# cc-ai/MUNIT

Hardware: AMD Instinct MI355X
Metric: images/sec (gen_update+dis_update) @256x256 bs=8 (higher is better)
Workload: dtype f32; 1 GPU; config_256.yaml AdaINGen_double+MsImageDis dis_update+gen_update, 256x256, per-GPU batch 8, fp32; global_batch=8, parallelism=dp1, gen_state=1

## Files before the change

### include/munit_hip.h

```cpp
#ifndef MUNIT_HIP_H
#define MUNIT_HIP_H

#include <stddef.h>
#include <stdint.h>

#ifdef __cplusplus
extern "C" {
#endif

typedef void* munit_stream_t;

enum { MUNIT_OK = 0, MUNIT_ERR_ARG = -1, MUNIT_ERR_WORKSPACE = -2, MUNIT_ERR_LAUNCH = -3 };
enum { MUNIT_ACT_NONE = 0, MUNIT_ACT_RELU = 1, MUNIT_ACT_LRELU = 2, MUNIT_ACT_TANH = 3 };
enum { MUNIT_PAD_ZERO = 0, MUNIT_PAD_REFLECT = 1 };
enum { MUNIT_COMPUTE_F32 = 0, MUNIT_COMPUTE_BF16 = 1, MUNIT_COMPUTE_F32X3 = 2 };
enum { MUNIT_DTYPE_F32 = 0, MUNIT_DTYPE_BF16 = 1 };

int munit_version(void);
const char* munit_last_error(void);

typedef void* munit_comm_t;
int munit_comm_unique_id(void* id_out, size_t bytes);
int munit_comm_init(munit_comm_t* comm, int rank, int world, const void* unique_id);
int munit_comm_allreduce(munit_comm_t comm, float* buf, size_t count, munit_stream_t stream);
int munit_comm_destroy(munit_comm_t comm);
int munit_shutdown(void);

int munit_stream_wait_stream(munit_stream_t waiter, munit_stream_t signaler);

typedef struct {
  int B, H, W, Cin;
  int Cout, KH, KW;
  int stride, pad, pad_mode;
  int upsample;
  int act;
  float slope;
  int compute;
  int in_dtype, out_dtype;
} munit_conv_desc;

int munit_conv2d_out_hw(const munit_conv_desc* d, int* Ho, int* Wo);

size_t munit_conv2d_fwd_workspace_bytes(const munit_conv_desc* d);
int munit_conv2d_fwd(const munit_conv_desc* d, const void* x, const float* w, const float* bias,
                     void* y, void* ws, size_t ws_bytes, munit_stream_t stream);

size_t munit_conv2d_dgrad_workspace_bytes(const munit_conv_desc* d);
int munit_conv2d_dgrad(const munit_conv_desc* d, const void* dy, const float* w, const void* add,
                       void* dx, void* ws, size_t ws_bytes, munit_stream_t stream);

size_t munit_conv2d_wgrad_workspace_bytes(const munit_conv_desc* d);
int munit_conv2d_wgrad(const munit_conv_desc* d, const void* x, const void* dy, float* dw,
                       float* db, float beta, void* ws, size_t ws_bytes, munit_stream_t stream);

enum { MUNIT_PASS_FWD = 0, MUNIT_PASS_DGRAD = 1, MUNIT_PASS_WGRAD = 2 };
enum { MUNIT_PREP_NONE = 0, MUNIT_PREP_DGRAD = 1, MUNIT_PREP_SUBPIXEL = 2, MUNIT_PREP_CAST = 3,
       MUNIT_PREP_WINOGRAD = 4, MUNIT_PREP_WINOGRAD_DGRAD = 5, MUNIT_PREP_SUBPIXEL_WINOGRAD = 6,
       MUNIT_PREP_WINOGRAD_S2 = 7, MUNIT_PREP_WINOGRAD_S2_DGRAD = 8,
       MUNIT_PREP_SUBPIXEL_WINOGRAD_DGRAD = 9  };
typedef struct {
  const float* w;
  float* wp;
  int Cout, KH, KW, Cin;
  int kind;
  int ps;
  int bf16;
} munit_prep_item;
size_t munit_conv2d_prepared_weight_bytes(const munit_conv_desc* d, int pass);
int munit_conv2d_prep_item(const munit_conv_desc* d, int pass, const float* w, float* wp, munit_prep_item* out);
int munit_conv2d_prepare_weights(const munit_prep_item* item, munit_stream_t stream);
int munit_conv2d_prepare_weights_batch(const munit_prep_item* items_dev, int n, munit_stream_t stream);
int munit_conv2d_fwd_prepared(const munit_conv_desc* d, const void* x, const float* w, const void* wp,
                              const float* bias, void* y, void* ws, size_t ws_bytes, munit_stream_t stream);
int munit_conv2d_dgrad_prepared(const munit_conv_desc* d, const void* dy, const float* w, const void* wp,
                                const void* add, void* dx, void* ws, size_t ws_bytes, munit_stream_t stream);

size_t munit_linear_workspace_bytes(int B, int K, int N);
int munit_linear_fwd(const float* x, const float* w, const float* bias, float* y, int B, int K, int N, int act,
                     float slope, void* ws, size_t ws_bytes, munit_stream_t stream);
int munit_linear_bwd(const float* x, const float* w, const float* dy, float* dx, float* dw, float* db, int B, int K,
                     int N, float beta, void* ws, size_t ws_bytes, munit_stream_t stream);

double munit_conv2d_executed_flops(const munit_conv_desc* d, int pass);
const char* munit_conv2d_kernel_name(const munit_conv_desc* d, int pass);

int munit_act_bwd(int act, float slope, const float* y, const float* dy, float* dx, size_t n,
                  munit_stream_t stream);

size_t munit_instnorm_workspace_bytes(int B, int HW, int C);
int munit_instnorm_fwd(const float* x, float* y, float* stats, int B, int HW, int C,
                       const float* adain, int ad_ld, int w_off, int b_off, const float* residual,
                       int relu, float eps, void* ws, size_t ws_bytes, munit_stream_t stream);
int munit_instnorm_bwd(const float* x, const float* dy, const float* stats, float* dx, int B, int HW,
                       int C, const float* adain, float* d_adain, int ad_ld, int w_off, int b_off,
                       int relu, void* ws, size_t ws_bytes, munit_stream_t stream);

int munit_instnorm_route(int B, int HW, int C, int dtype);

int munit_instnorm_fwd_bf16(const void* x, void* y, float* stats, int B, int HW, int C,
                            const float* adain, int ad_ld, int w_off, int b_off, const void* residual,
                            int relu, float eps, void* ws, size_t ws_bytes, munit_stream_t stream);
int munit_instnorm_bwd_bf16(const void* x, const void* dy, const float* stats, void* dx, int B, int HW,
                            int C, const float* adain, float* d_adain, int ad_ld, int w_off, int b_off,
                            int relu, void* ws, size_t ws_bytes, munit_stream_t stream);

size_t munit_layernorm_workspace_bytes(int B, int HW, int C);
int munit_layernorm_fwd(const float* x, float* y, float* stats, int B, int HW, int C,
                        const float* gamma, const float* beta, int relu, float eps, void* ws,
                        size_t ws_bytes, munit_stream_t stream);
int munit_layernorm_bwd(const float* x, const float* dy, const float* stats, float* dx, int B, int HW,
                        int C, const float* gamma, const float* beta, float* dgamma, float* dbeta,
                        float acc, int relu, float eps, void* ws, size_t ws_bytes,
                        munit_stream_t stream);

int munit_layernorm_fwd_bf16(const void* x, void* y, float* stats, int B, int HW, int C,
                             const float* gamma, const float* beta, int relu, float eps, void* ws,
                             size_t ws_bytes, munit_stream_t stream);
int munit_layernorm_bwd_bf16(const void* x, const void* dy, const float* stats, void* dx, int B, int HW,
                             int C, const float* gamma, const float* beta, float* dgamma, float* dbeta,
                             float acc, int relu, float eps, void* ws, size_t ws_bytes,
                             munit_stream_t stream);

int munit_avgpool3s2_fwd(const float* x, float* y, int B, int H, int W, int C, munit_stream_t stream);
int munit_avgpool3s2_bwd(const float* dy, float* dx, int B, int H, int W, int C, munit_stream_t stream);
int munit_gap_fwd(const float* x, float* y, int B, int HW, int C, munit_stream_t stream);
int munit_gap_bwd(const float* dy, float* dx, int B, int HW, int C, munit_stream_t stream);

size_t munit_loss_workspace_bytes(size_t n);
int munit_l1_mean_fwd(const float* a, const float* b, const float* mask, size_t npix, int C, float* out,
                      void* ws, size_t ws_bytes, munit_stream_t stream);
int munit_l1_mean_bwd(const float* a, const float* b, const float* mask, size_t npix, int C,
                      const float* gout, float* da, float* db, munit_stream_t stream);
int munit_l1_mean_fwd_bf16(const void* a, const void* b, const float* mask, size_t npix, int C, float* out,
                           void* ws, size_t ws_bytes, munit_stream_t stream);
int munit_l1_mean_bwd_bf16(const void* a, const void* b, const float* mask, size_t npix, int C,
                           const float* gout, void* da, void* db, munit_stream_t stream);
int munit_pair_l1_fwd(const float* x_a, const float* x_b, const float* x_ab, const float* x_ba, size_t npix, int C,
                      float* out, void* ws, size_t ws_bytes, munit_stream_t stream);
int munit_pair_l1_bwd(const float* x_a, const float* x_b, const float* x_ab, const float* x_ba, size_t npix, int C,
                      const float* gout, float* dx_ab, float* dx_ba, munit_stream_t stream);
int munit_mse_const_fwd(const float* x, float target, size_t n, float* out, void* ws, size_t ws_bytes,
                        munit_stream_t stream);
int munit_mse_const_bwd(const float* x, float target, size_t n, const float* gout, float* dx,
                        munit_stream_t stream);
size_t munit_lsgan_workspace_bytes(int nseg);
int munit_lsgan_fwd(const float* const* x, const size_t* n, const float* target, int nseg, float* out, float* seg_out,
                    void* ws, size_t ws_bytes, munit_stream_t stream);
int munit_lsgan_bwd(const float* const* x, const size_t* n, const float* target, int nseg, const float* gout,
                    float* const* dx, munit_stream_t stream);
size_t munit_nsgan_workspace_bytes(int nseg);
int munit_nsgan_fwd(const float* const* x, const size_t* n, const float* target, int nseg, float* out, float* seg_out,
                    void* ws, size_t ws_bytes, munit_stream_t stream);
int munit_nsgan_bwd(const float* const* x, const size_t* n, const float* target, int nseg, const float* gout,
                    float* const* dx, munit_stream_t stream);
int munit_weighted_sum(const float* const* terms, const float* w, int n, float* out,
                       munit_stream_t stream);

int munit_adam_step(float* p, const float* g, float* m, float* v, size_t n, double lr, double beta1,
                    double beta2, double eps, double weight_decay, int step, munit_stream_t stream);

int munit_extraadam_step(float* p, const float* g, float* m, float* v, float* p_saved, size_t n, double lr,
                         double beta1, double beta2, double eps, double weight_decay, int step, int mode,
                         munit_stream_t stream);

int munit_scale(const float* x, float* y, size_t n, float alpha, int accumulate, munit_stream_t stream);

typedef struct {
  long long src_off;
  int src_h, src_w;
  int rs_h, rs_w;
  int crop_i, crop_j;
  int flip;
  int kind;
} munit_image_desc;

int munit_image_ksize(int src_size, int rs_size);
size_t munit_image_preprocess_workspace_bytes(int B, int out_h, int out_w, int ksize_max);
int munit_image_preprocess(const unsigned char* pool, const munit_image_desc* descs, int B, int out_h,
                           int out_w, int ksize_max, float* out, void* ws, size_t ws_bytes,
                           munit_stream_t stream);
size_t munit_mask_preprocess_workspace_bytes(int B, int out_h, int out_w);
int munit_mask_preprocess(const unsigned char* pool, const munit_image_desc* descs, int B, int out_h,
                          int out_w, float* out, void* ws, size_t ws_bytes, munit_stream_t stream);
size_t munit_label_preprocess_workspace_bytes(int N, int out_h, int out_w);
int munit_label_preprocess(const unsigned char* pool, const munit_image_desc* descs, int N, int out_h,
                           int out_w, float* out, void* ws, size_t ws_bytes, munit_stream_t stream);

typedef struct {
  const float* data;
  int n;
  int channels;
  int layout;
} munit_grid_src;

size_t munit_image_grid_workspace_bytes(int nsrc, int H, int W, int nrow);
int munit_image_grid_u8(const munit_grid_src* src, int nsrc, int H, int W, int nrow, float pre_add, float pre_mul,
                        unsigned char* out, void* ws, size_t ws_bytes, munit_stream_t stream);

int munit_seg_input_fwd(const float* x, float* y, size_t npix, munit_stream_t stream);
int munit_seg_input_bwd(const float* dy, float* dx, size_t npix, munit_stream_t stream);
int munit_space_to_batch(const float* x, float* y, int N, int H, int W, int C, int f, int inverse, munit_stream_t stream);
int munit_maxpool3s2_fwd(const float* x, float* y, unsigned char* idx, int B, int H, int W, int C, munit_stream_t stream);
int munit_maxpool3s2_bwd(const float* dy, const unsigned char* idx, float* dx, int B, int H, int W, int C,
                         munit_stream_t stream);
int munit_add_relu_fwd(const float* a, const float* r, float* y, size_t n, munit_stream_t stream);
size_t munit_seg_ce_workspace_bytes(int B, int h, int w, int S);
int munit_seg_ce_fwd(const float* logits, const int* labels, const float* mask, int B, int h, int w, int S, float norm,
                     float* out, void* ws, size_t ws_bytes, munit_stream_t stream);
int munit_seg_ce_bwd(const float* logits, const int* labels, const float* mask, int B, int h, int w, int S, float norm,
                     const float* gout, float* dlogits, void* ws, size_t ws_bytes, munit_stream_t stream);
int munit_seg_ce_gt_fwd(const float* logits, const float* gt, const float* mask, int B, int h, int w, int S, float norm,
                        float* out, void* ws, size_t ws_bytes, munit_stream_t stream);
int munit_seg_ce_gt_bwd(const float* logits, const float* gt, const float* mask, int B, int h, int w, int S, float norm,
                        const float* gout, float* dlogits, void* ws, size_t ws_bytes, munit_stream_t stream);

size_t munit_seg_ce_direct_workspace_bytes(int B, int h, int w, int S, int K);
int munit_seg_ce_direct_fwd(const float* logits, const float* gt, int B, int h, int w, int S, int K, float norm, float* out,
                            void* ws, size_t ws_bytes, munit_stream_t stream);
int munit_seg_ce_direct_bwd(const float* logits, const float* gt, int B, int h, int w, int S, int K, float norm,
                            const float* gout, float* dlogits, void* ws, size_t ws_bytes, munit_stream_t stream);
int munit_avgpool7_fwd(const float* x, float* y, int B, int H, int W, int C, munit_stream_t stream);
int munit_avgpool7_bwd(const float* dy, float* dx, int B, int H, int W, int C, munit_stream_t stream);
int munit_seg_labels(const float* logits, int B, int h, int w, int S, int* labels, munit_stream_t stream);

size_t munit_batchnorm_workspace_bytes(int C);
int munit_batchnorm_fwd(const float* x, float* y, float* mean, float* rstd, float* running_mean, float* running_var,
                        long long R, int C, const float* gamma, const float* beta, int relu, int eval, float eps,
                        float momentum, void* ws, size_t ws_bytes, munit_stream_t stream);
int munit_batchnorm_bwd(const float* x, const float* dy, const float* y, const float* gamma, const float* mean,
                        const float* rstd, float* dx, float* dgamma, float* dbeta, float acc, long long R, int C,
                        int relu, void* ws, size_t ws_bytes, munit_stream_t stream);
size_t munit_batchnorm_dp_workspace_bytes(int C);
int munit_batchnorm_dp_stats_local(const float* x, long long R_local, int C, int W, int rank, float* xch, size_t xch_floats,
                                   void* ws, size_t ws_bytes, munit_stream_t stream);
int munit_batchnorm_dp_fwd_apply(const float* x, float* y, float* mean, float* rstd, float* running_mean, float* running_var,
                                 long long R_local, int C, int W, const float* xch, size_t xch_floats, const float* gamma,
                                 const float* beta, int relu, float eps, float momentum, munit_stream_t stream);
// ... 52 lines not shown
```

### munit_amd/_lib.py

```python
import ctypes
import os
from ctypes import POINTER, Structure, c_char_p, c_double, c_float, c_int, c_size_t, c_void_p

_HERE = os.path.dirname(os.path.abspath(__file__))
LIB_PATH = os.environ.get("MUNIT_HIP_LIB") or os.path.join(_HERE, "libmunit_hip.so")

ACT = {"none": 0, "relu": 1, "lrelu": 2, "tanh": 3}
PAD = {"zero": 0, "reflect": 1}
COMPUTE = {"f32": 0, "bf16": 1, "f32x3": 2}
DTYPE = {"f32": 0, "bf16": 1}


class ConvDesc(Structure):
    _fields_ = [("B", c_int), ("H", c_int), ("W", c_int), ("Cin", c_int),
                ("Cout", c_int), ("KH", c_int), ("KW", c_int),
                ("stride", c_int), ("pad", c_int), ("pad_mode", c_int),
                ("upsample", c_int), ("act", c_int), ("slope", c_float), ("compute", c_int),
                ("in_dtype", c_int), ("out_dtype", c_int)]


class PrepItem(Structure):
    _fields_ = [("w", c_void_p), ("wp", c_void_p), ("Cout", c_int), ("KH", c_int), ("KW", c_int), ("Cin", c_int),
                ("kind", c_int), ("ps", c_int), ("bf16", c_int)]


class ImageDesc(Structure):
    _fields_ = [("src_off", ctypes.c_longlong), ("src_h", c_int), ("src_w", c_int), ("rs_h", c_int), ("rs_w", c_int),
                ("crop_i", c_int), ("crop_j", c_int), ("flip", c_int), ("kind", c_int)]


class GemmProblem(Structure):
    _fields_ = [("A", c_void_p), ("B", c_void_p), ("C", c_void_p)]


class GridSrc(Structure):
    _fields_ = [("data", c_void_p), ("n", c_int), ("channels", c_int), ("layout", c_int)]


class RectDesc(Structure):
    _fields_ = [("B", c_int), ("H", c_int), ("W", c_int), ("Cin", c_int), ("x_ld", c_int), ("Cout", c_int), ("y_ld", c_int),
                ("KH", c_int), ("KW", c_int), ("stride", c_int), ("pad_h", c_int), ("pad_w", c_int), ("relu", c_int)]


WINDOW = {"max": 0, "avg": 1}
RECT_TILES = ("128x128", "64x64", "128x64")

_P = c_void_p
_DESC = POINTER(ConvDesc)

SIGNATURES = {
    "munit_version": (c_int, []),
    "munit_last_error": (c_char_p, []),
    "munit_stream_wait_stream": (c_int, [_P, _P]),
    "munit_comm_unique_id": (c_int, [_P, c_size_t]),
    "munit_comm_init": (c_int, [_P, c_int, c_int, _P]),
    "munit_comm_allreduce": (c_int, [_P, _P, c_size_t, _P]),
    "munit_comm_destroy": (c_int, [_P]),
    "munit_shutdown": (c_int, []),
    "munit_conv2d_out_hw": (c_int, [_DESC, POINTER(c_int), POINTER(c_int)]),
    "munit_conv2d_fwd_workspace_bytes": (c_size_t, [_DESC]),
    "munit_conv2d_fwd": (c_int, [_DESC, _P, _P, _P, _P, _P, c_size_t, _P]),
    "munit_conv2d_dgrad_workspace_bytes": (c_size_t, [_DESC]),
    "munit_conv2d_dgrad": (c_int, [_DESC, _P, _P, _P, _P, _P, c_size_t, _P]),
    "munit_conv2d_wgrad_workspace_bytes": (c_size_t, [_DESC]),
    "munit_conv2d_wgrad": (c_int, [_DESC, _P, _P, _P, _P, c_float, _P, c_size_t, _P]),
    "munit_conv2d_prepared_weight_bytes": (c_size_t, [_DESC, c_int]),
    "munit_conv2d_prep_item": (c_int, [_DESC, c_int, _P, _P, POINTER(PrepItem)]),
    "munit_conv2d_prepare_weights": (c_int, [POINTER(PrepItem), _P]),
    "munit_conv2d_prepare_weights_batch": (c_int, [_P, c_int, _P]),
    "munit_conv2d_fwd_prepared": (c_int, [_DESC, _P, _P, _P, _P, _P, _P, c_size_t, _P]),
    "munit_conv2d_dgrad_prepared": (c_int, [_DESC, _P, _P, _P, _P, _P, _P, c_size_t, _P]),
    "munit_conv2d_executed_flops": (c_double, [_DESC, c_int]),
    "munit_conv2d_kernel_name": (c_char_p, [_DESC, c_int]),
    "munit_linear_workspace_bytes": (c_size_t, [c_int, c_int, c_int]),
    "munit_linear_fwd": (c_int, [_P, _P, _P, _P, c_int, c_int, c_int, c_int, c_float, _P, c_size_t, _P]),
    "munit_linear_bwd": (c_int, [_P, _P, _P, _P, _P, _P, c_int, c_int, c_int, c_float, _P, c_size_t, _P]),
    "munit_act_bwd": (c_int, [c_int, c_float, _P, _P, _P, c_size_t, _P]),
    "munit_instnorm_workspace_bytes": (c_size_t, [c_int, c_int, c_int]),
    "munit_instnorm_route": (c_int, [c_int, c_int, c_int, c_int]),
    "munit_instnorm_fwd": (c_int, [_P, _P, _P, c_int, c_int, c_int, _P, c_int, c_int, c_int, _P, c_int,
                                   c_float, _P, c_size_t, _P]),
    "munit_instnorm_bwd": (c_int, [_P, _P, _P, _P, c_int, c_int, c_int, _P, _P, c_int, c_int, c_int, c_int,
                                   _P, c_size_t, _P]),
    "munit_instnorm_fwd_bf16": (c_int, [_P, _P, _P, c_int, c_int, c_int, _P, c_int, c_int, c_int, _P, c_int,
                                        c_float, _P, c_size_t, _P]),
    "munit_instnorm_bwd_bf16": (c_int, [_P, _P, _P, _P, c_int, c_int, c_int, _P, _P, c_int, c_int, c_int, c_int,
                                        _P, c_size_t, _P]),
    "munit_layernorm_workspace_bytes": (c_size_t, [c_int, c_int, c_int]),
    "munit_layernorm_fwd": (c_int, [_P, _P, _P, c_int, c_int, c_int, _P, _P, c_int, c_float, _P, c_size_t, _P]),
    "munit_layernorm_bwd": (c_int, [_P, _P, _P, _P, c_int, c_int, c_int, _P, _P, _P, _P, c_float, c_int,
                                    c_float, _P, c_size_t, _P]),
    "munit_layernorm_fwd_bf16": (c_int, [_P, _P, _P, c_int, c_int, c_int, _P, _P, c_int, c_float, _P, c_size_t, _P]),
    "munit_layernorm_bwd_bf16": (c_int, [_P, _P, _P, _P, c_int, c_int, c_int, _P, _P, _P, _P, c_float, c_int,
                                         c_float, _P, c_size_t, _P]),
    "munit_avgpool3s2_fwd": (c_int, [_P, _P, c_int, c_int, c_int, c_int, _P]),
    "munit_avgpool3s2_bwd": (c_int, [_P, _P, c_int, c_int, c_int, c_int, _P]),
    "munit_gap_fwd": (c_int, [_P, _P, c_int, c_int, c_int, _P]),
    "munit_gap_bwd": (c_int, [_P, _P, c_int, c_int, c_int, _P]),
    "munit_loss_workspace_bytes": (c_size_t, [c_size_t]),
    "munit_l1_mean_fwd": (c_int, [_P, _P, _P, c_size_t, c_int, _P, _P, c_size_t, _P]),
    "munit_l1_mean_bwd": (c_int, [_P, _P, _P, c_size_t, c_int, _P, _P, _P, _P]),
    "munit_l1_mean_fwd_bf16": (c_int, [_P, _P, _P, c_size_t, c_int, _P, _P, c_size_t, _P]),
    "munit_l1_mean_bwd_bf16": (c_int, [_P, _P, _P, c_size_t, c_int, _P, _P, _P, _P]),
    "munit_pair_l1_fwd": (c_int, [_P, _P, _P, _P, c_size_t, c_int, _P, _P, c_size_t, _P]),
    "munit_pair_l1_bwd": (c_int, [_P, _P, _P, _P, c_size_t, c_int, _P, _P, _P, _P]),
    "munit_mse_const_fwd": (c_int, [_P, c_float, c_size_t, _P, _P, c_size_t, _P]),
    "munit_mse_const_bwd": (c_int, [_P, c_float, c_size_t, _P, _P, _P]),
    "munit_lsgan_workspace_bytes": (c_size_t, [c_int]),
    "munit_lsgan_fwd": (c_int, [POINTER(c_void_p), POINTER(c_size_t), POINTER(c_float), c_int, _P, _P, _P, c_size_t, _P]),
    "munit_lsgan_bwd": (c_int, [POINTER(c_void_p), POINTER(c_size_t), POINTER(c_float), c_int, _P, POINTER(c_void_p), _P]),
    "munit_nsgan_workspace_bytes": (c_size_t, [c_int]),
    "munit_nsgan_fwd": (c_int, [POINTER(c_void_p), POINTER(c_size_t), POINTER(c_float), c_int, _P, _P, _P, c_size_t, _P]),
    "munit_nsgan_bwd": (c_int, [POINTER(c_void_p), POINTER(c_size_t), POINTER(c_float), c_int, _P, POINTER(c_void_p), _P]),
    "munit_weighted_sum": (c_int, [POINTER(c_void_p), POINTER(c_float), c_int, _P, _P]),
    "munit_adam_step": (c_int, [_P, _P, _P, _P, c_size_t, c_double, c_double, c_double, c_double, c_double, c_int,
                                _P]),
    "munit_extraadam_step": (c_int, [_P, _P, _P, _P, _P, c_size_t, c_double, c_double, c_double, c_double,
                                     c_double, c_int, c_int, _P]),
    "munit_scale": (c_int, [_P, _P, c_size_t, c_float, c_int, _P]),
    "munit_image_ksize": (c_int, [c_int, c_int]),
    "munit_image_preprocess_workspace_bytes": (c_size_t, [c_int, c_int, c_int, c_int]),
    "munit_image_preprocess": (c_int, [_P, _P, c_int, c_int, c_int, c_int, _P, _P, c_size_t, _P]),
    "munit_mask_preprocess_workspace_bytes": (c_size_t, [c_int, c_int, c_int]),
    "munit_mask_preprocess": (c_int, [_P, _P, c_int, c_int, c_int, _P, _P, c_size_t, _P]),
    "munit_label_preprocess_workspace_bytes": (c_size_t, [c_int, c_int, c_int]),
    "munit_label_preprocess": (c_int, [_P, _P, c_int, c_int, c_int, _P, _P, c_size_t, _P]),
    "munit_image_grid_workspace_bytes": (c_size_t, [c_int, c_int, c_int, c_int]),
    "munit_image_grid_u8": (c_int, [POINTER(GridSrc), c_int, c_int, c_int, c_int, c_float, c_float, _P, _P, c_size_t, _P]),
    "munit_seg_input_fwd": (c_int, [_P, _P, c_size_t, _P]),
    "munit_seg_input_bwd": (c_int, [_P, _P, c_size_t, _P]),
    "munit_space_to_batch": (c_int, [_P, _P, c_int, c_int, c_int, c_int, c_int, c_int, _P]),
    "munit_maxpool3s2_fwd": (c_int, [_P, _P, _P, c_int, c_int, c_int, c_int, _P]),
    "munit_maxpool3s2_bwd": (c_int, [_P, _P, _P, c_int, c_int, c_int, c_int, _P]),
    "munit_add_relu_fwd": (c_int, [_P, _P, _P, c_size_t, _P]),
    "munit_seg_ce_workspace_bytes": (c_size_t, [c_int, c_int, c_int, c_int]),
    "munit_seg_ce_fwd": (c_int, [_P, _P, _P, c_int, c_int, c_int, c_int, c_float, _P, _P, c_size_t, _P]),
    "munit_seg_ce_bwd": (c_int, [_P, _P, _P, c_int, c_int, c_int, c_int, c_float, _P, _P, _P, c_size_t, _P]),
    "munit_seg_ce_gt_fwd": (c_int, [_P, _P, _P, c_int, c_int, c_int, c_int, c_float, _P, _P, c_size_t, _P]),
    "munit_seg_ce_gt_bwd": (c_int, [_P, _P, _P, c_int, c_int, c_int, c_int, c_float, _P, _P, _P, c_size_t, _P]),
    "munit_seg_labels": (c_int, [_P, c_int, c_int, c_int, c_int, _P, _P]),
    "munit_seg_ce_direct_workspace_bytes": (c_size_t, [c_int, c_int, c_int, c_int, c_int]),
    "munit_seg_ce_direct_fwd": (c_int, [_P, _P, c_int, c_int, c_int, c_int, c_int, c_float, _P, _P, c_size_t, _P]),
    "munit_seg_ce_direct_bwd": (c_int, [_P, _P, c_int, c_int, c_int, c_int, c_int, c_float, _P, _P, _P, c_size_t, _P]),
    "munit_avgpool7_fwd": (c_int, [_P, _P, c_int, c_int, c_int, c_int, _P]),
    "munit_avgpool7_bwd": (c_int, [_P, _P, c_int, c_int, c_int, c_int, _P]),
    "munit_batchnorm_workspace_bytes": (c_size_t, [c_int]),
    "munit_batchnorm_fwd": (c_int, [_P, _P, _P, _P, _P, _P, ctypes.c_longlong, c_int, _P, _P, c_int, c_int, c_float, c_float,
                                    _P, c_size_t, _P]),
    "munit_batchnorm_bwd": (c_int, [_P, _P, _P, _P, _P, _P, _P, _P, _P, c_float, ctypes.c_longlong, c_int, c_int, _P,
                                    c_size_t, _P]),
    "munit_batchnorm_dp_workspace_bytes": (c_size_t, [c_int]),
    "munit_batchnorm_dp_stats_local": (c_int, [_P, ctypes.c_longlong, c_int, c_int, c_int, _P, c_size_t, _P, c_size_t, _P]),
    "munit_batchnorm_dp_fwd_apply": (c_int, [_P, _P, _P, _P, _P, _P, ctypes.c_longlong, c_int, c_int, _P, c_size_t, _P, _P,
                                             c_int, c_float, c_float, _P]),
    "munit_batchnorm_dp_bwd_local": (c_int, [_P, _P, _P, _P, _P, ctypes.c_longlong, c_int, c_int, c_int, c_int, _P, c_size_t,
                                             _P, c_size_t, _P]),
    "munit_batchnorm_dp_bwd_finish": (c_int, [_P, _P, _P, _P, _P, _P, _P, _P, _P, c_float, ctypes.c_longlong, c_int, c_int,
                                              c_int, c_int, _P, c_size_t, _P, c_size_t, _P]),
    "munit_maxpool2_fwd": (c_int, [_P, _P, _P, c_int, c_int, c_int, c_int, _P]),
    "munit_maxpool2_bwd": (c_int, [_P, _P, _P, c_int, c_int, c_int, c_int, _P]),
    "munit_avgpool16_fwd": (c_int, [_P, _P, c_int, c_int, c_int, c_int, _P]),
    "munit_avgpool16_bwd": (c_int, [_P, _P, c_int, c_int, c_int, c_int, _P]),
    "munit_gemm_f32": (c_int, [POINTER(GemmProblem), c_int, c_int, c_int, c_int, c_int, c_int, c_int, c_int, c_float,
                               c_float, _P]),
    "munit_fid_moments_workspace_bytes": (c_size_t, [c_int, c_int]),
    "munit_fid_moments": (c_int, [_P, c_int, c_int, _P, _P, _P, c_size_t, _P]),
    "munit_sqrt_newton_schulz_workspace_bytes": (c_size_t, [c_int, c_int]),
    "munit_sqrt_newton_schulz": (c_int, [_P, c_int, c_int, c_int, _P, _P, c_size_t, _P]),
    "munit_frechet_distance_workspace_bytes": (c_size_t, [c_int]),
    "munit_frechet_distance": (c_int, [_P, _P, _P, _P, c_int, c_int, _P, _P, c_size_t, _P]),
    "munit_conv2d_rect_out_hw": (c_int, [POINTER(RectDesc), POINTER(c_int), POINTER(c_int)]),
    "munit_conv2d_rect_tile": (c_int, [POINTER(RectDesc)]),
    "munit_conv2d_rect_fwd": (c_int, [POINTER(RectDesc), _P, _P, _P, _P, c_int, _P]),
    "munit_window3_fwd": (c_int, [_P, _P, c_int, c_int, c_int, c_int, c_int, c_int, c_int, c_int, c_int, _P]),
    "munit_inception_input": (c_int, [_P, c_int, c_int, c_int, c_int, _P, _P]),
}

_lib = None


def load():
    global _lib
    if _lib is not None:
        return _lib
    if not os.path.exists(LIB_PATH):
        raise RuntimeError(
            "munit_amd: %s not found. Build it with `python -c 'import __graft_entry__ as g; g.build()'` "
            "(or `make -C munit_amd/csrc`). There is no CPU / PyTorch fallback." % LIB_PATH)
    lib = ctypes.CDLL(LIB_PATH)
    for name, (res, args) in SIGNATURES.items():
        try:
            fn = getattr(lib, name)
        except AttributeError as e:
            raise RuntimeError("munit_amd: %s does not export %s" % (LIB_PATH, name)) from e
        fn.restype = res
        fn.argtypes = args
    _lib = lib
    return lib


def check(rc, what=""):
    if rc != 0:
        msg = load().munit_last_error()
        raise RuntimeError("munit_hip %s failed (rc=%d): %s" % (what, rc, (msg or b"").decode()))
```

### munit_amd/csrc/common.h

```cpp
#pragma once
#include <hip/hip_runtime.h>
#include <cstdarg>
#include <cstdio>
#include <cstdlib>
#include "../../include/munit_hip.h"

typedef float f32x4 __attribute__((ext_vector_type(4)));
typedef float f32x16 __attribute__((ext_vector_type(16)));

typedef __bf16 bf16_t;
typedef __bf16 bf16v4 __attribute__((ext_vector_type(4)));
typedef __bf16 bf16v8 __attribute__((ext_vector_type(8)));

__device__ inline f32x4 ld4(const float* p) { return *reinterpret_cast<const f32x4*>(p); }
__device__ inline f32x4 ld4(const bf16_t* p) {
  const bf16v4 h = *reinterpret_cast<const bf16v4*>(p);
  return f32x4{(float)h[0], (float)h[1], (float)h[2], (float)h[3]};
}
__device__ inline void st4(float* p, f32x4 v) { *reinterpret_cast<f32x4*>(p) = v; }
__device__ inline void st4(bf16_t* p, f32x4 v) {
  *reinterpret_cast<bf16v4*>(p) = bf16v4{(bf16_t)v[0], (bf16_t)v[1], (bf16_t)v[2], (bf16_t)v[3]};
}
__device__ inline float ld1(const float* p) { return *p; }
__device__ inline float ld1(const bf16_t* p) { return (float)*p; }
__device__ inline void st1(float* p, float v) { *p = v; }
__device__ inline void st1(bf16_t* p, float v) { *p = (bf16_t)v; }

void munit_set_error(const char* fmt, ...);

#define MUNIT_CHECK_ARG(cond, ...)         \
  do {                                     \
    if (!(cond)) {                         \
      munit_set_error(__VA_ARGS__);        \
      return MUNIT_ERR_ARG;                \
    }                                      \
  } while (0)

#define MUNIT_CHECK_LAUNCH(what)                                                   \
  do {                                                                             \
    hipError_t e_ = hipGetLastError();                                             \
    if (e_ != hipSuccess) {                                                        \
      munit_set_error("%s: launch failed: %s", what, hipGetErrorString(e_));       \
      return MUNIT_ERR_LAUNCH;                                                     \
    }                                                                              \
  } while (0)

#define MUNIT_ENV_FLAG(name) ([]() -> bool { static const bool v_ = getenv(name) != nullptr; return v_; }())

static inline size_t align_up(size_t v, size_t a) { return (v + a - 1) / a * a; }
static inline int cdiv(long long a, long long b) { return (int)((a + b - 1) / b); }

__device__ inline float wave_sum(float v) {
#pragma unroll
  for (int off = 32; off > 0; off >>= 1) v += __shfl_xor(v, off, 64);
  return v;
}

__device__ inline float apply_act(float v, int act, float slope) {
  if (act == MUNIT_ACT_RELU) return v > 0.f ? v : 0.f;
  if (act == MUNIT_ACT_LRELU) return v > 0.f ? v : v * slope;
  if (act == MUNIT_ACT_TANH) return tanhf(v);
  return v;
}

__device__ inline int src_coord(int v, int Hu, int ups, int reflect) {
  const bool inside = v >= 0 && v < Hu;
  int r = v < 0 ? -v : v;
  r = r >= Hu ? 2 * Hu - 2 - r : r;
  r = reflect ? r : (inside ? v : -1);
  return r < 0 ? -1 : (r >> ups);
}

double munit_igemm_executed_flops(const munit_conv_desc* d, int pass);
const char* munit_igemm_kernel_name(const munit_conv_desc* d, int pass);

bool munit_small_fwd_supported(const munit_conv_desc* d);
bool munit_small_fwd_ok(const munit_conv_desc* d);
bool munit_small_wgrad_ok(const munit_conv_desc* d);
enum SmallFwdKernel { SMALL_FWD_PK, SMALL_FWD_MFMA, SMALL_FWD_PATCH };
SmallFwdKernel munit_small_fwd_kernel(int Cin);
bool munit_small_wgrad_pk();
size_t munit_small_fwd_workspace(const munit_conv_desc* d);
int munit_small_fwd(const munit_conv_desc* d, int Ho, int Wo, const void* x, const float* w, const float* bias,
                    float* y, void* ws, hipStream_t st);
size_t munit_small_wgrad_workspace(const munit_conv_desc* d, int Ho);
int munit_small_wgrad(const munit_conv_desc* d, int Ho, int Wo, const void* x, const float* dy, float* dw,
                      float* db, float beta, void* ws, hipStream_t st);
```

### munit_amd/csrc/conv_igemm.hip

```cpp
#include "common.h"
#include "wino.h"
#include <cstdlib>

namespace {

struct IgemmParams {
  const float* x;
  const float* w;
  const float* bias;
  void* y;
  int B, H, W, Cin;
  int Hu, Wu, ups;
  int Ho, Wo, Cout;
  int KH, KW, stride, pad, reflect;
  int Ktot;
  long long w_row;
  long long y_sb;
  long long y_sh;
  int y_sw;
  int M;
  int act;
  float slope;
  int ps;
  long long w_phase;
  long long y_phase_row;
  int y_phase_col;
  int n_tiles;
  int f_pad, f_ups, f_reflect, f_Hu, f_Wu;
  int frame;
  int ksplit, kt_per_split;
  float* slab;
  int ct;
  int patch;
  int out_bf16;
  int bf16s;
  int cin4;
};

__device__ inline f32x4 bf16x8_add4(f32x4 l, f32x4 a, f32x4 b, f32x4 c) {
  const bf16v8 L = __builtin_bit_cast(bf16v8, l), A = __builtin_bit_cast(bf16v8, a), B = __builtin_bit_cast(bf16v8, b),
               C = __builtin_bit_cast(bf16v8, c);
  bf16v8 r;
#pragma unroll
  for (int e = 0; e < 8; ++e) r[e] = (bf16_t)((float)L[e] + (((float)A[e] + (float)B[e]) + (float)C[e]));
  return __builtin_bit_cast(f32x4, r);
}

__device__ inline void decode_pixel(int m, int Ho, int Wo, int frame, int& b, int& oh, int& ow) {
  if (!frame) {
    const int HoWo = Ho * Wo;
    b = m / HoWo;
    const int rem = m - b * HoWo;
    oh = rem / Wo;
    ow = rem - oh * Wo;
  } else {
    const int F = frame, F2 = 2 * frame;
    const int nb = F2 * Wo + F2 * (Ho - F2);
    b = m / nb;
    int r = m - b * nb;
    if (r < F2 * Wo) {
      const int q = r / Wo;
      ow = r - q * Wo;
      oh = q < F ? q : Ho - F2 + q;
    } else {
      r -= F2 * Wo;
      const int rr = r / F2, q = r - rr * F2;
      oh = F + rr;
      ow = q < F ? q : Wo - F2 + q;
    }
  }
}

constexpr int BM = 128;
constexpr int BK = 32;
#ifndef IGEMM_WAVES
#define IGEMM_WAVES 8
#endif
constexpr int NWAVES = IGEMM_WAVES;
constexpr int NTHR = 64 * NWAVES;
constexpr int LDS_LD = BK + 4;

__device__ inline uint2 fold_cands(int i, int Hu, int ups, int P, int reflect) {
  unsigned long long pk = ~0ull;
  int n = 0;
  auto push = [&](int v) {
    if (n < 4) {
      const int sh = 16 * n;
      pk = (pk & ~(0xFFFFull << sh)) | ((unsigned long long)(unsigned)v << sh);
      ++n;
    }
  };
  const int nu = 1 << ups;
  for (int du = 0; du < nu; ++du) {
    const int hu = (i << ups) + du;
    push(hu + P);
    if (reflect) {
      if (hu >= 1 && hu <= P) push(P - hu);
      if (hu >= Hu - 1 - P && hu <= Hu - 2) push(2 * Hu - 2 - hu + P);
    }
  }
  return make_uint2((unsigned)(pk & 0xFFFFFFFFull), (unsigned)(pk >> 32));
}
__device__ inline int cand_at(uint2 v, int a) {
  const unsigned w = (a & 2) ? v.y : v.x;
  return (int)((w >> ((a & 1) * 16)) & 0xFFFFu);
}

typedef __bf16 bf16x4 __attribute__((ext_vector_type(4)));
typedef __bf16 bf16x8 __attribute__((ext_vector_type(8)));

__device__ const float munit_zero_page[32] = {0.f};

template <int BN, bool ALIGNED, int ROLE, int CT = 0>
__global__ __launch_bounds__(NTHR, NWAVES == 8 ? ((CT == 3 && BN == 64) ? 6 : 4) : 2) void conv_igemm_kernel(IgemmParams p) {
  constexpr bool BF16 = CT == 1 || CT == 2;
  constexpr bool DMA = CT == 3 || CT == 4 || CT == 5;
  constexpr bool BF16S = CT == 4;
  constexpr bool CIN4 = CT == 5;
  static_assert(!CIN4 || ROLE != 2, "4-channel taps: single-gather roles only");
  static_assert(!DMA || (ALIGNED && NWAVES == 8), "direct-to-LDS loads: aligned variants only");
  constexpr bool PATCH = DMA && ROLE == 2;
  constexpr int NPL = CT == 2 ? 3 : 1;
  static_assert(!BF16 || ALIGNED, "bf16 operands need Cin % 32 == 0");
  constexpr int WN = NWAVES == 8 ? 32 : 64;
  constexpr int WAVES_N = BN / WN;
  constexpr int WAVES_M = NWAVES / WAVES_N;
  constexpr int WM = BM / WAVES_M;
  constexpr int MT = WM / 16;
  constexpr int NT = WN / 16;
#ifndef IGEMM_LOADER_WAVES
#define IGEMM_LOADER_WAVES 8
#endif
  constexpr int LW = (CT == 3 && ROLE != 2 && NWAVES == 8) ? IGEMM_LOADER_WAVES : NWAVES;
  constexpr int RSTEP = 64 * LW / 8;
  constexpr int AROWS = BM / RSTEP;
  constexpr int BROWS = BN / RSTEP;
  constexpr int CLD = BN + 4;
  static_assert(BM * CLD <= 2 * (BM + BN) * LDS_LD, "C staging tile must fit in the operand buffers");
  constexpr int SMEM_FLOATS = DMA ? (2 * (BM + BN) * 32 > BM * CLD ? 2 * (BM + BN) * 32 : BM * CLD) : 2 * (BM + BN) * LDS_LD;
  __shared__ __attribute__((aligned(16))) float smem[SMEM_FLOATS];
  float* const As = smem;
  float* const Bs = smem + 2 * BM * LDS_LD;

  const int tid = threadIdx.x;
  const int lane = tid & 63;
  const int wave = tid >> 6;
  const int wm = wave / WAVES_N, wn = wave % WAVES_N;

  int tile = blockIdx.x;
  {
    const int nb = gridDim.x, q = nb >> 3, r = nb & 7, xcd = tile & 7, idx = tile >> 3;
    tile = (xcd < r ? xcd * (q + 1) : r * (q + 1) + (xcd - r) * q) + idx;
  }
  const int n_tile = tile % p.n_tiles;
  const int m_tile = tile / p.n_tiles;
  const int m0 = m_tile * BM;
  const int n0 = n_tile * BN;

  const float* __restrict__ xg = p.x;
  const float* __restrict__ wg = p.w;
  long long y_base = 0;
  if (p.ps > 1) {
    const int pa = blockIdx.y / p.ps, pb = blockIdx.y % p.ps;
    wg += (long long)blockIdx.y * p.w_phase;
    y_base = (long long)pa * p.y_phase_row + (long long)pb * p.y_phase_col;
  }

  const int c4 = tid & 7;
  const int r0 = tid >> 3;
  int a_base[AROWS];
  int a_ih0[AROWS], a_iw0[AROWS];
  bool a_ok[AROWS];
  uint2 a_ch[AROWS], a_cw[AROWS];
  int a_nc[AROWS];
  int f_h1[PATCH ? AROWS : 1], f_w1[PATCH ? AROWS : 1];
#pragma unroll
  for (int i = 0; i < AROWS; ++i) {
    int m = m0 + r0 + RSTEP * i;
    a_ok[i] = m < p.M;
    int mm = a_ok[i] ? m : 0;
    int b, oh, ow;
    decode_pixel(mm, p.Ho, p.Wo, p.frame, b, oh, ow);
    a_base[i] = b * p.H * p.W;
    a_ih0[i] = oh * p.stride - p.pad;
    a_iw0[i] = ow * p.stride - p.pad;
    if constexpr (PATCH) {
      constexpr int NONE = -(1 << 20);
      const int P = p.f_pad, K1 = p.KH - 1;
      int h1 = NONE, w1 = NONE;
      if (p.f_reflect) {
        if (oh >= 1 && oh <= P) h1 = P - oh - K1;
        else if (oh >= p.f_Hu - 1 - P && oh <= p.f_Hu - 2) h1 = 2 * p.f_Hu - 2 - oh + P - K1;
        if (ow >= 1 && ow <= P) w1 = P - ow - K1;
        else if (ow >= p.f_Wu - 1 - P && ow <= p.f_Wu - 2) w1 = 2 * p.f_Wu - 2 - ow + P - K1;
      }
      a_ih0[i] = oh + P - K1;
      a_iw0[i] = ow + P - K1;
      f_h1[i] = h1;
      f_w1[i] = w1;
    } else if constexpr (ROLE == 2) {
      a_ch[i] = fold_cands(oh, p.f_Hu, p.f_ups, p.f_pad, p.f_reflect);
      a_cw[i] = fold_cands(ow, p.f_Wu, p.f_ups, p.f_pad, p.f_reflect);
      int nh = 0, nw = 0;
      for (int a = 0; a < 4; ++a) {
        nh += cand_at(a_ch[i], a) != 0xFFFF;
        nw += cand_at(a_cw[i], a) != 0xFFFF;
      }
      a_nc[i] = nh | (nw << 4);
    }
  }

  f32x4 ra[AROWS], rb[BROWS];
  f32x4 rx[ROLE == 2 ? AROWS : 1];
  int kh = 0, kw = 0, c0 = 0;
  const int nk_total = (p.Ktot + BK - 1) / BK;
  const int kt_begin = p.ksplit > 1 ? blockIdx.z * p.kt_per_split : 0;
  const int kt_end = p.ksplit > 1 ? min(nk_total, kt_begin + p.kt_per_split) : nk_total;
  if constexpr (ALIGNED) {
    if (kt_begin > 0) {
      const int k0 = kt_begin * BK, tap = k0 / p.Cin;
      c0 = k0 - tap * p.Cin;
      kh = tap / p.KW;
      kw = tap - kh * p.KW;
    }
  }
  int aoff[AROWS];
  int aoff1[ROLE == 2 ? AROWS : 1];
  int aoffp[PATCH ? 3 : 1][AROWS];
  f32x4 xp[PATCH ? 3 : 1][AROWS];
  bool wave_patch = false;

  auto tap_setup = [&]() {
#pragma unroll
    for (int i = 0; i < AROWS; ++i) {
      if constexpr (PATCH) {
        const int vh0 = a_ih0[i] + kh, vh1 = f_h1[i] + kh, vw0 = a_iw0[i] + kw, vw1 = f_w1[i] + kw;
        const bool h0 = a_ok[i] && (unsigned)vh0 < (unsigned)p.H, h1 = a_ok[i] && (unsigned)vh1 < (unsigned)p.H;
        const bool w0 = (unsigned)vw0 < (unsigned)p.W, w1 = (unsigned)vw1 < (unsigned)p.W;
        aoff[i] = (h0 && w0) ? (a_base[i] + vh0 * p.W + vw0) * p.Cin : -1;
        aoffp[0][i] = (h0 && w1) ? (a_base[i] + vh0 * p.W + vw1) * p.Cin : -1;
        aoffp[1][i] = (h1 && w0) ? (a_base[i] + vh1 * p.W + vw0) * p.Cin : -1;
        aoffp[2][i] = (h1 && w1) ? (a_base[i] + vh1 * p.W + vw1) * p.Cin : -1;
        if (i == 0) wave_patch = false;
        wave_patch = wave_patch || __builtin_amdgcn_ballot_w64((aoffp[0][i] & aoffp[1][i] & aoffp[2][i]) >= 0) != 0;
      } else if constexpr (ROLE == 2) {
        const int nw = a_nc[i] >> 4;
        const int ncomb = (a_nc[i] & 15) * nw;
        int o0 = -1, o1 = -1;
        {
          const int vh = cand_at(a_ch[i], 0) + kh - (p.KH - 1);
          const int vw = cand_at(a_cw[i], 0) + kw - (p.KW - 1);
          const bool ok = a_ok[i] && vh >= 0 && vh < p.H && vw >= 0 && vw < p.W;
          o0 = ok ? (a_base[i] + vh * p.W + vw) * p.Cin : -1;
        }
        {
          const int vh = cand_at(a_ch[i], nw >= 2 ? 0 : 1) + kh - (p.KH - 1);
          const int vw = cand_at(a_cw[i], nw >= 2 ? 1 : 0) + kw - (p.KW - 1);
          const bool ok = a_ok[i] && ncomb >= 2 && vh >= 0 && vh < p.H && vw >= 0 && vw < p.W;
          o1 = ok ? (a_base[i] + vh * p.W + vw) * p.Cin : -1;
        }
        aoff[i] = o0;
        aoff1[i] = o1;
      } else {
        const int ih = src_coord(a_ih0[i] + kh, p.Hu, p.ups, p.reflect);
        const int iw = src_coord(a_iw0[i] + kw, p.Wu, p.ups, p.reflect);
        const bool ok = a_ok[i] && ih >= 0 && iw >= 0;
// ... 205 lines not shown
#pragma unroll
      for (int pl = 0; pl < NPL; ++pl)
#pragma unroll
        for (int nt = 0; nt < NT; ++nt)
          hb[pl][nt] = *reinterpret_cast<const bf16x8*>(&Bc[pl * (BN * 32) + (wn * WN + nt * 16 + frag_row) * 32 + fr_col]);
#pragma unroll
      for (int mt = kg * (MT / 2); mt < (kg + 1) * (MT / 2); ++mt) {
        bf16x8 ha[NPL];
#pragma unroll
        for (int pl = 0; pl < NPL; ++pl)
          ha[pl] = *reinterpret_cast<const bf16x8*>(&Ac[pl * (BM * 32) + (wm * WM + mt * 16 + frag_row) * 32 + fr_col]);
#pragma unroll
        for (int sum = NPL - 1; sum >= 0; --sum)
#pragma unroll
          for (int i = 0; i <= sum; ++i)
#pragma unroll
            for (int nt = 0; nt < NT; ++nt)
              acc[mt][nt] = __builtin_amdgcn_mfma_f32_16x16x32_bf16(ha[i], hb[sum - i][nt], acc[mt][nt], 0, 0, 0);
      }
      return;
    }
    if constexpr (DMA) {
      const float* Ac = smem + buf * (BM * 32);
      const float* Bc = smem + 2 * BM * 32 + buf * (BN * 32);
      const int pos = ((kg * 4 + (lane >> 4)) ^ ((frag_row >> 1) & 7)) * 4;
      f32x4 a[MT], b[NT];
#pragma unroll
      for (int nt = 0; nt < NT; ++nt)
        b[nt] = *reinterpret_cast<const f32x4*>(&Bc[(wn * WN + nt * 16 + frag_row) * 32 + pos]);
#pragma unroll
      for (int mt = 0; mt < MT; ++mt)
        a[mt] = *reinterpret_cast<const f32x4*>(&Ac[(wm * WM + mt * 16 + frag_row) * 32 + pos]);
      if constexpr (BF16S) {
#pragma unroll
        for (int mt = 0; mt < MT; ++mt)
#pragma unroll
          for (int nt = 0; nt < NT; ++nt)
            acc[mt][nt] = __builtin_amdgcn_mfma_f32_16x16x32_bf16(__builtin_bit_cast(bf16x8, a[mt]),
                                                                  __builtin_bit_cast(bf16x8, b[nt]), acc[mt][nt], 0, 0, 0);
        return;
      }
#pragma unroll
      for (int t = 0; t < 4; ++t)
#pragma unroll
        for (int mt = 0; mt < MT; ++mt)
#pragma unroll
          for (int nt = 0; nt < NT; ++nt)
            acc[mt][nt] = __builtin_amdgcn_mfma_f32_16x16x4f32(a[mt][t], b[nt][t], acc[mt][nt], 0, 0, 0);
      return;
    }
    const float* Ac = As + buf * (BM * LDS_LD);
    const float* Bc = Bs + buf * (BN * LDS_LD);
    f32x4 a[MT], b[NT];
#pragma unroll
    for (int nt = 0; nt < NT; ++nt)
      b[nt] = *reinterpret_cast<const f32x4*>(&Bc[(wn * WN + nt * 16 + frag_row) * LDS_LD + kg * 16 + frag_k]);
    constexpr int MB = (ROLE == 2 && MT >= 4) ? MT / 2 : MT;
#pragma unroll
    for (int m0t = 0; m0t < MT; m0t += MB) {
#pragma unroll
      for (int mt = m0t; mt < m0t + MB; ++mt)
        a[mt] = *reinterpret_cast<const f32x4*>(&Ac[(wm * WM + mt * 16 + frag_row) * LDS_LD + kg * 16 + frag_k]);
#pragma unroll
      for (int t = 0; t < 4; ++t)
#pragma unroll
        for (int mt = m0t; mt < m0t + MB; ++mt)
#pragma unroll
          for (int nt = 0; nt < NT; ++nt)
            acc[mt][nt] = __builtin_amdgcn_mfma_f32_16x16x4f32(a[mt][t], b[nt][t], acc[mt][nt], 0, 0, 0);
      if constexpr (MB != MT) __builtin_amdgcn_sched_barrier(0);
    }
  };

  const int nk = kt_end - kt_begin;
  auto patch_tile = [&](int buf) {
    if constexpr (PATCH) {
      if (!wave_patch) return;
#pragma unroll
      for (int i = 0; i < AROWS; ++i) {
        if ((aoffp[0][i] & aoffp[1][i] & aoffp[2][i]) >= 0) {
          f32x4* l = reinterpret_cast<f32x4*>(smem + buf * (BM * 32) + (r0 + RSTEP * i) * 32 + c4 * 4);
          if constexpr (BF16S) *l = bf16x8_add4(*l, xp[0][i], xp[1][i], xp[2][i]);
          else *l = *l + ((xp[0][i] + xp[1][i]) + xp[2][i]);
        }
      }
    }
  };
  if constexpr (DMA) {
    if (nk > 0) dma_tile(kt_begin, 0);
    asm volatile("s_waitcnt vmcnt(0)" ::: "memory");
    if (nk > 0) patch_tile(0);
    __syncthreads();
    for (int kt = 0; kt < nk; ++kt) {
      const int cur = kt & 1;
      if (kt + 1 < nk) dma_tile(kt_begin + kt + 1, cur ^ 1);
      compute_half(cur, 0);
      compute_half(cur, 1);
      asm volatile("s_waitcnt vmcnt(0)" ::: "memory");
      if (kt + 1 < nk) patch_tile(cur ^ 1);
      __syncthreads();
    }
  } else if constexpr (CT == 2) {
    if (nk > 0) load_tile(kt_begin);
    for (int kt = 0; kt < nk; ++kt) {
      __syncthreads();
      store_tile(0);
      if (kt + 1 < nk) load_tile(kt_begin + kt + 1);
      __syncthreads();
      compute_half(0, 0);
      compute_half(0, 1);
    }
    __syncthreads();
  } else {
    if (nk > 0) {
      load_tile(kt_begin);
      store_tile(0);
    }
    __syncthreads();
    if (nk > 1) load_tile(kt_begin + 1);
    for (int kt = 0; kt < nk; ++kt) {
      const int cur = kt & 1;
      compute_half(cur, 0);
      if (kt + 1 < nk) {
#ifndef ABL_NOLDSW
        store_tile(cur ^ 1);
#endif
#ifndef ABL_NOGLOBAL
        if (kt + 2 < nk) load_tile(kt_begin + kt + 2);
#endif
      }
      if constexpr (ROLE == 2) __builtin_amdgcn_sched_barrier(0);
      compute_half(cur, 1);
#ifndef ABL_NOBAR
      __syncthreads();
#endif
    }
  }

  float* const Cs = smem;
#pragma unroll
  for (int nt = 0; nt < NT; ++nt)
#pragma unroll
    for (int mt = 0; mt < MT; ++mt)
#pragma unroll
      for (int r = 0; r < 4; ++r)
        Cs[(wm * WM + mt * 16 + 4 * (lane >> 4) + r) * CLD + wn * WN + nt * 16 + (lane & 15)] = acc[mt][nt][r];
  __syncthreads();
  constexpr int CQ = BN / 4;
  constexpr int CRPT = NTHR / CQ;
  const int cq = tid % CQ, cr0 = tid / CQ;
  const int n = n0 + cq * 4;
  const bool split = p.ksplit > 1;
  float* const sl = split ? p.slab + ((long long)blockIdx.y * p.ksplit + blockIdx.z) * (long long)p.M * p.Cout : nullptr;
  const bool vec = (p.Cout & 3) == 0 && (split || ((p.y_sw & 3) == 0 && (p.y_sh & 3) == 0 && (p.y_sb & 3) == 0));
  f32x4 bv = {0.f, 0.f, 0.f, 0.f};
  if (!split && p.bias != nullptr) {
#pragma unroll
    for (int e = 0; e < 4; ++e)
      if (n + e < p.Cout) bv[e] = p.bias[n + e];
  }
#pragma unroll 2
  for (int row = cr0; row < BM; row += CRPT) {
    const int m = m0 + row;
    if (m >= p.M || n >= p.Cout) continue;
    f32x4 v = *reinterpret_cast<const f32x4*>(&Cs[row * CLD + cq * 4]);
    if (split) {
      float* dst = sl + (long long)m * p.Cout + n;
      if (vec) {
        *reinterpret_cast<f32x4*>(dst) = v;
      } else {
#pragma unroll
        for (int e = 0; e < 4; ++e)
          if (n + e < p.Cout) dst[e] = v[e];
      }
      continue;
    }
    int b, oh, ow;
    decode_pixel(m, p.Ho, p.Wo, p.frame, b, oh, ow);
    const long long off = y_base + (long long)b * p.y_sb + (long long)oh * p.y_sh + (long long)ow * p.y_sw + n;
#pragma unroll
    for (int e = 0; e < 4; ++e) v[e] = apply_act(v[e] + bv[e], p.act, p.slope);
    if (p.out_bf16) {
      bf16_t* dst = reinterpret_cast<bf16_t*>(p.y) + off;
      if (vec) {
        st4(dst, v);
      } else {
#pragma unroll
        for (int e = 0; e < 4; ++e)
          if (n + e < p.Cout) dst[e] = (bf16_t)v[e];
      }
    } else {
      float* dst = reinterpret_cast<float*>(p.y) + off;
      if (vec) {
        *reinterpret_cast<f32x4*>(dst) = v;
      } else {
#pragma unroll
        for (int e = 0; e < 4; ++e)
          if (n + e < p.Cout) dst[e] = v[e];
      }
    }
  }
}

__global__ void splitk_epilogue_kernel(IgemmParams p, int phases) {
  const long long per = (long long)p.M * p.Cout;
  const long long total = per * phases;
  for (long long i = (long long)blockIdx.x * blockDim.x + threadIdx.x; i < total;
       i += (long long)gridDim.x * blockDim.x) {
    const int ph = (int)(i / per);
    const long long r = i - (long long)ph * per;
    const int m = (int)(r / p.Cout), n = (int)(r - (long long)m * p.Cout);
    float s = 0.f;
    for (int k = 0; k < p.ksplit; ++k) s += p.slab[((long long)ph * p.ksplit + k) * per + r];
    int b, oh, ow;
    decode_pixel(m, p.Ho, p.Wo, p.frame, b, oh, ow);
    long long off = (long long)b * p.y_sb + (long long)oh * p.y_sh + (long long)ow * p.y_sw + n;
    if (p.ps > 1) off += (long long)(ph / p.ps) * p.y_phase_row + (long long)(ph % p.ps) * p.y_phase_col;
    const float bv = p.bias != nullptr ? p.bias[n] : 0.f;
    const float res = apply_act(s + bv, p.act, p.slope);
    if (p.out_bf16) reinterpret_cast<bf16_t*>(p.y)[off] = (bf16_t)res;
    else reinterpret_cast<float*>(p.y)[off] = res;
  }
}

typedef munit_prep_item PrepItem;

__device__ inline void prep_dgrad_elem(const PrepItem& it, long long i) {
  const int ps = it.ps, TH = it.KH / ps, TW = it.KW / ps;
  long long r_ = i;
  int co = (int)(r_ % it.Cout); r_ /= it.Cout;
  int r = (int)(r_ % TW); r_ /= TW;
  int t = (int)(r_ % TH); r_ /= TH;
  int ci = (int)(r_ % it.Cin); r_ /= it.Cin;
  int ph = (int)r_;
  int pa = ph / ps, pb = ph % ps;
  int kh = pa + ps * (TH - 1 - t);
  int kw = pb + ps * (TW - 1 - r);
  const float v = it.w[(((long long)co * it.KH + kh) * it.KW + kw) * it.Cin + ci];
  if (it.bf16) reinterpret_cast<bf16_t*>(it.wp)[i] = (bf16_t)v;
  else it.wp[i] = v;
}

__device__ inline void prep_cast_elem(const PrepItem& it, long long i) { reinterpret_cast<bf16_t*>(it.wp)[i] = (bf16_t)it.w[i]; }

__device__ inline void prep_subpixel_elem(const PrepItem& it, long long i) {
  const long long merged = (long long)4 * 9 * it.Cout * it.Cin;
  if (i >= merged) {
    reinterpret_cast<bf16_t*>(it.wp)[i] = (bf16_t)it.w[i - merged];
    return;
  }
  long long r = i;
  const int ci = (int)(r % it.Cin); r /= it.Cin;
  const int dw = (int)(r % 3); r /= 3;
  const int dh = (int)(r % 3); r /= 3;
  const int co = (int)(r % it.Cout); r /= it.Cout;
  const int ph = (int)r;
  const int a = ph >> 1, b = ph & 1;
  const int h0 = a == 0 ? (dh == 0 ? 0 : dh == 1 ? 2 : 4) : (dh == 0 ? 0 : dh == 1 ? 1 : 3);
  const int hn = a == 0 ? (dh == 2 ? 1 : 2) : (dh == 0 ? 1 : 2);
  const int w0 = b == 0 ? (dw == 0 ? 0 : dw == 1 ? 2 : 4) : (dw == 0 ? 0 : dw == 1 ? 1 : 3);
  const int wn = b == 0 ? (dw == 2 ? 1 : 2) : (dw == 0 ? 1 : 2);
  float s = 0.f;
  for (int kh = h0; kh < h0 + hn; ++kh)
    for (int kw = w0; kw < w0 + wn; ++kw) s += it.w[(((long long)co * 5 + kh) * 5 + kw) * it.Cin + ci];
  if (it.bf16) reinterpret_cast<bf16_t*>(it.wp)[i] = (bf16_t)s;
  else it.wp[i] = s;
}

__host__ __device__ inline long long prep_elems(const PrepItem& it) {
  const long long cc = (long long)it.Cout * it.Cin;
  if (it.kind == MUNIT_PREP_SUBPIXEL) return it.bf16 ? (4 * 9 + 25) * cc : 4 * 9 * cc;
  if (it.kind == MUNIT_PREP_WINOGRAD || it.kind == MUNIT_PREP_WINOGRAD_DGRAD) return wino_image_elems(it.Cin, it.Cout);
  if (it.kind == MUNIT_PREP_SUBPIXEL_WINOGRAD_DGRAD) return cc * it.KH * it.KW + 4 * wino_image_elems(it.Cin, it.Cout);
  if (it.kind == MUNIT_PREP_SUBPIXEL_WINOGRAD || it.kind == MUNIT_PREP_WINOGRAD_S2 || it.kind == MUNIT_PREP_WINOGRAD_S2_DGRAD)
    return 4 * wino_image_elems(it.Cin, it.Cout);
  return cc * it.KH * it.KW;
}

__host__ __device__ inline long long prep_trips(const PrepItem& it) {
  const bool wino = it.kind == MUNIT_PREP_WINOGRAD || it.kind == MUNIT_PREP_WINOGRAD_DGRAD || it.kind == MUNIT_PREP_SUBPIXEL_WINOGRAD ||
                    it.kind == MUNIT_PREP_WINOGRAD_S2 || it.kind == MUNIT_PREP_WINOGRAD_S2_DGRAD;
  if (it.kind == MUNIT_PREP_SUBPIXEL_WINOGRAD_DGRAD) return (long long)it.Cout * it.Cin * (it.KH * it.KW + 4);
  return wino ? prep_elems(it) / 16 : prep_elems(it);
}
template <bool DEV>
__global__ void prep_weights_kernel(const PrepItem* __restrict__ items, PrepItem one) {
  const PrepItem it = DEV ? items[blockIdx.y] : one;
  const long long total = prep_trips(it);
  for (long long i = (long long)blockIdx.x * blockDim.x + threadIdx.x; i < total; i += (long long)gridDim.x * blockDim.x) {
    if (it.kind == MUNIT_PREP_SUBPIXEL) prep_subpixel_elem(it, i);
    else if (it.kind == MUNIT_PREP_WINOGRAD || it.kind == MUNIT_PREP_WINOGRAD_DGRAD)
      wino_weight_item(it.w, it.wp, it.Cout, it.Cin, it.kind == MUNIT_PREP_WINOGRAD_DGRAD, i);
    else if (it.kind == MUNIT_PREP_SUBPIXEL_WINOGRAD) wino_subpixel_weight_item(it.w, it.wp, it.Cout, it.Cin, i);
    else if (it.kind == MUNIT_PREP_WINOGRAD_S2) wino_s2_weight_item(it.w, it.wp, it.Cout, it.Cin, i);
    else if (it.kind == MUNIT_PREP_WINOGRAD_S2_DGRAD) wino_s2_dgrad_weight_item(it.w, it.wp, it.Cout, it.Cin, i);
    else if (it.kind == MUNIT_PREP_SUBPIXEL_WINOGRAD_DGRAD) {
      const long long nd = (long long)it.Cout * it.Cin * it.KH * it.KW;
      if (i < nd) prep_dgrad_elem(it, i);
      else wino_subpixel_dgrad_weight_item(it.w, it.wp + nd, it.Cout, it.Cin, i - nd);
    }
    else if (it.kind == MUNIT_PREP_CAST) prep_cast_elem(it, i);
    else prep_dgrad_elem(it, i);
  }
}

int launch_prep_one(const PrepItem& it, hipStream_t st) {
  const long long total = prep_trips(it);
  const int blocks = (int)std::min<long long>((total + 255) / 256, 4096);
  hipLaunchKernelGGL(prep_weights_kernel<false>, dim3(blocks), dim3(256), 0, st, nullptr, it);
  MUNIT_CHECK_LAUNCH("prep_weights");
  return MUNIT_OK;
}

template <typename T>
__global__ void fold_kernel(const T* __restrict__ g, const T* __restrict__ add,
                            T* __restrict__ dx, int B, int H, int W, int C, int ups, int pad,
                            int reflect, int Hq, int Wq) {
  const int C4 = C >> 2;
  const long long total = (long long)B * H * W * C4;
  const int Hu = H << ups, Wu = W << ups;
  for (long long i = (long long)blockIdx.x * blockDim.x + threadIdx.x; i < total;
       i += (long long)gridDim.x * blockDim.x) {
    long long r_ = i;
    int c4 = (int)(r_ % C4); r_ /= C4;
    int iw = (int)(r_ % W); r_ /= W;
    int ih = (int)(r_ % H); r_ /= H;
    int b = (int)r_;
    f32x4 s = {0.f, 0.f, 0.f, 0.f};
    const int nu = 1 << ups;
    for (int du = 0; du < nu; ++du) {
      int hu = (ih << ups) + du;
      int qr[3], nr = 0;
      qr[nr++] = hu + pad;
      if (reflect) {
        if (hu >= 1 && hu <= pad) qr[nr++] = pad - hu;
        if (hu >= Hu - 1 - pad && hu <= Hu - 2) qr[nr++] = 2 * Hu - 2 - hu + pad;
      }
      for (int dv = 0; dv < nu; ++dv) {
        int wu = (iw << ups) + dv;
        int qc[3], nc = 0;
        qc[nc++] = wu + pad;
        if (reflect) {
          if (wu >= 1 && wu <= pad) qc[nc++] = pad - wu;
          if (wu >= Wu - 1 - pad && wu <= Wu - 2) qc[nc++] = 2 * Wu - 2 - wu + pad;
        }
        for (int a = 0; a < nr; ++a) {
          if (qr[a] >= Hq) continue;
          for (int c = 0; c < nc; ++c) {
            if (qc[c] >= Wq) continue;
            s += ld4(g + (((long long)b * Hq + qr[a]) * Wq + qc[c]) * C + c4 * 4);
          }
        }
      }
    }
    if (add != nullptr) s += ld4(add + i * 4);
    st4(dx + i * 4, s);
  }
}

__global__ void fold_scalar_kernel(const float* __restrict__ g, const float* __restrict__ add,
                                   float* __restrict__ dx, int B, int H, int W, int C, int ups, int pad,
                                   int reflect, int Hq, int Wq) {
  const long long total = (long long)B * H * W * C;
  const int Hu = H << ups, Wu = W << ups;
  for (long long i = (long long)blockIdx.x * blockDim.x + threadIdx.x; i < total;
       i += (long long)gridDim.x * blockDim.x) {
    long long r_ = i;
    int c = (int)(r_ % C); r_ /= C;
    int iw = (int)(r_ % W); r_ /= W;
    int ih = (int)(r_ % H); r_ /= H;
    int b = (int)r_;
    float s = 0.f;
    const int nu = 1 << ups;
    for (int du = 0; du < nu; ++du) {
      int hu = (ih << ups) + du;
      int qr[3], nr = 0;
      qr[nr++] = hu + pad;
      if (reflect) {
        if (hu >= 1 && hu <= pad) qr[nr++] = pad - hu;
        if (hu >= Hu - 1 - pad && hu <= Hu - 2) qr[nr++] = 2 * Hu - 2 - hu + pad;
      }
      for (int dv = 0; dv < nu; ++dv) {
        int wu = (iw << ups) + dv;
        int qc[3], nc = 0;
        qc[nc++] = wu + pad;
        if (reflect) {
          if (wu >= 1 && wu <= pad) qc[nc++] = pad - wu;
          if (wu >= Wu - 1 - pad && wu <= Wu - 2) qc[nc++] = 2 * Wu - 2 - wu + pad;
        }
        for (int a = 0; a < nr; ++a) {
          if (qr[a] >= Hq) continue;
          for (int cc = 0; cc < nc; ++cc) {
            if (qc[cc] >= Wq) continue;
            s += g[(((long long)b * Hq + qr[a]) * Wq + qc[cc]) * C + c];
          }
        }
      }
    }
    if (add != nullptr) s += add[i];
    dx[i] = s;
  }
}

__global__ void add_inplace_kernel(float* __restrict__ y, const float* __restrict__ a, long long n) {
  for (long long i = (long long)blockIdx.x * blockDim.x + threadIdx.x; i < n; i += (long long)gridDim.x * blockDim.x)
    y[i] += a[i];
}

int pick_ksplit(int M, int Cout, int Ktot, int phases) {
  const int bn = Cout <= 64 ? 64 : 128;
  const int tiles = cdiv(M, BM) * cdiv(Cout, bn) * phases;
  const int nk = cdiv(Ktot, BK);
  if (tiles >= 192 || nk < 16 || MUNIT_ENV_FLAG("MUNIT_DEBUG_NO_SPLITK")) return 1;
  int ks = std::min(cdiv(512, tiles), nk / 4);
  return std::max(1, std::min(ks, 32));
}
size_t splitk_bytes(int M, int Cout, int Ktot, int phases) {
  const int ks = pick_ksplit(M, Cout, Ktot, phases);
  return ks > 1 ? align_up((size_t)ks * phases * M * Cout * sizeof(float), 256) : 0;
}

enum IgemmForm {
  IG_REFUSED_BF16_CIN, IG_REFUSED_CIN4_FOLD, IG_REFUSED_BF16_FOLD, IG_REFUSED_FOLD_UNALIGNED,
  IG_CIN4,
  IG_BF16S,
  IG_PATCH,
  IG_DMA,
  IG_CT2,
  IG_CT1,
  IG_F32,
  IG_UNALIGNED
};
IgemmForm igemm_form(const IgemmParams& p, int role) {
  if (p.bf16s && (p.Cin % (2 * BK) != 0 || NWAVES != 8)) return IG_REFUSED_BF16_CIN;
  const int cin = p.bf16s ? p.Cin / 2 : p.Cin, w_row = p.bf16s ? p.w_row / 2 : p.w_row;
  const bool aligned = (cin % BK == 0) && (w_row % 4 == 0);
  if (p.cin4) return role == 2 ? IG_REFUSED_CIN4_FOLD : IG_CIN4;
  if (p.bf16s) return role == 2 && (!p.patch || p.frame) ? IG_REFUSED_BF16_FOLD : IG_BF16S;
  if (role == 2) {
    if (!aligned) return IG_REFUSED_FOLD_UNALIGNED;
    if (p.ct == 0 && p.patch && !p.frame && NWAVES == 8 && !MUNIT_ENV_FLAG("MUNIT_DEBUG_NO_PATCH")) return IG_PATCH;
    return p.ct == 2 ? IG_CT2 : p.ct == 1 ? IG_CT1 : IG_F32;
  }
  if (aligned && p.ct == 0 && NWAVES == 8 && !MUNIT_ENV_FLAG("MUNIT_DEBUG_NO_DMA")) return IG_DMA;
  if (!aligned) return IG_UNALIGNED;
  return p.ct == 2 ? IG_CT2 : p.ct == 1 ? IG_CT1 : IG_F32;
}
int igemm_bn(const IgemmParams& p) { return p.Cout <= 64 ? 64 : 128; }

#define IGEMM_LAUNCH(...)                                                                                  \
  do {                                                                                                     \
    if (bn == 64) hipLaunchKernelGGL((conv_igemm_kernel<64, __VA_ARGS__>), grid, block, 0, st, q);         \
    else hipLaunchKernelGGL((conv_igemm_kernel<128, __VA_ARGS__>), grid, block, 0, st, q);                 \
  } while (0)

template <int ROLE>
int launch_igemm(const IgemmParams& p, int phases, hipStream_t st, void* slab = nullptr, size_t slab_bytes = 0) {
  const int bn = igemm_bn(p);
  IgemmParams q = p;
  const IgemmForm form = igemm_form(p, ROLE);
  switch (form) {
    case IG_REFUSED_BF16_CIN:
      munit_set_error("conv_igemm: bf16 storage needs a multiple of 64 input channels (got %d)", p.Cin);
      return MUNIT_ERR_ARG;
    case IG_REFUSED_CIN4_FOLD:
      munit_set_error("conv_igemm: 4-channel taps are not a folded-backward-data form");
      return MUNIT_ERR_ARG;
    case IG_REFUSED_BF16_FOLD:
      munit_set_error("conv_igemm: bf16-storage folded backward-data exists for the LDS-patch form only");
      return MUNIT_ERR_ARG;
    case IG_REFUSED_FOLD_UNALIGNED:
      munit_set_error("conv_igemm: folded backward-data needs Cout %% 32 == 0");
      return MUNIT_ERR_ARG;
    default: break;
  }
  if (p.bf16s) {
    q.Cin = p.Cin / 2; q.Ktot = p.Ktot / 2; q.w_row = p.w_row / 2; q.w_phase = p.w_phase / 2;
    slab = nullptr;
  }
  q.n_tiles = cdiv(p.Cout, bn);
  const int m_tiles = cdiv(p.M, BM);
  q.ksplit = 1;
  if (slab != nullptr) {
    const int ks = pick_ksplit(p.M, p.Cout, p.Ktot, phases);
    if (ks > 1 && slab_bytes >= splitk_bytes(p.M, p.Cout, p.Ktot, phases)) {
      const int nk = cdiv(p.Ktot, BK);
      q.kt_per_split = cdiv(nk, ks);
      q.ksplit = cdiv(nk, q.kt_per_split);
      q.slab = reinterpret_cast<float*>(slab);
    }
  }
  dim3 grid((unsigned)(m_tiles * q.n_tiles), (unsigned)phases, (unsigned)q.ksplit);
  dim3 block(NTHR);
  switch (form) {
    case IG_CIN4:
      if constexpr (ROLE != 2) IGEMM_LAUNCH(true, ROLE, 5);
      break;
    case IG_BF16S: IGEMM_LAUNCH(true, ROLE, 4); break;
    case IG_PATCH: IGEMM_LAUNCH(true, 2, 3); break;
    case IG_DMA: IGEMM_LAUNCH(true, ROLE, 3); break;
    case IG_CT2: IGEMM_LAUNCH(true, ROLE, 2); break;
    case IG_CT1: IGEMM_LAUNCH(true, ROLE, 1); break;
    case IG_F32: IGEMM_LAUNCH(true, ROLE); break;
    default:
      if constexpr (ROLE != 2) IGEMM_LAUNCH(false, ROLE);
      break;
  }
  MUNIT_CHECK_LAUNCH("conv_igemm");
  if (q.ksplit > 1) {
    const long long total = (long long)p.M * p.Cout * phases;
    const int blocks = (int)std::min<long long>((total + 255) / 256, 4096);
    hipLaunchKernelGGL(splitk_epilogue_kernel, dim3(blocks), dim3(256), 0, st, q, phases);
    MUNIT_CHECK_LAUNCH("splitk_epilogue");
  }
  return MUNIT_OK;
}

int check_desc(const munit_conv_desc* d) {
  MUNIT_CHECK_ARG(d != nullptr, "conv: null descriptor");
  MUNIT_CHECK_ARG(d->B > 0 && d->H > 0 && d->W > 0 && d->Cin > 0 && d->Cout > 0, "conv: bad dims");
  MUNIT_CHECK_ARG(d->KH > 0 && d->KW > 0 && d->stride > 0 && d->pad >= 0, "conv: bad kernel geometry");
  MUNIT_CHECK_ARG(d->upsample == 0 || d->upsample == 1, "conv: upsample must be 0 or 1");
  MUNIT_CHECK_ARG(d->compute >= MUNIT_COMPUTE_F32 && d->compute <= MUNIT_COMPUTE_F32X3, "conv: bad compute mode %d", d->compute);
  MUNIT_CHECK_ARG(d->pad_mode == MUNIT_PAD_ZERO || d->pad_mode == MUNIT_PAD_REFLECT, "conv: bad pad mode");
  MUNIT_CHECK_ARG((d->in_dtype == MUNIT_DTYPE_F32 || d->in_dtype == MUNIT_DTYPE_BF16) &&
                  (d->out_dtype == MUNIT_DTYPE_F32 || d->out_dtype == MUNIT_DTYPE_BF16), "conv: bad tensor dtype");
  MUNIT_CHECK_ARG(d->in_dtype == MUNIT_DTYPE_F32 || d->Cin % 64 == 0, "conv: a bf16 input needs Cin %% 64 == 0 (got %d)", d->Cin);
  MUNIT_CHECK_ARG(d->out_dtype == MUNIT_DTYPE_F32 || d->Cout % 64 == 0, "conv: a bf16 output needs Cout %% 64 == 0 (got %d)", d->Cout);
  const int Hu = d->H << d->upsample, Wu = d->W << d->upsample;
  if (d->pad_mode == MUNIT_PAD_REFLECT)
    MUNIT_CHECK_ARG(d->pad < Hu && d->pad < Wu, "conv: reflect pad %d needs input > pad (got %dx%d)", d->pad, Hu, Wu);
  MUNIT_CHECK_ARG(Hu + 2 * d->pad >= d->KH && Wu + 2 * d->pad >= d->KW, "conv: kernel larger than padded input");
  MUNIT_CHECK_ARG((long long)d->B * Hu * Wu < (1ll << 31) / 4, "conv: too many pixels for 32-bit tile indices");
  MUNIT_CHECK_ARG((long long)d->B * (Hu + 2 * d->pad) * (Wu + 2 * d->pad) * std::max(d->Cin, d->Cout) < (1ll << 31),
                  "conv: tensor too large for the 32-bit element offsets of the tile loader");
  return MUNIT_OK;
}

}

extern "C" int munit_conv2d_out_hw(const munit_conv_desc* d, int* Ho, int* Wo) {
  int rc = check_desc(d);
  if (rc) return rc;
  *Ho = ((d->H << d->upsample) + 2 * d->pad - d->KH) / d->stride + 1;
  *Wo = ((d->W << d->upsample) + 2 * d->pad - d->KW) / d->stride + 1;
  return MUNIT_OK;
}

namespace {
bool subpixel_ok(const munit_conv_desc* d) {
  return d->upsample == 1 && d->KH == 5 && d->KW == 5 && d->pad == 2 && d->stride == 1 &&
         d->pad_mode == MUNIT_PAD_REFLECT && d->Cin % 32 == 0 && d->H >= 3 && d->W >= 3 &&
         !MUNIT_ENV_FLAG("MUNIT_DEBUG_NO_SUBPIXEL");
}
}

namespace {
__global__ void pad3to4_image_kernel(const float* __restrict__ x, f32x4* __restrict__ x4, long long npix) {
  for (long long i = (long long)blockIdx.x * blockDim.x + threadIdx.x; i < npix; i += (long long)gridDim.x * blockDim.x)
    x4[i] = f32x4{x[3 * i], x[3 * i + 1], x[3 * i + 2], 0.f};
}
__global__ void pad3to4_weight_kernel(const float* __restrict__ w, float* __restrict__ w4, int N, int taps, int kpad) {
  const long long total = (long long)N * kpad;
  for (long long i = (long long)blockIdx.x * blockDim.x + threadIdx.x; i < total; i += (long long)gridDim.x * blockDim.x) {
    const int n = (int)(i / kpad), k = (int)(i - (long long)n * kpad);
    const int tap = k >> 2, c = k & 3;
    w4[i] = (tap < taps && c < 3) ? w[((long long)n * taps + tap) * 3 + c] : 0.f;
  }
}
struct Cin4Plan {
  int kpad;
  size_t x4_bytes, w4_bytes;
};
Cin4Plan plan_cin4(long long npix, int N, int taps) {
  Cin4Plan c;
  c.kpad = (taps * 4 + BK - 1) / BK * BK;
  c.x4_bytes = align_up((size_t)npix * 4 * sizeof(float), 256);
  c.w4_bytes = align_up((size_t)N * c.kpad * sizeof(float), 256);
  return c;
}
int build_cin4(const Cin4Plan& c, const float* x3, long long npix, const float* w3, int N, int taps, void* ws, hipStream_t st) {
  f32x4* x4 = reinterpret_cast<f32x4*>(ws);
  float* w4 = reinterpret_cast<float*>(reinterpret_cast<char*>(ws) + c.x4_bytes);
  hipLaunchKernelGGL(pad3to4_image_kernel, dim3((unsigned)std::min<long long>((npix + 255) / 256, 8192)), dim3(256), 0, st, x3, x4, npix);
  MUNIT_CHECK_LAUNCH("pad3to4_image");
  hipLaunchKernelGGL(pad3to4_weight_kernel, dim3((unsigned)cdiv((long long)N * c.kpad, 256)), dim3(256), 0, st, w3, w4, N, taps, c.kpad);
  MUNIT_CHECK_LAUNCH("pad3to4_weight");
  return MUNIT_OK;
}
bool cin4_fwd_ok(const munit_conv_desc* d) {
  return d->Cin == 3 && d->in_dtype == MUNIT_DTYPE_F32 && d->upsample == 0 && d->KH * d->KW <= 64 && d->Cout % 4 == 0 &&
         NWAVES == 8 && !MUNIT_ENV_FLAG("MUNIT_DEBUG_NO_CIN4");
}

void set_cin4(IgemmParams* p, const Cin4Plan& c) { p->Ktot = c.kpad; p->w_row = c.kpad; p->cin4 = 1; }

IgemmParams fwd_params(const munit_conv_desc* d, int Ho, int Wo) {
  IgemmParams p{};
  p.B = d->B; p.H = d->H; p.W = d->W; p.Cin = d->Cin;
  p.ups = d->upsample; p.Hu = d->H << p.ups; p.Wu = d->W << p.ups;
  p.Ho = Ho; p.Wo = Wo; p.Cout = d->Cout;
  p.KH = d->KH; p.KW = d->KW; p.stride = d->stride; p.pad = d->pad;
  p.reflect = d->pad_mode == MUNIT_PAD_REFLECT;
  p.Ktot = d->KH * d->KW * d->Cin;
  p.w_row = p.Ktot;
  p.y_sw = d->Cout;
  p.y_sh = (long long)Wo * d->Cout;
  p.y_sb = (long long)Ho * Wo * d->Cout;
  p.M = d->B * Ho * Wo;
  p.act = d->act; p.slope = d->slope;
  p.ct = d->compute;
  p.ps = 1;
  p.bf16s = d->in_dtype == MUNIT_DTYPE_BF16;
  p.out_bf16 = d->out_dtype == MUNIT_DTYPE_BF16;
  return p;
}
IgemmParams subpixel_phase_params(const IgemmParams& p, const munit_conv_desc* d, int Wo) {
  IgemmParams q = p;
  q.ups = 0; q.Hu = d->H; q.Wu = d->W;
  q.Ho = d->H; q.Wo = d->W;
  q.KH = 3; q.KW = 3; q.pad = 1; q.reflect = 0;
  q.Ktot = 9 * d->Cin; q.w_row = q.Ktot;
  q.y_sw = 2 * d->Cout;
  q.y_sh = (long long)2 * Wo * d->Cout;
  q.M = d->B * d->H * d->W;
  q.ps = 2;
  q.w_phase = (long long)d->Cout * q.Ktot;
  q.y_phase_row = (long long)Wo * d->Cout;
  q.y_phase_col = d->Cout;
  return q;
}
void set_subpixel_frame(IgemmParams* p, const munit_conv_desc* d, int Ho, int Wo, int ring) {
  p->frame = ring;
  p->M = d->B * (2 * ring * Wo + 2 * ring * (Ho - 2 * ring));
}

bool wino_geometry_ok(const munit_conv_desc* d) {
  return d->compute == MUNIT_COMPUTE_F32 && d->in_dtype == MUNIT_DTYPE_F32 && d->out_dtype == MUNIT_DTYPE_F32 &&
         d->KH == 3 && d->KW == 3 && d->stride == 1 && d->pad == 1 && d->upsample == 0 && d->act != MUNIT_ACT_TANH;
}
bool wino_fwd_ok(const munit_conv_desc* d) { return wino_geometry_ok(d) && munit_wino_ok(d->B, d->H, d->W, d->Cin, d->Cout); }
long long wino_s2_min_blocks(bool dgrad) {
  static const char* const e = getenv("MUNIT_WINO_S2_MIN_BLOCKS");
  static const long long v = e ? atoll(e) : 0;
  return e ? v : dgrad ? 100 : 192;
}
bool wino_s2_fwd_ok(const munit_conv_desc* d) {
  return d->compute == MUNIT_COMPUTE_F32 && d->in_dtype == MUNIT_DTYPE_F32 && d->out_dtype == MUNIT_DTYPE_F32 && d->KH == 4 &&
         d->KW == 4 && d->stride == 2 && d->pad == 1 && d->upsample == 0 && d->act != MUNIT_ACT_TANH && d->H >= 4 && d->W >= 4 &&
         munit_wino_ok(d->B, d->H, d->W, d->Cin, d->Cout) && !MUNIT_ENV_FLAG("MUNIT_DEBUG_NO_WINOGRAD_S2") &&
         (long long)cdiv((long long)d->B * cdiv(d->H / 2, 3) * cdiv(d->W / 2, 3), 64) * (d->Cout / 64) >= wino_s2_min_blocks(false);
}
bool wino_s2_dgrad_ok(const munit_conv_desc* d) {
  if (!(d->compute == MUNIT_COMPUTE_F32 && d->in_dtype == MUNIT_DTYPE_F32 && d->out_dtype == MUNIT_DTYPE_F32 && d->KH == 4 &&
        d->KW == 4 && d->stride == 2 && d->pad == 1 && d->upsample == 0 && d->H >= 4 && d->W >= 4 && d->H % 2 == 0 && d->W % 2 == 0 &&
        d->Cout % 8 == 0 && d->Cin % 64 == 0 && !MUNIT_ENV_FLAG("MUNIT_DEBUG_NO_WINOGRAD_S2") && !MUNIT_ENV_FLAG("MUNIT_DEBUG_NO_WINOGRAD")))
    return false;
  const int Hd = d->H / 2, Wd = d->W / 2;
  if (d->pad_mode == MUNIT_PAD_REFLECT && (Hd % 3 == 0 || Wd % 3 == 0)) return false;
  if ((long long)d->B * d->H * d->W * std::max(d->Cin, d->Cout) >= (1ll << 29)) return false;
  return (long long)cdiv((long long)d->B * cdiv(Hd + 1, 3) * cdiv(Wd + 1, 3), 64) * (d->Cin / 64) * 4 >= wino_s2_min_blocks(true);
}
bool subpixel_wino_ok(const munit_conv_desc* d) {
  return d->compute == MUNIT_COMPUTE_F32 && d->in_dtype == MUNIT_DTYPE_F32 && d->out_dtype == MUNIT_DTYPE_F32 &&
         d->act != MUNIT_ACT_TANH && munit_wino_ok(d->B, d->H, d->W, d->Cin, d->Cout);
}

enum FwdRoute { FWD_SMALL, FWD_SUBPIXEL_WINO, FWD_SUBPIXEL, FWD_WINO, FWD_WINO_S2, FWD_CIN4, FWD_IGEMM };
struct FwdPlan {
  int rc;
  FwdRoute route;
  int Ho, Wo;
  munit_prep_item prep;
  Cin4Plan cin4;
  int ring;
  size_t img_bytes, ws_bytes;
};
FwdPlan plan_fwd(const munit_conv_desc* d) {
  FwdPlan pl{};
  if ((pl.rc = munit_conv2d_out_hw(d, &pl.Ho, &pl.Wo)) != MUNIT_OK) return pl;
  const int Ho = pl.Ho, Wo = pl.Wo, Ktot = d->KH * d->KW * d->Cin;
  const bool bf16 = d->in_dtype == MUNIT_DTYPE_BF16;
  int kind = bf16 ? MUNIT_PREP_CAST : MUNIT_PREP_NONE;
  if (munit_small_fwd_ok(d)) {
    pl.route = FWD_SMALL; kind = MUNIT_PREP_NONE;
  } else if (subpixel_ok(d)) {
    const bool wino = subpixel_wino_ok(d);
    pl.route = wino ? FWD_SUBPIXEL_WINO : FWD_SUBPIXEL; kind = wino ? MUNIT_PREP_SUBPIXEL_WINOGRAD : MUNIT_PREP_SUBPIXEL;
    pl.ring = wino ? 1 : 2;
  } else if (wino_fwd_ok(d)) {
    pl.route = FWD_WINO; kind = MUNIT_PREP_WINOGRAD;
  } else if (wino_s2_fwd_ok(d)) {
    pl.route = FWD_WINO_S2; kind = MUNIT_PREP_WINOGRAD_S2;
  } else {
    pl.route = cin4_fwd_ok(d) ? FWD_CIN4 : FWD_IGEMM;
  }
  pl.prep = munit_prep_item{nullptr, nullptr, d->Cout, d->KH, d->KW, d->Cin, kind, 1, pl.route != FWD_SMALL && bf16};
  pl.ws_bytes = pl.img_bytes = kind == MUNIT_PREP_NONE ? 0 : align_up((size_t)prep_elems(pl.prep) * (bf16 ? 2 : 4), 256);
  if (pl.route == FWD_SMALL) pl.ws_bytes = munit_small_fwd_workspace(d);
  if (pl.route == FWD_CIN4) pl.cin4 = plan_cin4((long long)d->B * d->H * d->W, d->Cout, d->KH * d->KW), pl.ws_bytes = pl.cin4.x4_bytes + pl.cin4.w4_bytes;
  if (bf16 || munit_small_fwd_supported(d)) return pl;
  if (pl.ring)
    pl.ws_bytes += std::max(splitk_bytes(d->B * (4 * Wo + 4 * (Ho - 4)), d->Cout, Ktot, 1), splitk_bytes(d->B * (2 * Wo + 2 * (Ho - 2)), d->Cout, Ktot, 1));
  if (pl.route == FWD_IGEMM) pl.ws_bytes += splitk_bytes(d->B * Ho * Wo, d->Cout, Ktot, 1);
  return pl;
}

enum WinoForm { WINO_FWD, WINO_FWD_S2, WINO_FWD_SUBPIXEL, WINO_DGRAD, WINO_DGRAD_S2, WINO_DGRAD_UP };
WinoParams wino_params(const munit_conv_desc* d, int Ho, int Wo, WinoForm f, const float* x, const float* u, const float* bias, float* y) {
  const bool fwd = f <= WINO_FWD_SUBPIXEL, refl = d->pad_mode == MUNIT_PAD_REFLECT;
  WinoParams q{};
  q.x = x; q.u = u; q.bias = bias; q.y = y;
  q.B = d->B; q.H = d->H; q.W = d->W;
  q.xc = fwd ? d->Cin : d->Cout; q.N = fwd ? d->Cout : d->Cin; q.K = q.xc;
  const int oh = fwd ? Ho : d->H, ow = fwd ? Wo : d->W;
  q.y_sw = q.N; q.y_sh = (long long)ow * q.N; q.y_sb = (long long)oh * ow * q.N;
  q.mode = refl ? 0 : 1;
  q.th = d->H / 2; q.tw = d->W / 2;
  q.act = fwd ? d->act : MUNIT_ACT_NONE; q.slope = fwd ? d->slope : 0.f;
  switch (f) {
    case WINO_FWD: break;
    case WINO_FWD_S2:
      q.K = 4 * q.xc; q.s2 = 1; q.Ho = Ho; q.Wo = Wo;
      q.th = cdiv(Ho, 3); q.tw = cdiv(Wo, 3);
      break;
    case WINO_FWD_SUBPIXEL:
      q.y_sw *= 2; q.y_sh *= 2; q.y_prow = (long long)Wo * d->Cout; q.y_pcol = d->Cout;
      q.u_phase = wino_image_elems(d->Cin, d->Cout); q.phases = 4;
      q.mode = 1; q.edge = 1;
      break;
    case WINO_DGRAD: q.mode = refl ? 2 : 1; break;
    case WINO_DGRAD_S2:
      q.H = d->H / 2; q.W = d->W / 2; q.s2 = 2; q.Ho = d->H; q.Wo = d->W;
      q.th = cdiv(q.H + 1, 3); q.tw = cdiv(q.W + 1, 3);
      q.u_phase = wino_image_elems(d->Cout, d->Cin); q.phases = 4;
      break;
    case WINO_DGRAD_UP:
      q.H = Ho; q.W = Wo; q.K = 4 * q.xc; q.s2 = 3; q.mode = 1;
      q.th = (d->H - 4) / 2; q.tw = (d->W - 4) / 2;
      break;
  }
  q.cpp = q.xc / 8; q.NB = q.N / 64;
  q.x_bytes = (unsigned)((size_t)d->B * q.H * q.W * q.xc * 4);
  q.bth = cdiv(q.th, 8); q.btw = cdiv(q.tw, 8);
  return q;
}
}

extern "C" size_t munit_conv2d_fwd_workspace_bytes(const munit_conv_desc* d) {
  const FwdPlan pl = plan_fwd(d);
  return pl.rc ? 0 : pl.ws_bytes;
}

extern "C" int munit_conv2d_fwd(const munit_conv_desc* d, const void* x, const float* w,
                                const float* bias, void* y, void* ws, size_t ws_bytes,
                                munit_stream_t stream) {
  return munit_conv2d_fwd_prepared(d, x, w, nullptr, bias, y, ws, ws_bytes, stream);
}

extern "C" int munit_conv2d_fwd_prepared(const munit_conv_desc* d, const void* x, const float* w, const void* wp,
                                         const float* bias, void* y, void* ws, size_t ws_bytes,
                                         munit_stream_t stream) {
  const FwdPlan pl = plan_fwd(d);
  int rc = pl.rc;
  if (rc) return rc;
  const int Ho = pl.Ho, Wo = pl.Wo;
  MUNIT_CHECK_ARG(x && w && y, "conv2d_fwd: null pointer");
  MUNIT_CHECK_ARG(pl.route != FWD_SMALL || d->out_dtype == MUNIT_DTYPE_F32, "conv2d_fwd: the 3-channel image head writes fp32");
  hipStream_t st = (hipStream_t)stream;
  if (pl.ws_bytes != 0 && (ws == nullptr || ws_bytes < pl.ws_bytes)) {
    munit_set_error("conv2d_fwd: workspace %zu < %zu", ws_bytes, pl.ws_bytes);
    return MUNIT_ERR_WORKSPACE;
  }
  if (pl.route == FWD_SMALL) return munit_small_fwd(d, Ho, Wo, x, w, bias, reinterpret_cast<float*>(y), ws, st);
  const float* wimg = w;
  if (pl.prep.kind != MUNIT_PREP_NONE) {
    wimg = reinterpret_cast<const float*>(wp);
    if (wimg == nullptr) {
      munit_prep_item it = pl.prep;
      it.w = w; it.wp = reinterpret_cast<float*>(ws);
      rc = launch_prep_one(it, st);
      if (rc) return rc;
      wimg = it.wp;
    }
  }
  if (pl.route == FWD_WINO || pl.route == FWD_WINO_S2 || pl.route == FWD_SUBPIXEL_WINO) {
    const WinoForm f = pl.route == FWD_WINO ? WINO_FWD : pl.route == FWD_WINO_S2 ? WINO_FWD_S2 : WINO_FWD_SUBPIXEL;
    rc = munit_wino_launch(wino_params(d, Ho, Wo, f, reinterpret_cast<const float*>(x), wimg, bias, reinterpret_cast<float*>(y)), st);
    if (rc || pl.route != FWD_SUBPIXEL_WINO) return rc;
  }
  IgemmParams p = fwd_params(d, Ho, Wo);
  p.x = reinterpret_cast<const float*>(x); p.w = wimg; p.bias = bias; p.y = y;
  if (pl.route == FWD_CIN4) {
    const long long npix = (long long)d->B * d->H * d->W;
    rc = build_cin4(pl.cin4, reinterpret_cast<const float*>(x), npix, w, d->Cout, d->KH * d->KW, ws, st);
    if (rc) return rc;
    p.x = reinterpret_cast<const float*>(ws);
    p.w = reinterpret_cast<const float*>(reinterpret_cast<const char*>(ws) + pl.cin4.x4_bytes);
    set_cin4(&p, pl.cin4);
    return launch_igemm<0>(p, 1, st);
  }
  if (pl.ring) {
    if (pl.route == FWD_SUBPIXEL) rc = launch_igemm<0>(subpixel_phase_params(p, d, Wo), 4, st);
    if (rc) return rc;
    set_subpixel_frame(&p, d, Ho, Wo, pl.ring);
    p.w = pl.prep.bf16 ? reinterpret_cast<const float*>(reinterpret_cast<const bf16_t*>(wimg) + (size_t)4 * 9 * d->Cout * d->Cin) : w;
  }
  return launch_igemm<0>(p, 1, st, ws ? reinterpret_cast<char*>(ws) + pl.img_bytes : nullptr, ws ? ws_bytes - pl.img_bytes : 0);
}

namespace {
__global__ void box2x2_kernel(const f32x4* __restrict__ dy, f32x4* __restrict__ s, int B, int H, int W, int C4) {
  const long long total = (long long)B * H * W * C4;
  for (long long i = (long long)blockIdx.x * blockDim.x + threadIdx.x; i < total; i += (long long)gridDim.x * blockDim.x) {
    const int c = (int)(i % C4);
    long long r = i / C4;
    const int v = (int)(r % W); r /= W;
    const int u = (int)(r % H);
    f32x4 a = dy[i];
    if (v + 1 < W) a += dy[i + C4];
    if (u + 1 < H) {
      a += dy[i + (long long)W * C4];
      if (v + 1 < W) a += dy[i + (long long)W * C4 + C4];
    }
    s[i] = a;
    (void)c;
  }
}

enum DgradRoute {
  DG_WINO_S2,
  DG_WINO,
  DG_SMALL,
  DG_FOLD_UPWINO,
  DG_FOLD_BOXSUM,
  DG_FOLD,
  DG_CIN4,
  DG_DIRECT,
  DG_CORR
};
struct DgradPlan {
  int rc;
  DgradRoute route;
  int Ho, Wo, ps, TH, TW, Hq, Wq;
  bool bf16s;
  bool patch;
  munit_prep_item prep;
  munit_conv_desc t;
  Cin4Plan cin4;
  size_t off_g, off_tail, slab_bytes, ws_bytes;
};
int max_fold_cands(int H, int ups, int P, int reflect) {
  const int Hu = H << ups;
  int worst = 0;
  for (int i = 0; i < H; ++i) {
    int n = 0;
    for (int du = 0; du < (1 << ups); ++du) {
      const int hu = (i << ups) + du;
      ++n;
      if (reflect) {
        if (hu >= 1 && hu <= P) ++n;
        if (hu >= Hu - 1 - P && hu <= Hu - 2) ++n;
      }
    }
    worst = std::max(worst, n);
    if (i == 2 * P + 2 && H > 4 * P + 8) i = H - 2 * P - 4;
  }
  return worst;
}
DgradPlan plan_dgrad(const munit_conv_desc* d) {
  DgradPlan pl{};
  if ((pl.rc = munit_conv2d_out_hw(d, &pl.Ho, &pl.Wo)) != MUNIT_OK) return pl;
  if (d->KH % d->stride != 0 || d->KW % d->stride != 0) {
    munit_set_error("conv2d_dgrad: kernel %dx%d not a multiple of stride %d", d->KH, d->KW, d->stride);
    pl.rc = MUNIT_ERR_ARG;
    return pl;
  }
  pl.ps = d->stride;
  pl.TH = d->KH / d->stride;
  pl.TW = d->KW / d->stride;
  pl.Hq = d->stride * (pl.Ho + pl.TH - 1);
  pl.Wq = d->stride * (pl.Wo + pl.TW - 1);
  const bool direct = d->pad == 0 && d->upsample == 0 && pl.Hq == d->H && pl.Wq == d->W;
  const int reflect = d->pad_mode == MUNIT_PAD_REFLECT;
  munit_conv_desc& t = pl.t;
  t.B = d->B; t.H = pl.Ho; t.W = pl.Wo; t.Cin = d->Cout; t.Cout = d->Cin; t.KH = pl.TH; t.KW = pl.TW;
  t.stride = 1; t.pad = pl.TH - 1; t.pad_mode = MUNIT_PAD_ZERO; t.upsample = 0; t.act = MUNIT_ACT_NONE;
  t.in_dtype = d->out_dtype; t.out_dtype = MUNIT_DTYPE_F32;
  int kind = MUNIT_PREP_DGRAD;
  if (wino_s2_dgrad_ok(d)) {
    pl.route = DG_WINO_S2; kind = MUNIT_PREP_WINOGRAD_S2_DGRAD;
  } else if (wino_geometry_ok(d) && munit_wino_ok(d->B, d->H, d->W, d->Cout, d->Cin)) {
    pl.route = DG_WINO; kind = MUNIT_PREP_WINOGRAD_DGRAD;
  } else if (!direct && pl.ps == 1 && munit_small_fwd_supported(&t) && !MUNIT_ENV_FLAG("MUNIT_DEBUG_NO_SMALL_DGRAD")) {
    pl.route = DG_SMALL;
  } else {
    pl.bf16s = d->out_dtype == MUNIT_DTYPE_BF16;
    const bool foldable = !direct && d->stride == 1 && d->Cout % 32 == 0 && d->KH == d->KW &&
                          (d->H << d->upsample) + 2 * d->pad < 0xFFFF && (d->W << d->upsample) + 2 * d->pad < 0xFFFF &&
                          max_fold_cands(d->H, d->upsample, d->pad, reflect) <= 4 &&
                          max_fold_cands(d->W, d->upsample, d->pad, reflect) <= 4 && !MUNIT_ENV_FLAG("MUNIT_DEBUG_NO_FOLD");
    pl.patch = foldable && d->upsample == 0 && max_fold_cands(d->H, 0, d->pad, reflect) <= 2 &&
               max_fold_cands(d->W, 0, d->pad, reflect) <= 2;
    if (foldable && (!pl.bf16s || pl.patch)) {
      const bool boxsum = !pl.bf16s && d->in_dtype == MUNIT_DTYPE_F32 && d->upsample == 1 && d->KH == 5 && d->pad == 2 && reflect &&
                          d->Cin % 4 == 0 && d->H >= 8 && d->W >= 8 && !MUNIT_ENV_FLAG("MUNIT_DEBUG_NO_BOXSUM");
      const bool upwino = boxsum && d->compute == MUNIT_COMPUTE_F32 && d->H % 2 == 0 && d->W % 2 == 0 && d->Cout % 8 == 0 &&
                          d->Cin % 64 == 0 && (long long)d->B * 4 * d->H * d->W * d->Cout < (1ll << 29) &&
                          !MUNIT_ENV_FLAG("MUNIT_DEBUG_NO_WINOGRAD");
      pl.route = upwino ? DG_FOLD_UPWINO : boxsum ? DG_FOLD_BOXSUM : DG_FOLD;
      if (upwino) kind = MUNIT_PREP_SUBPIXEL_WINOGRAD_DGRAD;
    } else if (!direct && pl.ps == 1 && d->Cout == 3 && d->out_dtype == MUNIT_DTYPE_F32 && pl.TH * pl.TW <= 64 && d->Cin % 4 == 0 &&
               NWAVES == 8 && !MUNIT_ENV_FLAG("MUNIT_DEBUG_NO_CIN4")) {
      pl.route = DG_CIN4;
    } else {
      pl.route = direct ? DG_DIRECT : DG_CORR;
    }
  }
  pl.prep = munit_prep_item{nullptr, nullptr, d->Cout, d->KH, d->KW, d->Cin, kind, pl.ps, pl.bf16s};
  pl.off_g = align_up((size_t)prep_elems(pl.prep) * (pl.bf16s ? 2 : 4), 256);
  size_t g_bytes = align_up((size_t)d->B * pl.Hq * pl.Wq * d->Cin * (d->in_dtype == MUNIT_DTYPE_BF16 ? 2 : 4), 256), tail = 0;
  switch (pl.route) {
    case DG_WINO_S2: case DG_WINO: case DG_FOLD: g_bytes = 256; break;
    case DG_SMALL: tail = munit_small_fwd_workspace(&t); break;
    case DG_FOLD_UPWINO: case DG_FOLD_BOXSUM:
      g_bytes = align_up((size_t)d->B * pl.Ho * pl.Wo * d->Cout * sizeof(float), 256);
      tail = pl.slab_bytes = splitk_bytes(d->B * (4 * d->W + 4 * (d->H - 4)), d->Cin, d->KH * d->KW * d->Cout, 1);
      break;
    case DG_CIN4:
      pl.cin4 = plan_cin4((long long)d->B * pl.Ho * pl.Wo, d->Cin, pl.TH * pl.TW);
      tail = pl.cin4.x4_bytes + pl.cin4.w4_bytes;
      break;
    case DG_DIRECT: case DG_CORR:
      if (!pl.bf16s)
        tail = pl.slab_bytes = splitk_bytes(d->B * (pl.Ho + pl.TH - 1) * (pl.Wo + pl.TW - 1), d->Cin, pl.TH * pl.TW * d->Cout, pl.ps * pl.ps);
      break;
  }
  pl.off_tail = pl.off_g + g_bytes;
  pl.ws_bytes = pl.off_tail + tail;
  return pl;
}

IgemmParams dgrad_fold_params(const munit_conv_desc* d, const DgradPlan& pl) {
  IgemmParams p{};
  p.B = d->B; p.H = pl.Ho; p.W = pl.Wo; p.Cin = d->Cout;
  p.ups = 0; p.Hu = pl.Ho; p.Wu = pl.Wo;
  p.Ho = d->H; p.Wo = d->W; p.Cout = d->Cin;
  p.KH = d->KH; p.KW = d->KW; p.stride = 1; p.pad = d->KH - 1; p.reflect = 0;
  p.Ktot = d->KH * d->KW * d->Cout;
  p.w_row = p.Ktot;
  p.y_sw = d->Cin;
  p.y_sh = (long long)d->W * d->Cin;
  p.y_sb = (long long)d->H * d->W * d->Cin;
  p.M = d->B * d->H * d->W;
  p.act = MUNIT_ACT_NONE; p.slope = 0.f;
  p.ct = d->compute;
  p.ps = 1;
  p.f_pad = d->pad; p.f_ups = d->upsample; p.f_reflect = d->pad_mode == MUNIT_PAD_REFLECT;
  p.f_Hu = d->H << d->upsample; p.f_Wu = d->W << d->upsample;
  p.patch = pl.patch;
  p.bf16s = pl.bf16s; p.out_bf16 = d->in_dtype == MUNIT_DTYPE_BF16;
  return p;
}
bool dgrad_fold_dtypes_ok(const munit_conv_desc* d, const DgradPlan& pl) {
  return d->in_dtype != MUNIT_DTYPE_BF16 || pl.bf16s || pl.patch;
}
IgemmParams boxsum_interior_params(const IgemmParams& p, const munit_conv_desc* d) {
  IgemmParams q = p;
  q.Ho = d->H - 4; q.Wo = d->W - 4;
  q.stride = 2; q.pad = -2;
  q.M = d->B * q.Ho * q.Wo;
  return q;
}
void set_boxsum_frame(IgemmParams* p, const munit_conv_desc* d) {
  p->frame = 2;
  p->M = d->B * (4 * d->W + 4 * (d->H - 4));
}
IgemmParams dgrad_corr_params(const munit_conv_desc* d, const DgradPlan& pl) {
  IgemmParams p{};
  p.B = d->B; p.H = pl.Ho; p.W = pl.Wo; p.Cin = d->Cout;
  p.ups = 0; p.Hu = pl.Ho; p.Wu = pl.Wo;
  p.Ho = pl.Ho + pl.TH - 1; p.Wo = pl.Wo + pl.TW - 1; p.Cout = d->Cin;
  p.KH = pl.TH; p.KW = pl.TW; p.stride = 1; p.pad = pl.TH - 1;
  p.reflect = 0;
  p.Ktot = pl.TH * pl.TW * d->Cout;
  p.w_row = p.Ktot;
  p.y_sw = pl.ps * d->Cin;
  p.y_sh = (long long)pl.ps * pl.Wq * d->Cin;
  p.y_sb = (long long)pl.Hq * pl.Wq * d->Cin;
  p.M = d->B * p.Ho * p.Wo;
  p.act = MUNIT_ACT_NONE; p.slope = 0.f;
  p.ct = d->compute;
  p.ps = pl.ps;
  p.w_phase = (long long)d->Cin * p.Ktot;
  p.y_phase_row = (long long)pl.Wq * d->Cin;
  p.y_phase_col = d->Cin;
  p.bf16s = pl.bf16s; p.out_bf16 = d->in_dtype == MUNIT_DTYPE_BF16;
  return p;
}
bool fold_vectorised(const munit_conv_desc* d) { return d->Cin % 4 == 0; }
}

extern "C" size_t munit_conv2d_dgrad_workspace_bytes(const munit_conv_desc* d) {
  const DgradPlan pl = plan_dgrad(d);
  return pl.rc ? 0 : pl.ws_bytes;
}

extern "C" int munit_conv2d_dgrad(const munit_conv_desc* d, const void* dy, const float* w,
                                  const void* add, void* dx, void* ws, size_t ws_bytes,
                                  munit_stream_t stream) {
  return munit_conv2d_dgrad_prepared(d, dy, w, nullptr, add, dx, ws, ws_bytes, stream);
}

namespace {
template <typename T>
int launch_fold(const munit_conv_desc* d, const DgradPlan& pl, const void* g, const void* add, void* dx, hipStream_t st) {
  const int reflect = d->pad_mode == MUNIT_PAD_REFLECT;
  long long total = (long long)d->B * d->H * d->W * (d->Cin / 4);
  int blocks = (int)std::min<long long>((total + 255) / 256, 8192);
  hipLaunchKernelGGL(fold_kernel<T>, dim3(blocks), dim3(256), 0, st, reinterpret_cast<const T*>(g),
                     reinterpret_cast<const T*>(add), reinterpret_cast<T*>(dx), d->B, d->H, d->W, d->Cin, d->upsample,
                     d->pad, reflect, pl.Hq, pl.Wq);
  MUNIT_CHECK_LAUNCH("fold");
  return MUNIT_OK;
}
int launch_fold_scalar(const munit_conv_desc* d, const DgradPlan& pl, const float* g, const float* add, float* dx, hipStream_t st) {
  const int reflect = d->pad_mode == MUNIT_PAD_REFLECT;
  long long total = (long long)d->B * d->H * d->W * d->Cin;
  int blocks = (int)std::min<long long>((total + 255) / 256, 8192);
  hipLaunchKernelGGL(fold_scalar_kernel, dim3(blocks), dim3(256), 0, st, g, add, dx, d->B, d->H, d->W,
                     d->Cin, d->upsample, d->pad, reflect, pl.Hq, pl.Wq);
  MUNIT_CHECK_LAUNCH("fold");
  return MUNIT_OK;
}
int launch_add_inplace(const munit_conv_desc* d, float* dx, const float* add, hipStream_t st) {
  long long n = (long long)d->B * d->H * d->W * d->Cin;
  int blocks = (int)std::min<long long>((n + 255) / 256, 8192);
  hipLaunchKernelGGL(add_inplace_kernel, dim3(blocks), dim3(256), 0, st, dx, add, n);
  MUNIT_CHECK_LAUNCH("add_inplace");
  return MUNIT_OK;
}
}

extern "C" int munit_conv2d_dgrad_prepared(const munit_conv_desc* d, const void* dy_, const float* w, const void* wp,
                                           const void* add_, void* dx_, void* ws, size_t ws_bytes,
                                           munit_stream_t stream) {
  const DgradPlan pl = plan_dgrad(d);
  int rc = pl.rc;
  if (rc) return rc;
  MUNIT_CHECK_ARG(dy_ && (w || wp) && dx_ && ws, "conv2d_dgrad: null pointer");
  if (ws_bytes < pl.ws_bytes) {
    munit_set_error("conv2d_dgrad: workspace %zu < %zu", ws_bytes, pl.ws_bytes);
    return MUNIT_ERR_WORKSPACE;
  }
  const float* dy = reinterpret_cast<const float*>(dy_);
  const float* add = reinterpret_cast<const float*>(add_);
  float* dx = reinterpret_cast<float*>(dx_);
  const bool dx_bf16 = d->in_dtype == MUNIT_DTYPE_BF16;
  MUNIT_CHECK_ARG(!dx_bf16 || d->Cin % 4 == 0, "conv2d_dgrad: bf16 dx needs Cin %% 4 == 0");
  hipStream_t st = (hipStream_t)stream;
  const float* wt = reinterpret_cast<const float*>(wp);
  float* g = reinterpret_cast<float*>(reinterpret_cast<char*>(ws) + pl.off_g);
  char* tail = reinterpret_cast<char*>(ws) + pl.off_tail;
  if (wt == nullptr) {
    munit_prep_item it = pl.prep;
    it.w = w; it.wp = reinterpret_cast<float*>(ws);
    rc = launch_prep_one(it, st);
    if (rc) return rc;
    wt = it.wp;
  }
  switch (pl.route) {
    case DG_WINO_S2:
      rc = munit_wino_launch(wino_params(d, pl.Ho, pl.Wo, WINO_DGRAD_S2, dy, wt, nullptr, dx), st);
      if (rc || add == nullptr) return rc;
      return launch_add_inplace(d, dx, add, st);
    case DG_WINO: {
      WinoParams q = wino_params(d, pl.Ho, pl.Wo, WINO_DGRAD, dy, wt, nullptr, dx);
      q.add = add;
      return munit_wino_launch(q, st);
    }
    case DG_SMALL:
      MUNIT_CHECK_ARG(!dx_bf16, "conv2d_dgrad: the 3-channel data gradient is fp32");
      rc = munit_small_fwd(&pl.t, pl.Hq, pl.Wq, dy_, wt, nullptr, g, tail, st);
      if (rc) return rc;
      return launch_fold_scalar(d, pl, g, add, dx, st);
    case DG_FOLD_UPWINO: case DG_FOLD_BOXSUM: case DG_FOLD: {
      IgemmParams p = dgrad_fold_params(d, pl);
      p.x = dy; p.w = wt; p.bias = nullptr; p.y = dx;
      MUNIT_CHECK_ARG(dgrad_fold_dtypes_ok(d, pl), "conv2d_dgrad: unsupported dtype combination");
      if (pl.route == DG_FOLD) {
        rc = launch_igemm<2>(p, 1, st);
      } else {
        if (pl.route == DG_FOLD_UPWINO) {
          rc = munit_wino_launch(wino_params(d, pl.Ho, pl.Wo, WINO_DGRAD_UP, dy, wt + (size_t)d->Cout * 25 * d->Cin, nullptr,
                                             dx + ((long long)2 * d->W + 2) * d->Cin), st);
        } else {
          const long long total = (long long)d->B * pl.Ho * pl.Wo * (d->Cout / 4);
          hipLaunchKernelGGL(box2x2_kernel, dim3((unsigned)std::min<long long>((total + 255) / 256, 16384)), dim3(256), 0, st,
                             reinterpret_cast<const f32x4*>(dy), reinterpret_cast<f32x4*>(g), d->B, pl.Ho, pl.Wo, d->Cout / 4);
          MUNIT_CHECK_LAUNCH("box2x2");
          IgemmParams q = boxsum_interior_params(p, d);
          q.x = g;
          q.y = dx + ((long long)2 * d->W + 2) * d->Cin;
          rc = launch_igemm<0>(q, 1, st);
        }
        if (rc) return rc;
        set_boxsum_frame(&p, d);
        rc = launch_igemm<2>(p, 1, st, tail, pl.slab_bytes);
      }
      if (rc || add == nullptr) return rc;
      MUNIT_CHECK_ARG(!dx_bf16, "conv2d_dgrad: `add` with a bf16 dx is not supported on the folded path");
      return launch_add_inplace(d, dx, add, st);
    }
    case DG_CIN4: case DG_DIRECT: case DG_CORR: break;
  }
  MUNIT_CHECK_ARG(pl.TH == pl.TW, "conv2d_dgrad: non-square kernels are not supported");
  const bool direct = pl.route == DG_DIRECT && add == nullptr;
  IgemmParams p = dgrad_corr_params(d, pl);
  p.x = dy; p.w = wt; p.bias = nullptr; p.y = direct ? (void*)dx : (void*)g;
  if (pl.route == DG_CIN4) {
    rc = build_cin4(pl.cin4, dy, (long long)d->B * pl.Ho * pl.Wo, wt, d->Cin, pl.TH * pl.TW, tail, st);
    if (rc) return rc;
    p.x = reinterpret_cast<const float*>(tail);
    p.w = reinterpret_cast<const float*>(tail + pl.cin4.x4_bytes);
    set_cin4(&p, pl.cin4);
    rc = launch_igemm<1>(p, 1, st);
  } else {
    rc = launch_igemm<1>(p, pl.ps * pl.ps, st, tail, pl.slab_bytes);
  }
  if (rc || direct) return rc;
  if (!fold_vectorised(d)) return launch_fold_scalar(d, pl, g, add, dx, st);
  return dx_bf16 ? launch_fold<bf16_t>(d, pl, g, add_, dx_, st) : launch_fold<float>(d, pl, g, add_, dx_, st);
}

extern "C" int munit_conv2d_prep_item(const munit_conv_desc* d, int pass, const float* w, float* wp, munit_prep_item* out) {
  int Ho, Wo;
  int rc = munit_conv2d_out_hw(d, &Ho, &Wo);
  if (rc) return rc;
  MUNIT_CHECK_ARG(out != nullptr, "conv2d_prep_item: null item");
  MUNIT_CHECK_ARG(pass == MUNIT_PASS_FWD || pass == MUNIT_PASS_DGRAD, "conv2d_prep_item: pass must be MUNIT_PASS_FWD or _DGRAD");
  munit_prep_item it;
  if (pass == MUNIT_PASS_FWD) {
    it = plan_fwd(d).prep;
  } else {
    const DgradPlan pl = plan_dgrad(d);
    if (pl.rc) return pl.rc;
    it = pl.prep;
  }
  it.w = w; it.wp = wp;
  *out = it;
  return MUNIT_OK;
}

extern "C" size_t munit_conv2d_prepared_weight_bytes(const munit_conv_desc* d, int pass) {
  munit_prep_item it;
  if (munit_conv2d_prep_item(d, pass, nullptr, nullptr, &it) || it.kind == MUNIT_PREP_NONE) return 0;
  return (size_t)prep_elems(it) * (it.bf16 ? 2 : 4);
}

extern "C" int munit_conv2d_prepare_weights(const munit_prep_item* item, munit_stream_t stream) {
  MUNIT_CHECK_ARG(item && item->w && item->wp, "conv2d_prepare_weights: null pointer");
  const bool wino = item->kind == MUNIT_PREP_WINOGRAD || item->kind == MUNIT_PREP_WINOGRAD_DGRAD;
  const bool spw = item->kind == MUNIT_PREP_SUBPIXEL_WINOGRAD || item->kind == MUNIT_PREP_SUBPIXEL_WINOGRAD_DGRAD;
  const bool ws2 = item->kind == MUNIT_PREP_WINOGRAD_S2 || item->kind == MUNIT_PREP_WINOGRAD_S2_DGRAD;
  MUNIT_CHECK_ARG(!ws2 || (item->KH == 4 && item->KW == 4 && !item->bf16 &&
                           (item->kind == MUNIT_PREP_WINOGRAD_S2 ? item->Cin % 8 == 0 && item->Cout % 64 == 0
                                                                 : item->Cout % 8 == 0 && item->Cin % 64 == 0)),
                  "conv2d_prepare_weights: stride-2 Winograd image needs a 4x4 fp32 filter, K %% 8 == 0, N %% 64 == 0");
  MUNIT_CHECK_ARG(!spw || (item->KH == 5 && item->KW == 5 && !item->bf16 &&
                           (item->kind != MUNIT_PREP_SUBPIXEL_WINOGRAD_DGRAD ? item->Cin % 8 == 0 && item->Cout % 64 == 0
                                                                       : item->Cout % 8 == 0 && item->Cin % 64 == 0)),
                  "conv2d_prepare_weights: sub-pixel Winograd image needs a 5x5 fp32 filter, Cin %% 8 == 0, Cout %% 64 == 0");
  MUNIT_CHECK_ARG(item->kind == MUNIT_PREP_DGRAD || item->kind == MUNIT_PREP_SUBPIXEL || wino || spw || ws2 || (item->kind == MUNIT_PREP_CAST && item->bf16),
                  "conv2d_prepare_weights: bad kind %d", item->kind);
  MUNIT_CHECK_ARG(!wino || (item->KH == 3 && item->KW == 3 && !item->bf16 &&
                            (item->kind != MUNIT_PREP_WINOGRAD_DGRAD ? item->Cin % 8 == 0 && item->Cout % 64 == 0
                                                               : item->Cout % 8 == 0 && item->Cin % 64 == 0)),
                  "conv2d_prepare_weights: Winograd image needs a 3x3 fp32 filter, K %% 8 == 0, N %% 64 == 0");
  MUNIT_CHECK_ARG(item->ps >= 1 && item->KH % item->ps == 0 && item->KW % item->ps == 0, "conv2d_prepare_weights: bad phase count");
  MUNIT_CHECK_ARG(item->kind != MUNIT_PREP_SUBPIXEL || (item->KH == 5 && item->KW == 5), "conv2d_prepare_weights: sub-pixel needs 5x5");
  return launch_prep_one(*item, (hipStream_t)stream);
}

extern "C" int munit_conv2d_prepare_weights_batch(const munit_prep_item* items_dev, int n, munit_stream_t stream) {
  MUNIT_CHECK_ARG(items_dev != nullptr && n > 0 && n <= 65535, "conv2d_prepare_weights_batch: bad table (n=%d)", n);
  hipLaunchKernelGGL(prep_weights_kernel<true>, dim3(64, (unsigned)n), dim3(256), 0, (hipStream_t)stream, items_dev, PrepItem{});
  MUNIT_CHECK_LAUNCH("prep_weights_batch");
  return MUNIT_OK;
}

namespace {
const char* igemm_refusal(IgemmForm f) {
  switch (f) {
    case IG_REFUSED_BF16_CIN: return "refused: bf16 storage needs a multiple of 64 input channels";
    case IG_REFUSED_CIN4_FOLD: return "refused: 4-channel taps are not a folded backward-data form";
    case IG_REFUSED_BF16_FOLD: return "refused: bf16-storage folded backward-data exists for the LDS-patch form only";
    case IG_REFUSED_FOLD_UNALIGNED: return "refused: folded backward-data needs Cout % 32 == 0";
    default: return nullptr;
  }
}
}

const char* munit_igemm_kernel_name(const munit_conv_desc* d, int pass) {
  const bool refl = d->pad_mode == MUNIT_PAD_REFLECT;
  const bool x_bf16 = d->in_dtype == MUNIT_DTYPE_BF16, y_bf16 = d->out_dtype == MUNIT_DTYPE_BF16;
  static const char* const head[2][3][2] = {
      {{"conv_head_pk_kernel", "conv_head_pk_kernel<bf16_t>"}, {"conv_head_mfma_kernel", "conv_head_mfma_kernel<bf16_t>"},
       {"conv_patch_fwd_kernel", "conv_patch_fwd_kernel<bf16_t>"}},
      {{"conv_head_pk_kernel (padded-domain correlation)", "conv_head_pk_kernel<bf16_t> (padded-domain correlation)"},
       {"conv_head_mfma_kernel (padded-domain correlation)", "conv_head_mfma_kernel<bf16_t> (padded-domain correlation)"},
       {"conv_patch_fwd_kernel (padded-domain correlation)", "conv_patch_fwd_kernel<bf16_t> (padded-domain correlation)"}}};
  if (pass == MUNIT_PASS_FWD) {
    const FwdPlan fp = plan_fwd(d);
    if (fp.rc) return "invalid";
    const int Ho = fp.Ho, Wo = fp.Wo;
    IgemmParams p = fwd_params(d, Ho, Wo);
    const int bn = igemm_bn(p);
    switch (fp.route) {
      case FWD_SMALL: return y_bf16 ? "refused: the 3-channel image head writes fp32" : head[0][munit_small_fwd_kernel(d->Cin)][x_bf16];
      case FWD_SUBPIXEL_WINO: return "conv_wino_kernel<1, 0> x4 sub-pixel phases + conv_igemm_kernel frame";
      case FWD_SUBPIXEL: {
        const IgemmForm ph = igemm_form(subpixel_phase_params(p, d, Wo), 0);
        set_subpixel_frame(&p, d, Ho, Wo, fp.ring);
        const IgemmForm fr = igemm_form(p, 0);
        if (igemm_refusal(ph)) return igemm_refusal(ph);
        if (igemm_refusal(fr)) return igemm_refusal(fr);
        if (ph != fr) return "invalid";
        if (ph == IG_BF16S) return bn == 64 ? "conv_igemm_kernel<64, true, 0, 4> x4 sub-pixel phases + frame"
                                            : "conv_igemm_kernel<128, true, 0, 4> x4 sub-pixel phases + frame";
        if (ph == IG_CT1) return "conv_igemm_kernel<.., 0, 1> x4 sub-pixel phases + frame";
        if (ph == IG_CT2) return "conv_igemm_kernel<.., 0, 2> x4 sub-pixel phases + frame";
        return "conv_igemm_kernel x4 sub-pixel phases + frame";
      }
      case FWD_WINO: return refl ? "conv_wino_kernel<0, 0>" : "conv_wino_kernel<1, 0>";
      case FWD_WINO_S2: return refl ? "conv_wino_kernel<0, 1>" : "conv_wino_kernel<1, 1>";
      case FWD_CIN4: set_cin4(&p, fp.cin4); break;
      case FWD_IGEMM: break;
    }
    const IgemmForm f = igemm_form(p, 0);
    if (igemm_refusal(f)) return igemm_refusal(f);
    if (fp.route == FWD_CIN4) return y_bf16 ? "conv_igemm_kernel<.., 5> (3 input channels as 4-channel taps, bf16 y)"
                                            : "conv_igemm_kernel<.., 5> (3 input channels as 4-channel taps)";
    if (f == IG_BF16S) return bn == 64 ? "conv_igemm_kernel<64, true, 0, 4>" : "conv_igemm_kernel<128, true, 0, 4>";
    if (f == IG_CT1) return "conv_igemm_kernel<.., 0, 1>";
    if (f == IG_CT2) return "conv_igemm_kernel<.., 0, 2>";
    return "conv_igemm_kernel<fwd>";
  }
  const DgradPlan pl = plan_dgrad(d);
  if (pl.rc) return "invalid";
  if (x_bf16 && d->Cin % 4 != 0) return "refused: bf16 dx needs Cin % 4 == 0";
  switch (pl.route) {
    case DG_WINO_S2: return refl ? "conv_wino_kernel<0, 2>" : "conv_wino_kernel<1, 2>";
    case DG_WINO: return refl ? "conv_wino_kernel<2, 0>" : "conv_wino_kernel<1, 0>";
    case DG_SMALL: return x_bf16 ? "refused: the 3-channel data gradient is fp32" : head[1][munit_small_fwd_kernel(d->Cout)][y_bf16];
    case DG_FOLD_UPWINO: case DG_FOLD_BOXSUM: case DG_FOLD: {
      if (!dgrad_fold_dtypes_ok(d, pl)) return "refused: unsupported dtype combination";
      IgemmParams p = dgrad_fold_params(d, pl);
      const int bn = igemm_bn(p);
      if (pl.route == DG_FOLD_UPWINO) return "conv_wino_kernel<1, 3> + conv_igemm_kernel frame";
      if (pl.route == DG_FOLD_BOXSUM) {
        const IgemmForm in = igemm_form(boxsum_interior_params(p, d), 0);
        set_boxsum_frame(&p, d);
        const IgemmForm fr = igemm_form(p, 2);
        if (igemm_refusal(in)) return igemm_refusal(in);
        if (igemm_refusal(fr)) return igemm_refusal(fr);
        if (in == IG_CT1 && fr == IG_CT1) return "box2x2_kernel + conv_igemm_kernel<.., 1> (box-sum backward-data)";
        if (in == IG_CT2 && fr == IG_CT2) return "box2x2_kernel + conv_igemm_kernel<.., 2> (box-sum backward-data)";
        return "box2x2_kernel + conv_igemm_kernel (box-sum backward-data)";
      }
      const IgemmForm f = igemm_form(p, 2);
      if (igemm_refusal(f)) return igemm_refusal(f);
      if (f == IG_BF16S) return bn == 64 ? "conv_igemm_kernel<64, true, 2, 4> (LDS-patch fold)" : "conv_igemm_kernel<128, true, 2, 4> (LDS-patch fold)";
      if (f == IG_PATCH) return "conv_igemm_kernel<.., 2, 3> (LDS-patch fold)";
      if (f == IG_CT1) return "conv_igemm_kernel<.., 2, 1> (folded gather)";
      if (f == IG_CT2) return "conv_igemm_kernel<.., 2, 2> (folded gather)";
      return "conv_igemm_kernel<.., 2, 0> (folded gather)";
    }
    case DG_CIN4: case DG_DIRECT: case DG_CORR: break;
  }
  if (pl.TH != pl.TW) return "refused: non-square kernels are not supported";
  IgemmParams p = dgrad_corr_params(d, pl);
  const int bn = igemm_bn(p);
  if (pl.route == DG_CIN4) set_cin4(&p, pl.cin4);
  const IgemmForm f = igemm_form(p, 1);
  if (igemm_refusal(f)) return igemm_refusal(f);
  if (pl.route == DG_CIN4) return x_bf16 ? "conv_igemm_kernel<.., 1, 5> (3 output channels as 4-channel taps) + fold_kernel<bf16_t>"
                                         : "conv_igemm_kernel<.., 1, 5> (3 output channels as 4-channel taps)";
  if (pl.route == DG_DIRECT) {
    if (f == IG_BF16S) return bn == 64 ? "conv_igemm_kernel<64, true, 1, 4> direct" : "conv_igemm_kernel<128, true, 1, 4> direct";
    if (f == IG_CT1) return "conv_igemm_kernel<.., 1, 1> direct";
    if (f == IG_CT2) return "conv_igemm_kernel<.., 1, 2> direct";
    return "conv_igemm_kernel<dgrad direct>";
  }
  const bool fold16 = x_bf16 && fold_vectorised(d);
  if (f == IG_BF16S) {
    if (fold16) return bn == 64 ? "conv_igemm_kernel<64, true, 1, 4> phases + fold_kernel<bf16_t>" : "conv_igemm_kernel<128, true, 1, 4> phases + fold_kernel<bf16_t>";
    return bn == 64 ? "conv_igemm_kernel<64, true, 1, 4> phases + fold_kernel" : "conv_igemm_kernel<128, true, 1, 4> phases + fold_kernel";
  }
  if (f == IG_CT1) return fold16 ? "conv_igemm_kernel<.., 1, 1> phases + fold_kernel<bf16_t>" : "conv_igemm_kernel<.., 1, 1> phases + fold_kernel";
  if (f == IG_CT2) return fold16 ? "conv_igemm_kernel<.., 1, 2> phases + fold_kernel<bf16_t>" : "conv_igemm_kernel<.., 1, 2> phases + fold_kernel";
  return fold16 ? "conv_igemm_kernel<.., 1, .> phases + fold_kernel<bf16_t>" : "conv_igemm_kernel<.., 1, .> phases + fold_kernel";
}

double munit_igemm_executed_flops(const munit_conv_desc* d, int pass) {
  int Ho, Wo;
  if (munit_conv2d_out_hw(d, &Ho, &Wo)) return 0.0;
  const double cc = 2.0 * d->Cin * d->Cout;
  if (pass == MUNIT_PASS_FWD) {
    const FwdPlan fp = plan_fwd(d);
    switch (fp.route) {
      case FWD_SUBPIXEL_WINO: return cc * d->B * ((double)(d->H / 2) * (d->W / 2) * 4 * 16 + (2.0 * Wo + 2.0 * (Ho - 2)) * 25);
      case FWD_SUBPIXEL: return cc * d->B * ((double)d->H * d->W * 4 * 9 + (4.0 * Wo + 4.0 * (Ho - 4)) * 25);
      case FWD_WINO: return cc * d->B * (d->H / 2) * (d->W / 2) * 16;
      case FWD_WINO_S2: return 4 * cc * d->B * cdiv(Ho, 3) * cdiv(Wo, 3) * 16;
      case FWD_CIN4: return 2.0 * d->Cout * d->B * Ho * Wo * fp.cin4.kpad;
      default: return cc * d->B * Ho * Wo * d->KH * d->KW;
    }
  }
  const DgradPlan pl = plan_dgrad(d);
  if (pl.rc) return 0.0;
  switch (pl.route) {
    case DG_WINO_S2: return 4 * cc * d->B * cdiv(d->H / 2 + 1, 3) * cdiv(d->W / 2 + 1, 3) * 16;
    case DG_WINO: return cc * d->B * (d->H / 2) * (d->W / 2) * 16;
    case DG_FOLD_UPWINO: return cc * d->B * ((double)((d->H - 4) / 2) * ((d->W - 4) / 2) * 4 * 16 + (4.0 * d->W + 4.0 * (d->H - 4)) * 25);
    case DG_FOLD_BOXSUM: return cc * d->B * ((double)(d->H - 4) * (d->W - 4) + 4.0 * d->W + 4.0 * (d->H - 4)) * d->KH * d->KW;
    case DG_FOLD: return cc * d->B * d->H * d->W * d->KH * d->KW;
    case DG_DIRECT: return cc * d->B * Ho * Wo * d->KH * d->KW;
    case DG_CIN4: return 2.0 * d->Cin * d->B * (double)(pl.Ho + pl.TH - 1) * (pl.Wo + pl.TW - 1) * pl.cin4.kpad;
    case DG_SMALL: case DG_CORR: return cc * d->B * (double)(pl.Ho + pl.TH - 1) * (pl.Wo + pl.TW - 1) * pl.TH * pl.TW * pl.ps * pl.ps;
  }
  return 0.0;
}

namespace {
munit_conv_desc linear_desc(int B, int K, int N, int act, float slope, int compute) {
  munit_conv_desc d{};
  d.B = B; d.H = 1; d.W = 1; d.Cin = K; d.Cout = N; d.KH = 1; d.KW = 1; d.stride = 1; d.pad = 0;
  d.pad_mode = MUNIT_PAD_ZERO; d.upsample = 0; d.act = act; d.slope = slope; d.compute = compute;
  return d;
}
}
// ... 31 lines not shown
```

### munit_amd/csrc/conv_small.hip

```cpp
#include "common.h"

namespace {

struct SmallParams {
  const void* x;
  const float* w;
  const float* bias;
  const float* dy;
  float* y;
  float* slab;
  int B, H, W, Cin, Ho, Wo;
  int pad, reflect, act;
  float slope;
  int tiles_x, tiles_y;
  int rows_per_unit, units_per_img;
};

__device__ inline int map_coord(int v, int n, int reflect) {
  if (v < 0) return reflect ? -v : -1;
  if (v >= n) return reflect ? 2 * n - 2 - v : -1;
  return v;
}

template <int CO, int K, typename XT>
// ... 32 lines not shown
#pragma unroll 1
      for (int c4 = 0; c4 < 4; ++c4) {
#pragma unroll
        for (int kw = 0; kw < K; ++kw) {
          const f32x4 xv = patch[c4 * PLANE + (ty + kh) * PW + tx + kw];
#pragma unroll
          for (int c = 0; c < CO; ++c) {
            const f32x4 wv = *reinterpret_cast<const f32x4*>(wg + ((long long)(c * K + kh) * K + kw) * p.Cin + ch0 + c4 * 4);
            acc[c] = fmaf(wv[0], xv[0], acc[c]);
            acc[c] = fmaf(wv[1], xv[1], acc[c]);
            acc[c] = fmaf(wv[2], xv[2], acc[c]);
            acc[c] = fmaf(wv[3], xv[3], acc[c]);
          }
        }
      }
    }
  }
  const int oh = oh0 + ty, ow = ow0 + tx;
  if (oh < p.Ho && ow < p.Wo) {
    float* yo = p.y + (((long long)b * p.Ho + oh) * p.Wo + ow) * CO;
#pragma unroll
    for (int c = 0; c < CO; ++c) {
      float v = acc[c] + (p.bias != nullptr ? p.bias[c] : 0.f);
      yo[c] = apply_act(v, p.act, p.slope);
    }
  }
}

__device__ const float munit_head_zero16[4] = {0.f, 0.f, 0.f, 0.f};

template <typename XT>
__global__ __launch_bounds__(256, 2) void conv_head_mfma_kernel(SmallParams p) {
  constexpr int K = 7, CO = 3, TW = 16, TH = 8, PW = TW + K - 1, PH = TH + K - 1, PS = 64;
  constexpr int NG_W = 2 * (TW / 4);
  constexpr int NPIX = PH * PW;
  static_assert(NPIX % 4 == 0, "patch fills go four pixels at a time");
  __shared__ __attribute__((aligned(16))) float patch[NPIX * PS];
  const int tid = threadIdx.x, lane = tid & 63;
  const int ty = __builtin_amdgcn_readfirstlane(tid >> 6);
  const int blk = lane >> 2, j = lane & 3;
  int bid = blockIdx.x;
  const int tile_x = bid % p.tiles_x; bid /= p.tiles_x;
  const int tile_y = bid % p.tiles_y;
  const int b = bid / p.tiles_y;
  const int ow0 = tile_x * TW, oh0 = tile_y * TH;
  const XT* xb = reinterpret_cast<const XT*>(p.x) + (long long)b * p.H * p.W * p.Cin;
  const float* __restrict__ wg = p.w;

  f32x4 acc[NG_W];
#pragma unroll
  for (int g = 0; g < NG_W; ++g) acc[g] = f32x4{0.f, 0.f, 0.f, 0.f};
  const int wi = j < CO ? j : 0;
  const float wmask = j < CO ? 1.f : 0.f;

  for (int ch0 = 0; ch0 < p.Cin; ch0 += 64) {
    __syncthreads();
    {
      const int wv = __builtin_amdgcn_readfirstlane(tid >> 6);
      const int sub = lane >> 4, c4 = (lane & 15) ^ (4 * sub);
      constexpr int NG = NPIX / 4, PER = (NG + 3) / 4;
      if constexpr (sizeof(XT) == 4) {
#pragma unroll
        for (int it = 0; it < PER; ++it) {
          const int grp = wv + 4 * it;
          if (grp < NG) {
            const int pix = 4 * grp + sub;
            const int pr = pix / PW, pc = pix - pr * PW;
            const int ih = map_coord(oh0 + pr - p.pad, p.H, p.reflect);
            const int iw = map_coord(ow0 + pc - p.pad, p.W, p.reflect);
            const void* g = (ih >= 0 && iw >= 0) ? (const void*)(xb + ((long long)ih * p.W + iw) * p.Cin + ch0 + c4 * 4)
                                                 : (const void*)munit_head_zero16;
            __builtin_amdgcn_global_load_lds((const __attribute__((address_space(1))) void*)g,
                                             (__attribute__((address_space(3))) void*)(patch + grp * 4 * PS), 16, 0, 0);
          }
        }
        asm volatile("s_waitcnt vmcnt(0)" ::: "memory");
      } else {
        f32x4 stage[PER];
#pragma unroll
        for (int it = 0; it < PER; ++it) {
          const int grp = wv + 4 * it;
          f32x4 v = {0.f, 0.f, 0.f, 0.f};
          if (grp < NG) {
            const int pix = 4 * grp + sub;
            const int pr = pix / PW, pc = pix - pr * PW;
            const int ih = map_coord(oh0 + pr - p.pad, p.H, p.reflect);
            const int iw = map_coord(ow0 + pc - p.pad, p.W, p.reflect);
            if (ih >= 0 && iw >= 0) v = ld4(xb + ((long long)ih * p.W + iw) * p.Cin + ch0 + c4 * 4);
          }
          stage[it] = v;
        }
#pragma unroll
        for (int it = 0; it < PER; ++it) {
          const int grp = wv + 4 * it;
          if (grp < NG) *reinterpret_cast<f32x4*>(&patch[grp * 4 * PS + lane * 4]) = stage[it];
        }
      }
    }
    __syncthreads();
    const float* wl = wg + (long long)wi * K * K * p.Cin + ch0 + 4 * blk;
    f32x4 wrow[K], wnext[K];
#pragma unroll
    for (int kw = 0; kw < K; ++kw) wrow[kw] = *reinterpret_cast<const f32x4*>(wl + (long long)kw * p.Cin) * wmask;
#pragma unroll 1
    for (int kh = 0; kh < K; ++kh) {
      const int khn = kh + 1 < K ? kh + 1 : kh;
#pragma unroll
      for (int kw = 0; kw < K; ++kw)
        wnext[kw] = *reinterpret_cast<const f32x4*>(wl + (long long)(khn * K + kw) * p.Cin) * wmask;
#pragma unroll
      for (int kw = 0; kw < K; ++kw) {
        f32x4 xf[NG_W];
#pragma unroll
        for (int g = 0; g < NG_W; ++g) {
          const int q = (ty + 4 * (g >> 2) + kh) * PW + 4 * (g & 3) + j + kw;
          xf[g] = *reinterpret_cast<const f32x4*>(&patch[q * PS + 4 * (blk ^ (4 * (q & 3)))]);
        }
#pragma unroll
        for (int t = 0; t < 4; ++t)
#pragma unroll
          for (int g = 0; g < NG_W; ++g)
            acc[g] = __builtin_amdgcn_mfma_f32_4x4x1f32(wrow[kw][t], xf[g][t], acc[g], 0, 0, 0);
      }
#pragma unroll
      for (int kw = 0; kw < K; ++kw) wrow[kw] = wnext[kw];
    }
  }
#pragma unroll
  for (int g = 0; g < NG_W; ++g) {
    const int oh = oh0 + ty + 4 * (g >> 2);
    float v[CO];
#pragma unroll
    for (int c = 0; c < CO; ++c) {
      float s = acc[g][c];
      s += __shfl_xor(s, 4, 64);
      s += __shfl_xor(s, 8, 64);
      s += __shfl_xor(s, 16, 64);
      s += __shfl_xor(s, 32, 64);
      v[c] = s;
    }
    const int ow = ow0 + 4 * (g & 3) + j;
    if (blk == 0 && oh < p.Ho && ow < p.Wo) {
      float* yo = p.y + (((long long)b * p.Ho + oh) * p.Wo + ow) * CO;
#pragma unroll
      for (int c = 0; c < CO; ++c) yo[c] = apply_act(v[c] + (p.bias != nullptr ? p.bias[c] : 0.f), p.act, p.slope);
    }
  }
}

constexpr int HP_TW = 32, HP_TH = 16, HP_K = 7, HP_PW = HP_TW + HP_K - 1, HP_PH = HP_TH + HP_K - 1, HP_CP = 8;
constexpr int HP_IDX = 20;
constexpr int HP_ROW = (HP_CP / 4) * 2 * HP_IDX * 4;
constexpr int HP_ITEMS = HP_PH * (HP_CP / 4) * 2 * HP_IDX;

__global__ void head_pk_weights_kernel(const float* __restrict__ w, float* __restrict__ wp, int Cin) {
  const int total = (Cin / HP_CP) * HP_K * 2 * HP_K * 12;
  for (int i = blockIdx.x * blockDim.x + threadIdx.x; i < total; i += gridDim.x * blockDim.x) {
    int r = i;
    const int e = r % 12; r /= 12;
    const int kw = r % HP_K; r /= HP_K;
    const int quad = r & 1; r >>= 1;
    const int kh = r % HP_K;
    const int pass = r / HP_K;
    const int co = e < 8 ? (e & 1) : 2, c = e < 8 ? (e >> 1) : e - 8;
    wp[i] = w[((long long)(co * HP_K + kh) * HP_K + kw) * Cin + pass * HP_CP + quad * 4 + c];
  }
}

template <typename XT>
__global__ __launch_bounds__(256, 4) void conv_head_pk_kernel(SmallParams p, const float* __restrict__ wp) {
  __shared__ __attribute__((aligned(16))) float patch[HP_PH * HP_ROW];
  const int tid = threadIdx.x, lane = tid & 63;
  const int wv = __builtin_amdgcn_readfirstlane(tid >> 6);
  const int j = lane & 15, lr = 4 * wv + (lane >> 4);
  int bid = blockIdx.x;
  const int tile_x = bid % p.tiles_x; bid /= p.tiles_x;
  const int tile_y = bid % p.tiles_y;
  const int b = bid / p.tiles_y;
  const int ow0 = tile_x * HP_TW, oh0 = tile_y * HP_TH;
  const XT* xb = reinterpret_cast<const XT*>(p.x) + (long long)b * p.H * p.W * p.Cin;

  constexpr int PER = (HP_ITEMS + 255) / 256;
  int foff[PER];
#pragma unroll
  for (int it = 0; it < PER; ++it) {
    const int n = (wv + 4 * it) * 64 + lane;
    int r = n;
    const int idx = r % HP_IDX; r /= HP_IDX;
    const int par = r & 1; r >>= 1;
    const int quad = r & 1;
    const int row = r >> 1;
    const int pc = 2 * idx + par;
    const int ih = map_coord(oh0 + row - p.pad, p.H, p.reflect);
    const int iw = map_coord(ow0 + pc - p.pad, p.W, p.reflect);
    foff[it] = (n < HP_ITEMS && pc < HP_PW && ih >= 0 && iw >= 0) ? (ih * p.W + iw) * p.Cin + quad * 4 : -1;
  }

  typedef float f32x2 __attribute__((ext_vector_type(2)));
  f32x2 a01 = {0.f, 0.f}, b01 = {0.f, 0.f};
  f32x2 a2 = {0.f, 0.f}, b2 = {0.f, 0.f};
  const float* rd = patch + lr * HP_ROW + j * 4;
  const int npass = p.Cin / HP_CP;
  for (int pass = 0; pass < npass; ++pass) {
    __syncthreads();
    if constexpr (sizeof(XT) == 4) {
#pragma unroll
      for (int it = 0; it < PER; ++it) {
        const int n0 = (wv + 4 * it) * 64;
        if (n0 < HP_ITEMS) {
          const void* g = foff[it] >= 0 ? (const void*)(xb + foff[it] + pass * HP_CP) : (const void*)munit_head_zero16;
          if (n0 + 64 <= HP_ITEMS || n0 + lane < HP_ITEMS)
            __builtin_amdgcn_global_load_lds((const __attribute__((address_space(1))) void*)g,
                                             (__attribute__((address_space(3))) void*)(patch + n0 * 4), 16, 0, 0);
        }
      }
      asm volatile("s_waitcnt vmcnt(0)" ::: "memory");
    } else {
      f32x4 stage[PER];
#pragma unroll
      for (int it = 0; it < PER; ++it) {
        f32x4 v = {0.f, 0.f, 0.f, 0.f};
        if (foff[it] >= 0) v = ld4(xb + foff[it] + pass * HP_CP);
        stage[it] = v;
      }
#pragma unroll
      for (int it = 0; it < PER; ++it) {
        const int n = (wv + 4 * it) * 64 + lane;
        if (n < HP_ITEMS) *reinterpret_cast<f32x4*>(&patch[n * 4]) = stage[it];
      }
    }
    __syncthreads();
#pragma unroll 1
    for (int kh = 0; kh < HP_K; ++kh) {
#pragma unroll
      for (int quad = 0; quad < 2; ++quad) {
        f32x4 xs[8];
#pragma unroll
        for (int i = 0; i < 8; ++i)
          xs[i] = *reinterpret_cast<const f32x4*>(rd + kh * HP_ROW + ((quad * 2 + (i & 1)) * HP_IDX + (i >> 1)) * 4);
        const float* wq = wp + (((pass * HP_K + kh) * 2 + quad) * HP_K) * 12;
#pragma unroll
        for (int kw = 0; kw < HP_K; ++kw) {
          const f32x4 xa = xs[kw], xb2 = xs[kw + 1];
#pragma unroll
          for (int c = 0; c < 4; ++c) {
            const f32x2 w01 = {wq[kw * 12 + 2 * c], wq[kw * 12 + 2 * c + 1]};
            a01 = __builtin_elementwise_fma(f32x2{xa[c], xa[c]}, w01, a01);
            b01 = __builtin_elementwise_fma(f32x2{xb2[c], xb2[c]}, w01, b01);
          }
#pragma unroll
          for (int h = 0; h < 2; ++h) {
            const f32x2 w2 = {wq[kw * 12 + 8 + 2 * h], wq[kw * 12 + 9 + 2 * h]};
            a2 = __builtin_elementwise_fma(f32x2{xa[2 * h], xa[2 * h + 1]}, w2, a2);
            b2 = __builtin_elementwise_fma(f32x2{xb2[2 * h], xb2[2 * h + 1]}, w2, b2);
          }
        }
      }
    }
  }
  const int oh = oh0 + lr, ow = ow0 + 2 * j;
  if (oh < p.Ho) {
    const float bias0 = p.bias != nullptr ? p.bias[0] : 0.f, bias1 = p.bias != nullptr ? p.bias[1] : 0.f,
                bias2 = p.bias != nullptr ? p.bias[2] : 0.f;
    float* yo = p.y + (((long long)b * p.Ho + oh) * p.Wo + ow) * 3;
    if (ow < p.Wo) {
      yo[0] = apply_act(a01[0] + bias0, p.act, p.slope);
      yo[1] = apply_act(a01[1] + bias1, p.act, p.slope);
      yo[2] = apply_act((a2[0] + a2[1]) + bias2, p.act, p.slope);
    }
    if (ow + 1 < p.Wo) {
      yo[3] = apply_act(b01[0] + bias0, p.act, p.slope);
      yo[4] = apply_act(b01[1] + bias1, p.act, p.slope);
      yo[5] = apply_act((b2[0] + b2[1]) + bias2, p.act, p.slope);
    }
  }
}

template <int CO, int K, typename XT>
__global__ __launch_bounds__(256) void conv_lanes_wgrad_kernel(SmallParams p) {
  const int lane = threadIdx.x & 63;
  const int wv = __builtin_amdgcn_readfirstlane(threadIdx.x >> 6);
  const int G = p.Cin >> 6;
  const long long unit = (long long)blockIdx.x * 4 + wv;
  const long long per_band = (long long)K * G;
  const long long nunits = (long long)p.B * p.units_per_img * per_band;
  if (unit >= nunits) return;
  const int g = (int)(unit % G);
  const int kh = (int)((unit / G) % K);
  const long long band = unit / per_band;
  const int bi = (int)(band % p.units_per_img);
  const int b = (int)(band / p.units_per_img);
  const int ci = g * 64 + lane;

  float acc[CO][K];
#pragma unroll
  for (int c = 0; c < CO; ++c)
#pragma unroll
    for (int kw = 0; kw < K; ++kw) acc[c][kw] = 0.f;
  float bsum[CO];
#pragma unroll
  for (int c = 0; c < CO; ++c) bsum[c] = 0.f;

  constexpr int CH = (64 / K) * K;
  const int oh_begin = bi * p.rows_per_unit, oh_end = min(p.Ho, oh_begin + p.rows_per_unit);
  for (int oh = oh_begin; oh < oh_end; ++oh) {
    const int ih = map_coord(oh - p.pad + kh, p.H, p.reflect);
    const bool rowok = ih >= 0;
    const XT* rowp = reinterpret_cast<const XT*>(p.x) + ((long long)b * p.H + (rowok ? ih : 0)) * p.W * p.Cin + ci;
    const float* dyrow = p.dy + ((long long)b * p.Ho + oh) * p.Wo * CO;
    float win[K];
#pragma unroll
    for (int j = 0; j < K - 1; ++j) {
      const int iw = map_coord(j - p.pad, p.W, p.reflect);
      win[j] = (rowok && iw >= 0) ? ld1(rowp + (long long)iw * p.Cin) : 0.f;
    }
    for (int ow0 = 0; ow0 < p.Wo; ow0 += CH) {
      const int n = min(CH, p.Wo - ow0);
      float dyv[CO];
#pragma unroll
      for (int c = 0; c < CO; ++c) dyv[c] = (lane < n) ? dyrow[(long long)(ow0 + lane) * CO + c] : 0.f;
// ... 12 lines not shown
            for (int kw = 0; kw < K; ++kw) acc[c][kw] = fmaf(d, win[(kw + s) % K], acc[c][kw]);
          }
        }
      }
    }
  }
  const long long n_w = (long long)CO * K * K * p.Cin;
  float* out = p.slab + band * (n_w + CO);
#pragma unroll
  for (int c = 0; c < CO; ++c)
#pragma unroll
    for (int kw = 0; kw < K; ++kw) out[((long long)(c * K + kh) * K + kw) * p.Cin + ci] = acc[c][kw];
  if (g == 0 && kh == 0 && lane < CO) {
    float v = 0.f;
#pragma unroll
    for (int c = 0; c < CO; ++c) v = (lane == c) ? bsum[c] : v;
    out[n_w + lane] = v;
  }
}

__global__ void small_slab_reduce_kernel(const float* __restrict__ slab, float* __restrict__ dw,
                                         float* __restrict__ db, long long n_w, int co, long long rows,
                                         float beta) {
  const long long stride = n_w + co;
  for (long long i = (long long)blockIdx.x * blockDim.x + threadIdx.x; i < stride;
       i += (long long)gridDim.x * blockDim.x) {
    float s0 = 0.f, s1 = 0.f, s2 = 0.f, s3 = 0.f;
    long long r = 0;
    for (; r + 3 < rows; r += 4) {
      s0 += slab[r * stride + i];
      s1 += slab[(r + 1) * stride + i];
      s2 += slab[(r + 2) * stride + i];
      s3 += slab[(r + 3) * stride + i];
    }
    for (; r < rows; ++r) s0 += slab[r * stride + i];
    const float s = (s0 + s1) + (s2 + s3);
    if (i < n_w) dw[i] = (beta != 0.f ? beta * dw[i] : 0.f) + s;
    else if (db != nullptr) db[i - n_w] = (beta != 0.f ? beta * db[i - n_w] : 0.f) + s;
  }
}

}

namespace {
template <int CO, int K, typename XT>
__global__ __launch_bounds__(256) void conv_lanes_wgrad_pk_kernel(SmallParams p) {
  typedef float f32x2 __attribute__((ext_vector_type(2)));
  const int lane = threadIdx.x & 63;
  const int wv = __builtin_amdgcn_readfirstlane(threadIdx.x >> 6);
  const int G = p.Cin >> 6;
  const long long unit = (long long)blockIdx.x * 4 + wv;
  const long long per_band = (long long)K * G;
  const long long nunits = (long long)p.B * p.units_per_img * per_band;
  if (unit >= nunits) return;
  const int g = (int)(unit % G);
  const int kh = (int)((unit / G) % K);
  const long long band = unit / per_band;
  const int bi = (int)(band % p.units_per_img);
  const int b = (int)(band / p.units_per_img);
  const int rh = lane >> 5, cp = lane & 31;
  const int ci = g * 64 + 2 * cp;
  const bool want_b = g == 0 && kh == 0;

  f32x2 acc[CO][K];
#pragma unroll
  for (int c = 0; c < CO; ++c)
#pragma unroll
    for (int kw = 0; kw < K; ++kw) acc[c][kw] = f32x2{0.f, 0.f};
  float bsum[CO];
#pragma unroll
  for (int c = 0; c < CO; ++c) bsum[c] = 0.f;

  auto ldx = [&](const XT* q) -> f32x2 {
    if constexpr (sizeof(XT) == 4) return *reinterpret_cast<const f32x2*>(q);
    else { const bf16_t* h = reinterpret_cast<const bf16_t*>(q); return f32x2{(float)h[0], (float)h[1]}; }
  };
  constexpr int CH = (32 / K) * K;
  const int oh_begin = bi * p.rows_per_unit, oh_end = min(p.Ho, oh_begin + p.rows_per_unit);
  for (int oh2 = oh_begin; oh2 < oh_end; oh2 += 2) {
    const int oh = oh2 + rh;
    const bool live = oh < oh_end;
    const int ih = map_coord(min(oh, p.Ho - 1) - p.pad + kh, p.H, p.reflect);
    const bool rowok = live && ih >= 0;
    const XT* rowp = reinterpret_cast<const XT*>(p.x) + ((long long)b * p.H + (rowok ? ih : 0)) * p.W * p.Cin + ci;
    const float* dyrow = p.dy + ((long long)b * p.Ho + min(oh, p.Ho - 1)) * p.Wo * CO;
    f32x2 win[K];
#pragma unroll
    for (int j = 0; j < K - 1; ++j) {
      const int iw = map_coord(j - p.pad, p.W, p.reflect);
      win[j] = (rowok && iw >= 0) ? ldx(rowp + (long long)iw * p.Cin) : f32x2{0.f, 0.f};
    }
    for (int ow0 = 0; ow0 < p.Wo; ow0 += CH) {
      const int n = min(CH, p.Wo - ow0);
      float dyv[CO];
#pragma unroll
      for (int c = 0; c < CO; ++c) dyv[c] = (live && cp < n) ? dyrow[(long long)(ow0 + cp) * CO + c] : 0.f;
#pragma unroll 1
      for (int i0 = 0; i0 < n; i0 += K) {
#pragma unroll
        for (int s = 0; s < K; ++s) {
          const int i = i0 + s;
          const int iw = map_coord(min(ow0 + i, p.Wo - 1) + (K - 1) - p.pad, p.W, p.reflect);
          win[(K - 1 + s) % K] = (rowok && iw >= 0) ? ldx(rowp + (long long)iw * p.Cin) : f32x2{0.f, 0.f};
          const int src = ((lane & 32) + min(i, 31)) << 2;
#pragma unroll
          for (int c = 0; c < CO; ++c) {
            const float d = __builtin_bit_cast(float, __builtin_amdgcn_ds_bpermute(src, __builtin_bit_cast(int, dyv[c])));
            if (want_b) bsum[c] += d;
            const f32x2 dd = {d, d};
#pragma unroll
            for (int kw = 0; kw < K; ++kw) acc[c][kw] = __builtin_elementwise_fma(dd, win[(kw + s) % K], acc[c][kw]);
          }
        }
      }
    }
  }
  const long long n_w = (long long)CO * K * K * p.Cin;
  float* out = p.slab + band * (n_w + CO);
#pragma unroll
  for (int c = 0; c < CO; ++c)
#pragma unroll
    for (int kw = 0; kw < K; ++kw) {
      f32x2 v = acc[c][kw];
      v[0] += __shfl_xor(v[0], 32, 64);
      v[1] += __shfl_xor(v[1], 32, 64);
      if (rh == 0) *reinterpret_cast<f32x2*>(out + ((long long)(c * K + kh) * K + kw) * p.Cin + ci) = v;
    }
  if (want_b) {
    float v = 0.f;
#pragma unroll
    for (int c = 0; c < CO; ++c) {
      const float t = bsum[c] + __shfl_xor(bsum[c], 32, 64);
      v = (lane == c) ? t : v;
    }
    if (lane < CO) out[n_w + lane] = v;
  }
}
}

bool munit_small_fwd_supported(const munit_conv_desc* d) {
  return d->Cout == 3 && d->KH == 7 && d->KW == 7 && d->stride == 1 && d->upsample == 0 && d->Cin % 16 == 0;
}
bool munit_small_fwd_ok(const munit_conv_desc* d) { return munit_small_fwd_supported(d) && !MUNIT_ENV_FLAG("MUNIT_DEBUG_NO_SMALL_FWD"); }
bool munit_small_wgrad_ok(const munit_conv_desc* d) {
  return munit_small_fwd_supported(d) && d->Cin % 64 == 0 && !MUNIT_ENV_FLAG("MUNIT_DEBUG_NO_SMALL_WGRAD");
}

SmallFwdKernel munit_small_fwd_kernel(int Cin) {
  if (!MUNIT_ENV_FLAG("MUNIT_DEBUG_NO_HEAD_PK")) return SMALL_FWD_PK;
  return Cin % 64 == 0 && !MUNIT_ENV_FLAG("MUNIT_DEBUG_NO_HEAD_MFMA") ? SMALL_FWD_MFMA : SMALL_FWD_PATCH;
}
bool munit_small_wgrad_pk() { return !MUNIT_ENV_FLAG("MUNIT_DEBUG_NO_WGRAD_PK"); }

size_t munit_small_fwd_workspace(const munit_conv_desc* d) {
  if (munit_small_fwd_kernel(d->Cin) != SMALL_FWD_PK) return 0;
  return align_up((size_t)(d->Cin / HP_CP) * HP_K * 2 * HP_K * 12 * sizeof(float), 256);
}

int munit_small_fwd(const munit_conv_desc* d, int Ho, int Wo, const void* x, const float* w, const float* bias,
                    float* y, void* ws, hipStream_t st) {
  SmallParams p{};
  p.x = x; p.w = w; p.bias = bias; p.y = y;
  p.B = d->B; p.H = d->H; p.W = d->W; p.Cin = d->Cin; p.Ho = Ho; p.Wo = Wo;
  p.pad = d->pad; p.reflect = d->pad_mode == MUNIT_PAD_REFLECT; p.act = d->act; p.slope = d->slope;
  const SmallFwdKernel k = munit_small_fwd_kernel(d->Cin);
  const bool b16 = d->in_dtype == MUNIT_DTYPE_BF16;
  p.tiles_x = cdiv(Wo, k == SMALL_FWD_PK ? HP_TW : k == SMALL_FWD_MFMA ? 16 : 64);
  p.tiles_y = cdiv(Ho, k == SMALL_FWD_PK ? HP_TH : k == SMALL_FWD_MFMA ? 8 : 4);
  const dim3 grid((unsigned)((long long)d->B * p.tiles_x * p.tiles_y));
  if (k == SMALL_FWD_PK) {
    MUNIT_CHECK_ARG(ws != nullptr, "conv_head_pk: null workspace");
    float* wp = reinterpret_cast<float*>(ws);
    const int total = (d->Cin / HP_CP) * HP_K * 2 * HP_K * 12;
    hipLaunchKernelGGL(head_pk_weights_kernel, dim3(cdiv(total, 256)), dim3(256), 0, st, w, wp, d->Cin);
    MUNIT_CHECK_LAUNCH("head_pk_weights");
    if (b16) hipLaunchKernelGGL((conv_head_pk_kernel<bf16_t>), grid, dim3(256), 0, st, p, wp);
    else hipLaunchKernelGGL((conv_head_pk_kernel<float>), grid, dim3(256), 0, st, p, wp);
  } else if (k == SMALL_FWD_MFMA) {
    if (b16) hipLaunchKernelGGL((conv_head_mfma_kernel<bf16_t>), grid, dim3(256), 0, st, p);
    else hipLaunchKernelGGL((conv_head_mfma_kernel<float>), grid, dim3(256), 0, st, p);
  } else {
    if (b16) hipLaunchKernelGGL((conv_patch_fwd_kernel<3, 7, bf16_t>), grid, dim3(256), 0, st, p);
    else hipLaunchKernelGGL((conv_patch_fwd_kernel<3, 7, float>), grid, dim3(256), 0, st, p);
  }
  MUNIT_CHECK_LAUNCH(k == SMALL_FWD_PK ? "conv_head_pk" : k == SMALL_FWD_MFMA ? "conv_head_mfma" : "conv_patch_fwd");
  return MUNIT_OK;
}

namespace {
constexpr int WG_ROWS = 4;
}

size_t munit_small_wgrad_workspace(const munit_conv_desc* d, int Ho) {
  const long long bands = (long long)d->B * cdiv(Ho, WG_ROWS);
  return align_up((size_t)bands * ((size_t)3 * 49 * d->Cin + 3) * sizeof(float), 256);
}

int munit_small_wgrad(const munit_conv_desc* d, int Ho, int Wo, const void* x, const float* dy, float* dw,
                      float* db, float beta, void* ws, hipStream_t st) {
  SmallParams p{};
  p.x = x; p.dy = dy; p.slab = reinterpret_cast<float*>(ws);
  p.B = d->B; p.H = d->H; p.W = d->W; p.Cin = d->Cin; p.Ho = Ho; p.Wo = Wo;
  p.pad = d->pad; p.reflect = d->pad_mode == MUNIT_PAD_REFLECT;
  p.rows_per_unit = WG_ROWS; p.units_per_img = cdiv(Ho, WG_ROWS);
  const int G = d->Cin / 64;
  const long long bands = (long long)d->B * p.units_per_img;
  const long long units = bands * 7 * G;
  if (munit_small_wgrad_pk()) {
    if (d->in_dtype == MUNIT_DTYPE_BF16) hipLaunchKernelGGL((conv_lanes_wgrad_pk_kernel<3, 7, bf16_t>), dim3((unsigned)cdiv(units, 4)), dim3(256), 0, st, p);
    else hipLaunchKernelGGL((conv_lanes_wgrad_pk_kernel<3, 7, float>), dim3((unsigned)cdiv(units, 4)), dim3(256), 0, st, p);
  } else {
    if (d->in_dtype == MUNIT_DTYPE_BF16) hipLaunchKernelGGL((conv_lanes_wgrad_kernel<3, 7, bf16_t>), dim3((unsigned)cdiv(units, 4)), dim3(256), 0, st, p);
    else hipLaunchKernelGGL((conv_lanes_wgrad_kernel<3, 7, float>), dim3((unsigned)cdiv(units, 4)), dim3(256), 0, st, p);
  }
  MUNIT_CHECK_LAUNCH("conv_lanes_wgrad");
  const long long n_w = (long long)3 * 49 * d->Cin;
  const int blocks = cdiv(n_w + 3, 256);
  hipLaunchKernelGGL(small_slab_reduce_kernel, dim3(blocks), dim3(256), 0, st, p.slab, dw, db, n_w, 3, bands, beta);
  MUNIT_CHECK_LAUNCH("small_slab_reduce");
  return MUNIT_OK;
}
```

### munit_amd/csrc/runtime.hip

```cpp
#include "common.h"
#include <cstring>

namespace {
thread_local char g_err[512] = "";
}

void munit_set_error(const char* fmt, ...) {
  va_list ap;
  va_start(ap, fmt);
  vsnprintf(g_err, sizeof(g_err), fmt, ap);
  va_end(ap);
}

extern "C" const char* munit_last_error(void) { return g_err; }
extern "C" int munit_version(void) { return 5; }

extern "C" int munit_stream_wait_stream(munit_stream_t waiter, munit_stream_t signaler) {
  constexpr int MAX_DEV = 16;
  static thread_local hipEvent_t ev[MAX_DEV] = {};
  int dev = 0;
  if (hipGetDevice(&dev) != hipSuccess || dev < 0 || dev >= MAX_DEV) {
    munit_set_error("stream_wait_stream: no current device");
    return MUNIT_ERR_ARG;
  }
  if (ev[dev] == nullptr && hipEventCreateWithFlags(&ev[dev], hipEventDisableTiming) != hipSuccess) {
    munit_set_error("stream_wait_stream: hipEventCreate failed");
    return MUNIT_ERR_LAUNCH;
  }
  hipEvent_t use = ev[dev];
  hipError_t e = hipEventRecord(use, (hipStream_t)signaler);
  if (e == hipSuccess) e = hipStreamWaitEvent((hipStream_t)waiter, use, 0);
  if (e != hipSuccess) {
    munit_set_error("stream_wait_stream: %s", hipGetErrorString(e));
    return MUNIT_ERR_LAUNCH;
  }
  return MUNIT_OK;
}
```

Before: 79.90 images/s.

## Fuse split-K reduction into igemm kernel via last-block counters; prebuild head weights

Adds an in-launch split-K path: each K-slice block writes its partial tile to the slab, bumps a per-tile atomic counter, and the last-arriving block sums all slices and applies bias and activation. This removes the separate split-K epilogue launch and its extra pass over the slab for small tiles. Separately, the 3-channel padded and packed 7x7 head weight images move into the shared weight-prep path, so they are no longer rebuilt on every forward call. The cost is cross-block atomics, fences and reliance on a per-stream counter region allocated on first use.

```diff
diff --git a/include/munit_hip.h b/include/munit_hip.h
--- a/include/munit_hip.h
+++ b/include/munit_hip.h
@@ -57,7 +57,8 @@
 enum { MUNIT_PREP_NONE = 0, MUNIT_PREP_DGRAD = 1, MUNIT_PREP_SUBPIXEL = 2, MUNIT_PREP_CAST = 3,
        MUNIT_PREP_WINOGRAD = 4, MUNIT_PREP_WINOGRAD_DGRAD = 5, MUNIT_PREP_SUBPIXEL_WINOGRAD = 6,
        MUNIT_PREP_WINOGRAD_S2 = 7, MUNIT_PREP_WINOGRAD_S2_DGRAD = 8,
-       MUNIT_PREP_SUBPIXEL_WINOGRAD_DGRAD = 9  };
+       MUNIT_PREP_SUBPIXEL_WINOGRAD_DGRAD = 9,
+       MUNIT_PREP_CIN4 = 10, MUNIT_PREP_CIN4_DGRAD = 11, MUNIT_PREP_HEAD_PK = 12, MUNIT_PREP_HEAD_PK_DGRAD = 13 };
 typedef struct {
   const float* w;
   float* wp;
@@ -83,6 +84,9 @@
 
 double munit_conv2d_executed_flops(const munit_conv_desc* d, int pass);
 const char* munit_conv2d_kernel_name(const munit_conv_desc* d, int pass);
+int munit_igemm_splitk_route(int M, int Cout, int Ktot, int phases);
+int munit_conv2d_splitk_shape(const munit_conv_desc* d, int pass, int shape[4]);
+int munit_debug_splitk_counters_busy(void);
 
 int munit_act_bwd(int act, float slope, const float* y, const float* dy, float* dx, size_t n,
                   munit_stream_t stream);
diff --git a/munit_amd/_lib.py b/munit_amd/_lib.py
--- a/munit_amd/_lib.py
+++ b/munit_amd/_lib.py
@@ -72,6 +72,9 @@
     "munit_conv2d_dgrad_prepared": (c_int, [_DESC, _P, _P, _P, _P, _P, _P, c_size_t, _P]),
     "munit_conv2d_executed_flops": (c_double, [_DESC, c_int]),
     "munit_conv2d_kernel_name": (c_char_p, [_DESC, c_int]),
+    "munit_igemm_splitk_route": (c_int, [c_int, c_int, c_int, c_int]),
+    "munit_conv2d_splitk_shape": (c_int, [_DESC, c_int, POINTER(c_int * 4)]),
+    "munit_debug_splitk_counters_busy": (c_int, []),
     "munit_linear_workspace_bytes": (c_size_t, [c_int, c_int, c_int]),
     "munit_linear_fwd": (c_int, [_P, _P, _P, _P, c_int, c_int, c_int, c_int, c_float, _P, c_size_t, _P]),
     "munit_linear_bwd": (c_int, [_P, _P, _P, _P, _P, _P, c_int, c_int, c_int, c_float, _P, c_size_t, _P]),
diff --git a/munit_amd/csrc/common.h b/munit_amd/csrc/common.h
--- a/munit_amd/csrc/common.h
+++ b/munit_amd/csrc/common.h
@@ -71,6 +71,9 @@
   return r < 0 ? -1 : (r >> ups);
 }
 
+constexpr int MUNIT_SPLITK_COUNTERS = 256;
+unsigned* munit_splitk_counters(hipStream_t st);
+
 double munit_igemm_executed_flops(const munit_conv_desc* d, int pass);
 const char* munit_igemm_kernel_name(const munit_conv_desc* d, int pass);
 
@@ -80,9 +83,19 @@
 enum SmallFwdKernel { SMALL_FWD_PK, SMALL_FWD_MFMA, SMALL_FWD_PATCH };
 SmallFwdKernel munit_small_fwd_kernel(int Cin);
 bool munit_small_wgrad_pk();
-size_t munit_small_fwd_workspace(const munit_conv_desc* d);
+__host__ __device__ inline long long munit_head_pk_elems(int C) { return (long long)(C / 8) * 7 * 2 * 7 * 12; }
+__host__ __device__ inline void munit_head_pk_source(int i, int& co, int& kh, int& kw, int& ch) {
+  int r = i;
+  const int e = r % 12; r /= 12;
+  kw = r % 7; r /= 7;
+  const int quad = r & 1; r >>= 1;
+  kh = r % 7;
+  const int pass = r / 7;
+  co = e < 8 ? (e & 1) : 2;
+  ch = pass * 8 + quad * 4 + (e < 8 ? (e >> 1) : e - 8);
+}
 int munit_small_fwd(const munit_conv_desc* d, int Ho, int Wo, const void* x, const float* w, const float* bias,
-                    float* y, void* ws, hipStream_t st);
+                    float* y, hipStream_t st);
 size_t munit_small_wgrad_workspace(const munit_conv_desc* d, int Ho);
 int munit_small_wgrad(const munit_conv_desc* d, int Ho, int Wo, const void* x, const float* dy, float* dw,
                       float* db, float beta, void* ws, hipStream_t st);
diff --git a/munit_amd/csrc/conv_igemm.hip b/munit_amd/csrc/conv_igemm.hip
--- a/munit_amd/csrc/conv_igemm.hip
+++ b/munit_amd/csrc/conv_igemm.hip
@@ -30,6 +30,7 @@
   int frame;
   int ksplit, kt_per_split;
   float* slab;
+  unsigned* cnt;
   int ct;
   int patch;
   int out_bf16;
@@ -111,7 +112,7 @@
 
 __device__ const float munit_zero_page[32] = {0.f};
 
-template <int BN, bool ALIGNED, int ROLE, int CT = 0>
+template <int BN, bool ALIGNED, int ROLE, int CT = 0, bool INL = false>
 __global__ __launch_bounds__(NTHR, NWAVES == 8 ? ((CT == 3 && BN == 64) ? 6 : 4) : 2) void conv_igemm_kernel(IgemmParams p) {
   constexpr bool BF16 = CT == 1 || CT == 2;
   constexpr bool DMA = CT == 3 || CT == 4 || CT == 5;
@@ -623,29 +624,15 @@
   const int n = n0 + cq * 4;
   const bool split = p.ksplit > 1;
   float* const sl = split ? p.slab + ((long long)blockIdx.y * p.ksplit + blockIdx.z) * (long long)p.M * p.Cout : nullptr;
-  const bool vec = (p.Cout & 3) == 0 && (split || ((p.y_sw & 3) == 0 && (p.y_sh & 3) == 0 && (p.y_sb & 3) == 0));
+  const bool vec_y = (p.Cout & 3) == 0 && (p.y_sw & 3) == 0 && (p.y_sh & 3) == 0 && (p.y_sb & 3) == 0;
+  const bool vec = split ? (p.Cout & 3) == 0 : vec_y;
   f32x4 bv = {0.f, 0.f, 0.f, 0.f};
-  if (!split && p.bias != nullptr) {
+  if ((!split || INL) && p.bias != nullptr) {
 #pragma unroll
     for (int e = 0; e < 4; ++e)
       if (n + e < p.Cout) bv[e] = p.bias[n + e];
   }
-#pragma unroll 2
-  for (int row = cr0; row < BM; row += CRPT) {
-    const int m = m0 + row;
-    if (m >= p.M || n >= p.Cout) continue;
-    f32x4 v = *reinterpret_cast<const f32x4*>(&Cs[row * CLD + cq * 4]);
-    if (split) {
-      float* dst = sl + (long long)m * p.Cout + n;
-      if (vec) {
-        *reinterpret_cast<f32x4*>(dst) = v;
-      } else {
-#pragma unroll
-        for (int e = 0; e < 4; ++e)
-          if (n + e < p.Cout) dst[e] = v[e];
-      }
-      continue;
-    }
+  auto store_y = [&](int m, f32x4 v) {
     int b, oh, ow;
     decode_pixel(m, p.Ho, p.Wo, p.frame, b, oh, ow);
     const long long off = y_base + (long long)b * p.y_sb + (long long)oh * p.y_sh + (long long)ow * p.y_sw + n;
@@ -653,7 +640,7 @@
     for (int e = 0; e < 4; ++e) v[e] = apply_act(v[e] + bv[e], p.act, p.slope);
     if (p.out_bf16) {
       bf16_t* dst = reinterpret_cast<bf16_t*>(p.y) + off;
-      if (vec) {
+      if (vec_y) {
         st4(dst, v);
       } else {
 #pragma unroll
@@ -662,13 +649,90 @@
       }
     } else {
       float* dst = reinterpret_cast<float*>(p.y) + off;
-      if (vec) {
+      if (vec_y) {
         *reinterpret_cast<f32x4*>(dst) = v;
       } else {
 #pragma unroll
         for (int e = 0; e < 4; ++e)
           if (n + e < p.Cout) dst[e] = v[e];
       }
+    }
+  };
+  if constexpr (!INL) {
+#pragma unroll 2
+    for (int row = cr0; row < BM; row += CRPT) {
+      const int m = m0 + row;
+      if (m >= p.M || n >= p.Cout) continue;
+      const f32x4 v = *reinterpret_cast<const f32x4*>(&Cs[row * CLD + cq * 4]);
+      if (split) {
+        float* dst = sl + (long long)m * p.Cout + n;
+        if (vec) {
+          *reinterpret_cast<f32x4*>(dst) = v;
+        } else {
+#pragma unroll
+          for (int e = 0; e < 4; ++e)
+            if (n + e < p.Cout) dst[e] = v[e];
+        }
+        continue;
+      }
+      store_y(m, v);
+    }
+  } else {
+    for (int row = cr0; row < BM; row += CRPT) {
+      const int m = m0 + row;
+      if (m >= p.M || n >= p.Cout) continue;
+      const f32x4 v = *reinterpret_cast<const f32x4*>(&Cs[row * CLD + cq * 4]);
+      float* dst = sl + (long long)m * p.Cout + n;
+      if (vec) {
+        asm volatile("global_store_dwordx4 %0, %1, off sc1\n\ts_nop 1" ::"v"(dst), "v"(v) : "memory");
+      } else {
+#pragma unroll
+        for (int e = 0; e < 4; ++e)
+          if (n + e < p.Cout) __hip_atomic_store(dst + e, v[e], __ATOMIC_RELAXED, __HIP_MEMORY_SCOPE_AGENT);
+      }
+    }
+    asm volatile("s_waitcnt vmcnt(0)" ::: "memory");
+    __syncthreads();
+    int* const last_flag = reinterpret_cast<int*>(smem);
+    if (tid == 0) {
+      unsigned* const c = p.cnt + blockIdx.y * gridDim.x + blockIdx.x;
+      const bool last = __hip_atomic_fetch_add(c, 1u, __ATOMIC_RELAXED, __HIP_MEMORY_SCOPE_AGENT) == (unsigned)p.ksplit - 1u;
+      if (last) {
+        __hip_atomic_store(c, 0u, __ATOMIC_RELAXED, __HIP_MEMORY_SCOPE_AGENT);
+        __builtin_amdgcn_fence(__ATOMIC_ACQUIRE, "agent");
+        asm volatile("s_waitcnt vmcnt(0)" ::: "memory");
+      }
+      *last_flag = last;
+    }
+    __syncthreads();
+    if (!*last_flag) return;
+    constexpr int RPT = BM / CRPT;
+    const long long per = (long long)p.M * p.Cout;
+    const float* const sl0 = p.slab + (long long)blockIdx.y * p.ksplit * per + n;
+    f32x4 s[RPT];
+#pragma unroll
+    for (int i = 0; i < RPT; ++i) s[i] = f32x4{0.f, 0.f, 0.f, 0.f};
+#pragma unroll 2
+    for (int k = 0; k < p.ksplit; ++k) {
+      const float* const slk = sl0 + k * per;
+#pragma unroll
+      for (int i = 0; i < RPT; ++i) {
+        const int m = m0 + cr0 + i * CRPT;
+        if (m >= p.M || n >= p.Cout) continue;
+        const float* src = slk + (long long)m * p.Cout;
+        if (vec) {
+          s[i] += *reinterpret_cast<const f32x4*>(src);
+        } else {
+#pragma unroll
+          for (int e = 0; e < 4; ++e)
+            if (n + e < p.Cout) s[i][e] += src[e];
+        }
+      }
+    }
+#pragma unroll
+    for (int i = 0; i < RPT; ++i) {
+      const int m = m0 + cr0 + i * CRPT;
+      if (m < p.M && n < p.Cout) store_y(m, s[i]);
     }
   }
 }
@@ -738,6 +802,29 @@
   else it.wp[i] = s;
 }
 
+__host__ __device__ inline int cin4_kpad(int taps) { return (taps * 4 + BK - 1) / BK * BK; }
+__device__ inline void prep_cin4_elem(const PrepItem& it, long long i) {
+  const int taps = it.KH * it.KW, kpad = cin4_kpad(taps);
+  const int n = (int)(i / kpad), k = (int)(i - (long long)n * kpad);
+  const int tap = k >> 2, c = k & 3;
+  float v = 0.f;
+  if (tap < taps && c < 3) {
+    if (it.kind == MUNIT_PREP_CIN4) {
+      v = it.w[((long long)n * taps + tap) * 3 + c];
+    } else {
+      const int t = tap / it.KW, r = tap - t * it.KW;
+      v = it.w[(((long long)c * it.KH + it.KH - 1 - t) * it.KW + it.KW - 1 - r) * it.Cin + n];
+    }
+  }
+  it.wp[i] = v;
+}
+__device__ inline void prep_head_pk_elem(const PrepItem& it, long long i) {
+  int o, kh, kw, ch;
+  munit_head_pk_source((int)i, o, kh, kw, ch);
+  it.wp[i] = it.kind == MUNIT_PREP_HEAD_PK ? it.w[((long long)(o * 7 + kh) * 7 + kw) * it.Cin + ch]
+                                           : it.w[((long long)(ch * 7 + 6 - kh) * 7 + 6 - kw) * 3 + o];
+}
+
 __host__ __device__ inline long long prep_elems(const PrepItem& it) {
   const long long cc = (long long)it.Cout * it.Cin;
   if (it.kind == MUNIT_PREP_SUBPIXEL) return it.bf16 ? (4 * 9 + 25) * cc : 4 * 9 * cc;
@@ -745,6 +832,10 @@
   if (it.kind == MUNIT_PREP_SUBPIXEL_WINOGRAD_DGRAD) return cc * it.KH * it.KW + 4 * wino_image_elems(it.Cin, it.Cout);
   if (it.kind == MUNIT_PREP_SUBPIXEL_WINOGRAD || it.kind == MUNIT_PREP_WINOGRAD_S2 || it.kind == MUNIT_PREP_WINOGRAD_S2_DGRAD)
     return 4 * wino_image_elems(it.Cin, it.Cout);
+  if (it.kind == MUNIT_PREP_CIN4 || it.kind == MUNIT_PREP_CIN4_DGRAD)
+    return (long long)(it.kind == MUNIT_PREP_CIN4 ? it.Cout : it.Cin) * cin4_kpad(it.KH * it.KW);
+  if (it.kind == MUNIT_PREP_HEAD_PK || it.kind == MUNIT_PREP_HEAD_PK_DGRAD)
+    return munit_head_pk_elems(it.kind == MUNIT_PREP_HEAD_PK ? it.Cin : it.Cout);
   return cc * it.KH * it.KW;
 }
 
@@ -771,6 +862,8 @@
       else wino_subpixel_dgrad_weight_item(it.w, it.wp + nd, it.Cout, it.Cin, i - nd);
     }
     else if (it.kind == MUNIT_PREP_CAST) prep_cast_elem(it, i);
+    else if (it.kind == MUNIT_PREP_CIN4 || it.kind == MUNIT_PREP_CIN4_DGRAD) prep_cin4_elem(it, i);
+    else if (it.kind == MUNIT_PREP_HEAD_PK || it.kind == MUNIT_PREP_HEAD_PK_DGRAD) prep_head_pk_elem(it, i);
     else prep_dgrad_elem(it, i);
   }
 }
@@ -781,6 +874,11 @@
   hipLaunchKernelGGL(prep_weights_kernel<false>, dim3(blocks), dim3(256), 0, st, nullptr, it);
   MUNIT_CHECK_LAUNCH("prep_weights");
   return MUNIT_OK;
+}
+int rebuild_image(const PrepItem& it, const char* who, hipStream_t st) {
+  if (MUNIT_ENV_FLAG("MUNIT_DEBUG_PREP_LOG"))
+    fprintf(stderr, "munit: %s builds image kind %d of %dx%dx%dx%d (ps %d, bf16 %d)\n", who, it.kind, it.Cout, it.KH, it.KW, it.Cin, it.ps, it.bf16);
+  return launch_prep_one(it, st);
 }
 
 template <typename T>
@@ -891,6 +989,29 @@
   return ks > 1 ? align_up((size_t)ks * phases * M * Cout * sizeof(float), 256) : 0;
 }
 
+enum SplitkRoute { SPLITK_NONE = 0, SPLITK_TWO_LAUNCHES = 1, SPLITK_INLAUNCH = 2 };
+struct SplitkPlan {
+  SplitkRoute route;
+  int ksplit, kt_per_split;
+};
+long long splitk_inlaunch_max_bytes(bool vector_stores) {
+  static const char* const e = getenv("MUNIT_SPLITK_INLAUNCH_MAX_BYTES");
+  static const long long v = e ? atoll(e) : 0;
+  return e ? v : vector_stores ? 256 * 1024 : 0;
+}
+SplitkPlan splitk_plan(int M, int Cout, int Ktot, int phases) {
+  SplitkPlan s{SPLITK_NONE, 1, 0};
+  const int ks = pick_ksplit(M, Cout, Ktot, phases);
+  if (ks <= 1) return s;
+  const int nk = cdiv(Ktot, BK), bn = Cout <= 64 ? 64 : 128;
+  s.kt_per_split = cdiv(nk, ks);
+  s.ksplit = cdiv(nk, s.kt_per_split);
+  const bool inlaunch = (long long)s.ksplit * BM * bn * 4 <= splitk_inlaunch_max_bytes(Cout % 4 == 0) &&
+                        !MUNIT_ENV_FLAG("MUNIT_DEBUG_NO_INLAUNCH_SPLITK");
+  s.route = inlaunch ? SPLITK_INLAUNCH : SPLITK_TWO_LAUNCHES;
+  return s;
+}
+
 enum IgemmForm {
   IG_REFUSED_BF16_CIN, IG_REFUSED_CIN4_FOLD, IG_REFUSED_BF16_FOLD, IG_REFUSED_FOLD_UNALIGNED,
   IG_CIN4,
@@ -924,6 +1045,11 @@
     if (bn == 64) hipLaunchKernelGGL((conv_igemm_kernel<64, __VA_ARGS__>), grid, block, 0, st, q);         \
     else hipLaunchKernelGGL((conv_igemm_kernel<128, __VA_ARGS__>), grid, block, 0, st, q);                 \
   } while (0)
+#define IGEMM_LAUNCH_SPLITTABLE(ALIGNED, ROLE, CT)   \
+  do {                                               \
+    if (q.cnt != nullptr) IGEMM_LAUNCH(ALIGNED, ROLE, CT, true); \
+    else IGEMM_LAUNCH(ALIGNED, ROLE, CT);            \
+  } while (0)
 
 template <int ROLE>
 int launch_igemm(const IgemmParams& p, int phases, hipStream_t st, void* slab = nullptr, size_t slab_bytes = 0) {
@@ -952,13 +1078,20 @@
   q.n_tiles = cdiv(p.Cout, bn);
   const int m_tiles = cdiv(p.M, BM);
   q.ksplit = 1;
+  q.cnt = nullptr;
   if (slab != nullptr) {
-    const int ks = pick_ksplit(p.M, p.Cout, p.Ktot, phases);
-    if (ks > 1 && slab_bytes >= splitk_bytes(p.M, p.Cout, p.Ktot, phases)) {
-      const int nk = cdiv(p.Ktot, BK);
-      q.kt_per_split = cdiv(nk, ks);
-      q.ksplit = cdiv(nk, q.kt_per_split);
+    const SplitkPlan sp = splitk_plan(p.M, p.Cout, p.Ktot, phases);
+    if (sp.route != SPLITK_NONE && slab_bytes >= splitk_bytes(p.M, p.Cout, p.Ktot, phases)) {
+      q.kt_per_split = sp.kt_per_split;
+      q.ksplit = sp.ksplit;
       q.slab = reinterpret_cast<float*>(slab);
+      const bool inl_form = form == IG_DMA || form == IG_CT2 || form == IG_CT1 || form == IG_F32 || form == IG_UNALIGNED;
+      if (sp.route == SPLITK_INLAUNCH && inl_form) {
+        MUNIT_CHECK_ARG(m_tiles * q.n_tiles * phases <= MUNIT_SPLITK_COUNTERS, "conv_igemm: %d split tiles, %d counters",
+                        m_tiles * q.n_tiles * phases, MUNIT_SPLITK_COUNTERS);
+        q.cnt = munit_splitk_counters(st);
+        if (q.cnt == nullptr) return MUNIT_ERR_LAUNCH;
+      }
     }
   }
   dim3 grid((unsigned)(m_tiles * q.n_tiles), (unsigned)phases, (unsigned)q.ksplit);
@@ -969,16 +1102,18 @@
       break;
     case IG_BF16S: IGEMM_LAUNCH(true, ROLE, 4); break;
     case IG_PATCH: IGEMM_LAUNCH(true, 2, 3); break;
-    case IG_DMA: IGEMM_LAUNCH(true, ROLE, 3); break;
-    case IG_CT2: IGEMM_LAUNCH(true, ROLE, 2); break;
-    case IG_CT1: IGEMM_LAUNCH(true, ROLE, 1); break;
-    case IG_F32: IGEMM_LAUNCH(true, ROLE); break;
+    case IG_DMA:
+      if constexpr (ROLE != 2) IGEMM_LAUNCH_SPLITTABLE(true, ROLE, 3);
+      break;
+    case IG_CT2: IGEMM_LAUNCH_SPLITTABLE(true, ROLE, 2); break;
+    case IG_CT1: IGEMM_LAUNCH_SPLITTABLE(true, ROLE, 1); break;
+    case IG_F32: IGEMM_LAUNCH_SPLITTABLE(true, ROLE, 0); break;
     default:
-      if constexpr (ROLE != 2) IGEMM_LAUNCH(false, ROLE);
+      if constexpr (ROLE != 2) IGEMM_LAUNCH_SPLITTABLE(false, ROLE, 0);
       break;
   }
   MUNIT_CHECK_LAUNCH("conv_igemm");
-  if (q.ksplit > 1) {
+  if (q.ksplit > 1 && q.cnt == nullptr) {
     const long long total = (long long)p.M * p.Cout * phases;
     const int blocks = (int)std::min<long long>((total + 255) / 256, 4096);
     hipLaunchKernelGGL(splitk_epilogue_kernel, dim3(blocks), dim3(256), 0, st, q, phases);
@@ -1018,6 +1153,8 @@
   return MUNIT_OK;
 }
 
+extern "C" int munit_igemm_splitk_route(int M, int Cout, int Ktot, int phases) { return splitk_plan(M, Cout, Ktot, phases).route; }
+
 namespace {
 bool subpixel_ok(const munit_conv_desc* d) {
   return d->upsample == 1 && d->KH == 5 && d->KW == 5 && d->pad == 2 && d->stride == 1 &&
@@ -1031,32 +1168,20 @@
   for (long long i = (long long)blockIdx.x * blockDim.x + threadIdx.x; i < npix; i += (long long)gridDim.x * blockDim.x)
     x4[i] = f32x4{x[3 * i], x[3 * i + 1], x[3 * i + 2], 0.f};
 }
-__global__ void pad3to4_weight_kernel(const float* __restrict__ w, float* __restrict__ w4, int N, int taps, int kpad) {
-  const long long total = (long long)N * kpad;
-  for (long long i = (long long)blockIdx.x * blockDim.x + threadIdx.x; i < total; i += (long long)gridDim.x * blockDim.x) {
-    const int n = (int)(i / kpad), k = (int)(i - (long long)n * kpad);
-    const int tap = k >> 2, c = k & 3;
-    w4[i] = (tap < taps && c < 3) ? w[((long long)n * taps + tap) * 3 + c] : 0.f;
-  }
-}
 struct Cin4Plan {
   int kpad;
-  size_t x4_bytes, w4_bytes;
+  size_t x4_bytes;
 };
-Cin4Plan plan_cin4(long long npix, int N, int taps) {
+Cin4Plan plan_cin4(long long npix, int taps) {
   Cin4Plan c;
-  c.kpad = (taps * 4 + BK - 1) / BK * BK;
+  c.kpad = cin4_kpad(taps);
   c.x4_bytes = align_up((size_t)npix * 4 * sizeof(float), 256);
-  c.w4_bytes = align_up((size_t)N * c.kpad * sizeof(float), 256);
   return c;
 }
-int build_cin4(const Cin4Plan& c, const float* x3, long long npix, const float* w3, int N, int taps, void* ws, hipStream_t st) {
-  f32x4* x4 = reinterpret_cast<f32x4*>(ws);
-  float* w4 = reinterpret_cast<float*>(reinterpret_cast<char*>(ws) + c.x4_bytes);
-  hipLaunchKernelGGL(pad3to4_image_kernel, dim3((unsigned)std::min<long long>((npix + 255) / 256, 8192)), dim3(256), 0, st, x3, x4, npix);
+int build_cin4(const float* x3, long long npix, void* x4, hipStream_t st) {
+  hipLaunchKernelGGL(pad3to4_image_kernel, dim3((unsigned)std::min<long long>((npix + 255) / 256, 8192)), dim3(256), 0, st, x3,
+                     reinterpret_cast<f32x4*>(x4), npix);
   MUNIT_CHECK_LAUNCH("pad3to4_image");
-  hipLaunchKernelGGL(pad3to4_weight_kernel, dim3((unsigned)cdiv((long long)N * c.kpad, 256)), dim3(256), 0, st, w3, w4, N, taps, c.kpad);
-  MUNIT_CHECK_LAUNCH("pad3to4_weight");
   return MUNIT_OK;
 }
 bool cin4_fwd_ok(const munit_conv_desc* d) {
@@ -1154,7 +1279,7 @@
   const bool bf16 = d->in_dtype == MUNIT_DTYPE_BF16;
   int kind = bf16 ? MUNIT_PREP_CAST : MUNIT_PREP_NONE;
   if (munit_small_fwd_ok(d)) {
-    pl.route = FWD_SMALL; kind = MUNIT_PREP_NONE;
+    pl.route = FWD_SMALL; kind = munit_small_fwd_kernel(d->Cin) == SMALL_FWD_PK ? MUNIT_PREP_HEAD_PK : MUNIT_PREP_NONE;
   } else if (subpixel_ok(d)) {
     const bool wino = subpixel_wino_ok(d);
     pl.route = wino ? FWD_SUBPIXEL_WINO : FWD_SUBPIXEL; kind = wino ? MUNIT_PREP_SUBPIXEL_WINOGRAD : MUNIT_PREP_SUBPIXEL;
@@ -1165,11 +1290,12 @@
     pl.route = FWD_WINO_S2; kind = MUNIT_PREP_WINOGRAD_S2;
   } else {
     pl.route = cin4_fwd_ok(d) ? FWD_CIN4 : FWD_IGEMM;
-  }
-  pl.prep = munit_prep_item{nullptr, nullptr, d->Cout, d->KH, d->KW, d->Cin, kind, 1, pl.route != FWD_SMALL && bf16};
-  pl.ws_bytes = pl.img_bytes = kind == MUNIT_PREP_NONE ? 0 : align_up((size_t)prep_elems(pl.prep) * (bf16 ? 2 : 4), 256);
-  if (pl.route == FWD_SMALL) pl.ws_bytes = munit_small_fwd_workspace(d);
-  if (pl.route == FWD_CIN4) pl.cin4 = plan_cin4((long long)d->B * d->H * d->W, d->Cout, d->KH * d->KW), pl.ws_bytes = pl.cin4.x4_bytes + pl.cin4.w4_bytes;
+    if (pl.route == FWD_CIN4) kind = MUNIT_PREP_CIN4;
+  }
+  const bool img16 = pl.route != FWD_SMALL && bf16;
+  pl.prep = munit_prep_item{nullptr, nullptr, d->Cout, d->KH, d->KW, d->Cin, kind, 1, img16};
+  pl.ws_bytes = pl.img_bytes = kind == MUNIT_PREP_NONE ? 0 : align_up((size_t)prep_elems(pl.prep) * (img16 ? 2 : 4), 256);
+  if (pl.route == FWD_CIN4) pl.cin4 = plan_cin4((long long)d->B * d->H * d->W, d->KH * d->KW), pl.ws_bytes += pl.cin4.x4_bytes;
   if (bf16 || munit_small_fwd_supported(d)) return pl;
   if (pl.ring)
     pl.ws_bytes += std::max(splitk_bytes(d->B * (4 * Wo + 4 * (Ho - 4)), d->Cout, Ktot, 1), splitk_bytes(d->B * (2 * Wo + 2 * (Ho - 2)), d->Cout, Ktot, 1));
@@ -1243,18 +1369,18 @@
     munit_set_error("conv2d_fwd: workspace %zu < %zu", ws_bytes, pl.ws_bytes);
     return MUNIT_ERR_WORKSPACE;
   }
-  if (pl.route == FWD_SMALL) return munit_small_fwd(d, Ho, Wo, x, w, bias, reinterpret_cast<float*>(y), ws, st);
   const float* wimg = w;
   if (pl.prep.kind != MUNIT_PREP_NONE) {
     wimg = reinterpret_cast<const float*>(wp);
     if (wimg == nullptr) {
       munit_prep_item it = pl.prep;
       it.w = w; it.wp = reinterpret_cast<float*>(ws);
-      rc = launch_prep_one(it, st);
+      rc = rebuild_image(it, "conv2d_fwd", st);
       if (rc) return rc;
       wimg = it.wp;
     }
   }
+  if (pl.route == FWD_SMALL) return munit_small_fwd(d, Ho, Wo, x, wimg, bias, reinterpret_cast<float*>(y), st);
   if (pl.route == FWD_WINO || pl.route == FWD_WINO_S2 || pl.route == FWD_SUBPIXEL_WINO) {
     const WinoForm f = pl.route == FWD_WINO ? WINO_FWD : pl.route == FWD_WINO_S2 ? WINO_FWD_S2 : WINO_FWD_SUBPIXEL;
     rc = munit_wino_launch(wino_params(d, Ho, Wo, f, reinterpret_cast<const float*>(x), wimg, bias, reinterpret_cast<float*>(y)), st);
@@ -1263,11 +1389,10 @@
   IgemmParams p = fwd_params(d, Ho, Wo);
   p.x = reinterpret_cast<const float*>(x); p.w = wimg; p.bias = bias; p.y = y;
   if (pl.route == FWD_CIN4) {
-    const long long npix = (long long)d->B * d->H * d->W;
-    rc = build_cin4(pl.cin4, reinterpret_cast<const float*>(x), npix, w, d->Cout, d->KH * d->KW, ws, st);
+    void* const x4 = reinterpret_cast<char*>(ws) + pl.img_bytes;
+    rc = build_cin4(reinterpret_cast<const float*>(x), (long long)d->B * d->H * d->W, x4, st);
     if (rc) return rc;
-    p.x = reinterpret_cast<const float*>(ws);
-    p.w = reinterpret_cast<const float*>(reinterpret_cast<const char*>(ws) + pl.cin4.x4_bytes);
+    p.x = reinterpret_cast<const float*>(x4);
     set_cin4(&p, pl.cin4);
     return launch_igemm<0>(p, 1, st);
   }
@@ -1365,6 +1490,7 @@
     pl.route = DG_WINO; kind = MUNIT_PREP_WINOGRAD_DGRAD;
   } else if (!direct && pl.ps == 1 && munit_small_fwd_supported(&t) && !MUNIT_ENV_FLAG("MUNIT_DEBUG_NO_SMALL_DGRAD")) {
     pl.route = DG_SMALL;
+    if (munit_small_fwd_kernel(t.Cin) == SMALL_FWD_PK) kind = MUNIT_PREP_HEAD_PK_DGRAD;
   } else {
     pl.bf16s = d->out_dtype == MUNIT_DTYPE_BF16;
     const bool foldable = !direct && d->stride == 1 && d->Cout % 32 == 0 && d->KH == d->KW &&
@@ -1383,7 +1509,7 @@
       if (upwino) kind = MUNIT_PREP_SUBPIXEL_WINOGRAD_DGRAD;
     } else if (!direct && pl.ps == 1 && d->Cout == 3 && d->out_dtype == MUNIT_DTYPE_F32 && pl.TH * pl.TW <= 64 && d->Cin % 4 == 0 &&
                NWAVES == 8 && !MUNIT_ENV_FLAG("MUNIT_DEBUG_NO_CIN4")) {
-      pl.route = DG_CIN4;
+      pl.route = DG_CIN4; kind = MUNIT_PREP_CIN4_DGRAD;
     } else {
       pl.route = direct ? DG_DIRECT : DG_CORR;
     }
@@ -1393,14 +1519,14 @@
   size_t g_bytes = align_up((size_t)d->B * pl.Hq * pl.Wq * d->Cin * (d->in_dtype == MUNIT_DTYPE_BF16 ? 2 : 4), 256), tail = 0;
   switch (pl.route) {
     case DG_WINO_S2: case DG_WINO: case DG_FOLD: g_bytes = 256; break;
-    case DG_SMALL: tail = munit_small_fwd_workspace(&t); break;
+    case DG_SMALL: break;
     case DG_FOLD_UPWINO: case DG_FOLD_BOXSUM:
       g_bytes = align_up((size_t)d->B * pl.Ho * pl.Wo * d->Cout * sizeof(float), 256);
       tail = pl.slab_bytes = splitk_bytes(d->B * (4 * d->W + 4 * (d->H - 4)), d->Cin, d->KH * d->KW * d->Cout, 1);
       break;
     case DG_CIN4:
-      pl.cin4 = plan_cin4((long long)d->B * pl.Ho * pl.Wo, d->Cin, pl.TH * pl.TW);
-      tail = pl.cin4.x4_bytes + pl.cin4.w4_bytes;
+      pl.cin4 = plan_cin4((long long)d->B * pl.Ho * pl.Wo, pl.TH * pl.TW);
+      tail = pl.cin4.x4_bytes;
       break;
     case DG_DIRECT: case DG_CORR:
       if (!pl.bf16s)
@@ -1536,7 +1662,7 @@
   if (wt == nullptr) {
     munit_prep_item it = pl.prep;
     it.w = w; it.wp = reinterpret_cast<float*>(ws);
-    rc = launch_prep_one(it, st);
+    rc = rebuild_image(it, "conv2d_dgrad", st);
     if (rc) return rc;
     wt = it.wp;
   }
@@ -1552,7 +1678,7 @@
     }
     case DG_SMALL:
       MUNIT_CHECK_ARG(!dx_bf16, "conv2d_dgrad: the 3-channel data gradient is fp32");
-      rc = munit_small_fwd(&pl.t, pl.Hq, pl.Wq, dy_, wt, nullptr, g, tail, st);
+      rc = munit_small_fwd(&pl.t, pl.Hq, pl.Wq, dy_, wt, nullptr, g, st);
       if (rc) return rc;
       return launch_fold_scalar(d, pl, g, add, dx, st);
     case DG_FOLD_UPWINO: case DG_FOLD_BOXSUM: case DG_FOLD: {
@@ -1590,10 +1716,9 @@
   IgemmParams p = dgrad_corr_params(d, pl);
   p.x = dy; p.w = wt; p.bias = nullptr; p.y = direct ? (void*)dx : (void*)g;
   if (pl.route == DG_CIN4) {
-    rc = build_cin4(pl.cin4, dy, (long long)d->B * pl.Ho * pl.Wo, wt, d->Cin, pl.TH * pl.TW, tail, st);
+    rc = build_cin4(dy, (long long)d->B * pl.Ho * pl.Wo, tail, st);
     if (rc) return rc;
     p.x = reinterpret_cast<const float*>(tail);
-    p.w = reinterpret_cast<const float*>(tail + pl.cin4.x4_bytes);
     set_cin4(&p, pl.cin4);
     rc = launch_igemm<1>(p, 1, st);
   } else {
@@ -1642,15 +1767,22 @@
                            (item->kind != MUNIT_PREP_SUBPIXEL_WINOGRAD_DGRAD ? item->Cin % 8 == 0 && item->Cout % 64 == 0
                                                                        : item->Cout % 8 == 0 && item->Cin % 64 == 0)),
                   "conv2d_prepare_weights: sub-pixel Winograd image needs a 5x5 fp32 filter, Cin %% 8 == 0, Cout %% 64 == 0");
-  MUNIT_CHECK_ARG(item->kind == MUNIT_PREP_DGRAD || item->kind == MUNIT_PREP_SUBPIXEL || wino || spw || ws2 || (item->kind == MUNIT_PREP_CAST && item->bf16),
-                  "conv2d_prepare_weights: bad kind %d", item->kind);
+  const bool cin4 = item->kind == MUNIT_PREP_CIN4 || item->kind == MUNIT_PREP_CIN4_DGRAD;
+  const bool head = item->kind == MUNIT_PREP_HEAD_PK || item->kind == MUNIT_PREP_HEAD_PK_DGRAD;
+  MUNIT_CHECK_ARG(!cin4 || (!item->bf16 && item->ps == 1 && (item->kind == MUNIT_PREP_CIN4 ? item->Cin : item->Cout) == 3),
+                  "conv2d_prepare_weights: the 4-channel-tap image needs fp32, stride 1 and three channels on the contracted side");
+  MUNIT_CHECK_ARG(!head || (!item->bf16 && item->ps == 1 && item->KH == 7 && item->KW == 7 &&
+                            (item->kind == MUNIT_PREP_HEAD_PK ? item->Cout == 3 && item->Cin % 16 == 0 : item->Cin == 3 && item->Cout % 16 == 0)),
+                  "conv2d_prepare_weights: the packed head image needs a 7x7 fp32 filter, 3 channels out and a multiple of 16 in");
+  MUNIT_CHECK_ARG(item->kind == MUNIT_PREP_DGRAD || item->kind == MUNIT_PREP_SUBPIXEL || wino || spw || ws2 || cin4 || head ||
+                  (item->kind == MUNIT_PREP_CAST && item->bf16), "conv2d_prepare_weights: bad kind %d", item->kind);
   MUNIT_CHECK_ARG(!wino || (item->KH == 3 && item->KW == 3 && !item->bf16 &&
                             (item->kind != MUNIT_PREP_WINOGRAD_DGRAD ? item->Cin % 8 == 0 && item->Cout % 64 == 0
                                                                : item->Cout % 8 == 0 && item->Cin % 64 == 0)),
                   "conv2d_prepare_weights: Winograd image needs a 3x3 fp32 filter, K %% 8 == 0, N %% 64 == 0");
   MUNIT_CHECK_ARG(item->ps >= 1 && item->KH % item->ps == 0 && item->KW % item->ps == 0, "conv2d_prepare_weights: bad phase count");
   MUNIT_CHECK_ARG(item->kind != MUNIT_PREP_SUBPIXEL || (item->KH == 5 && item->KW == 5), "conv2d_prepare_weights: sub-pixel needs 5x5");
-  return launch_prep_one(*item, (hipStream_t)stream);
+  return rebuild_image(*item, "conv2d_prepare_weights", (hipStream_t)stream);
 }
 
 extern "C" int munit_conv2d_prepare_weights_batch(const munit_prep_item* items_dev, int n, munit_stream_t stream) {
@@ -1658,6 +1790,29 @@
   hipLaunchKernelGGL(prep_weights_kernel<true>, dim3(64, (unsigned)n), dim3(256), 0, (hipStream_t)stream, items_dev, PrepItem{});
   MUNIT_CHECK_LAUNCH("prep_weights_batch");
   return MUNIT_OK;
+}
+
+extern "C" int munit_conv2d_splitk_shape(const munit_conv_desc* d, int pass, int shape[4]) {
+  if (pass == MUNIT_PASS_FWD) {
+    const FwdPlan pl = plan_fwd(d);
+    if (pl.rc || d->in_dtype == MUNIT_DTYPE_BF16 || munit_small_fwd_supported(d)) return 0;
+    const int Ktot = d->KH * d->KW * d->Cin;
+    if (!pl.ring && pl.route != FWD_IGEMM) return 0;
+    const int M = pl.ring ? d->B * (2 * pl.ring * pl.Wo + 2 * pl.ring * (pl.Ho - 2 * pl.ring)) : d->B * pl.Ho * pl.Wo;
+    if (splitk_bytes(M, d->Cout, Ktot, 1) == 0) return 0;
+    shape[0] = M; shape[1] = d->Cout; shape[2] = Ktot; shape[3] = 1;
+    return 1;
+  }
+  if (pass != MUNIT_PASS_DGRAD) return 0;
+  const DgradPlan pl = plan_dgrad(d);
+  if (pl.rc || pl.slab_bytes == 0) return 0;
+  shape[1] = d->Cin;
+  if (pl.route == DG_FOLD_UPWINO || pl.route == DG_FOLD_BOXSUM) {
+    shape[0] = d->B * (4 * d->W + 4 * (d->H - 4)); shape[2] = d->KH * d->KW * d->Cout; shape[3] = 1;
+  } else {
+    shape[0] = d->B * (pl.Ho + pl.TH - 1) * (pl.Wo + pl.TW - 1); shape[2] = pl.TH * pl.TW * d->Cout; shape[3] = pl.ps * pl.ps;
+  }
+  return 1;
 }
 
 namespace {
diff --git a/munit_amd/csrc/conv_small.hip b/munit_amd/csrc/conv_small.hip
--- a/munit_amd/csrc/conv_small.hip
+++ b/munit_amd/csrc/conv_small.hip
@@ -208,20 +208,6 @@
 constexpr int HP_IDX = 20;
 constexpr int HP_ROW = (HP_CP / 4) * 2 * HP_IDX * 4;
 constexpr int HP_ITEMS = HP_PH * (HP_CP / 4) * 2 * HP_IDX;
-
-__global__ void head_pk_weights_kernel(const float* __restrict__ w, float* __restrict__ wp, int Cin) {
-  const int total = (Cin / HP_CP) * HP_K * 2 * HP_K * 12;
-  for (int i = blockIdx.x * blockDim.x + threadIdx.x; i < total; i += gridDim.x * blockDim.x) {
-    int r = i;
-    const int e = r % 12; r /= 12;
-    const int kw = r % HP_K; r /= HP_K;
-    const int quad = r & 1; r >>= 1;
-    const int kh = r % HP_K;
-    const int pass = r / HP_K;
-    const int co = e < 8 ? (e & 1) : 2, c = e < 8 ? (e >> 1) : e - 8;
-    wp[i] = w[((long long)(co * HP_K + kh) * HP_K + kw) * Cin + pass * HP_CP + quad * 4 + c];
-  }
-}
 
 template <typename XT>
 __global__ __launch_bounds__(256, 4) void conv_head_pk_kernel(SmallParams p, const float* __restrict__ wp) {
@@ -540,13 +526,8 @@
 }
 bool munit_small_wgrad_pk() { return !MUNIT_ENV_FLAG("MUNIT_DEBUG_NO_WGRAD_PK"); }
 
-size_t munit_small_fwd_workspace(const munit_conv_desc* d) {
-  if (munit_small_fwd_kernel(d->Cin) != SMALL_FWD_PK) return 0;
-  return align_up((size_t)(d->Cin / HP_CP) * HP_K * 2 * HP_K * 12 * sizeof(float), 256);
-}
-
 int munit_small_fwd(const munit_conv_desc* d, int Ho, int Wo, const void* x, const float* w, const float* bias,
-                    float* y, void* ws, hipStream_t st) {
+                    float* y, hipStream_t st) {
   SmallParams p{};
   p.x = x; p.w = w; p.bias = bias; p.y = y;
   p.B = d->B; p.H = d->H; p.W = d->W; p.Cin = d->Cin; p.Ho = Ho; p.Wo = Wo;
@@ -557,13 +538,8 @@
   p.tiles_y = cdiv(Ho, k == SMALL_FWD_PK ? HP_TH : k == SMALL_FWD_MFMA ? 8 : 4);
   const dim3 grid((unsigned)((long long)d->B * p.tiles_x * p.tiles_y));
   if (k == SMALL_FWD_PK) {
-    MUNIT_CHECK_ARG(ws != nullptr, "conv_head_pk: null workspace");
-    float* wp = reinterpret_cast<float*>(ws);
-    const int total = (d->Cin / HP_CP) * HP_K * 2 * HP_K * 12;
-    hipLaunchKernelGGL(head_pk_weights_kernel, dim3(cdiv(total, 256)), dim3(256), 0, st, w, wp, d->Cin);
-    MUNIT_CHECK_LAUNCH("head_pk_weights");
-    if (b16) hipLaunchKernelGGL((conv_head_pk_kernel<bf16_t>), grid, dim3(256), 0, st, p, wp);
-    else hipLaunchKernelGGL((conv_head_pk_kernel<float>), grid, dim3(256), 0, st, p, wp);
+    if (b16) hipLaunchKernelGGL((conv_head_pk_kernel<bf16_t>), grid, dim3(256), 0, st, p, w);
+    else hipLaunchKernelGGL((conv_head_pk_kernel<float>), grid, dim3(256), 0, st, p, w);
   } else if (k == SMALL_FWD_MFMA) {
     if (b16) hipLaunchKernelGGL((conv_head_mfma_kernel<bf16_t>), grid, dim3(256), 0, st, p);
     else hipLaunchKernelGGL((conv_head_mfma_kernel<float>), grid, dim3(256), 0, st, p);
diff --git a/munit_amd/csrc/runtime.hip b/munit_amd/csrc/runtime.hip
--- a/munit_amd/csrc/runtime.hip
+++ b/munit_amd/csrc/runtime.hip
@@ -1,5 +1,7 @@
 #include "common.h"
 #include <cstring>
+#include <mutex>
+#include <vector>
 
 namespace {
 thread_local char g_err[512] = "";
@@ -36,3 +38,48 @@
   }
   return MUNIT_OK;
 }
+
+namespace {
+struct CounterRegion {
+  int dev;
+  hipStream_t st;
+  unsigned* cnt;
+};
+std::mutex g_cnt_mutex;
+std::vector<CounterRegion> g_cnt;
+}
+
+unsigned* munit_splitk_counters(hipStream_t st) {
+  int dev = 0;
+  if (hipGetDevice(&dev) != hipSuccess) {
+    munit_set_error("splitk_counters: no current device");
+    return nullptr;
+  }
+  std::lock_guard<std::mutex> lock(g_cnt_mutex);
+  for (const CounterRegion& r : g_cnt)
+    if (r.dev == dev && r.st == st) return r.cnt;
+  unsigned* cnt = nullptr;
+  const size_t bytes = MUNIT_SPLITK_COUNTERS * sizeof(unsigned);
+  if (hipMalloc(reinterpret_cast<void**>(&cnt), bytes) != hipSuccess || hipMemset(cnt, 0, bytes) != hipSuccess ||
+      hipDeviceSynchronize() != hipSuccess) {
+    munit_set_error("splitk_counters: cannot allocate %zu bytes of device memory", bytes);
+    if (cnt != nullptr) (void)hipFree(cnt);
+    return nullptr;
+  }
+  g_cnt.push_back(CounterRegion{dev, st, cnt});
+  return cnt;
+}
+
+extern "C" int munit_debug_splitk_counters_busy(void) {
+  int dev = 0;
+  if (hipGetDevice(&dev) != hipSuccess) return -1;
+  std::lock_guard<std::mutex> lock(g_cnt_mutex);
+  int busy = 0;
+  for (const CounterRegion& r : g_cnt) {
+    if (r.dev != dev) continue;
+    unsigned host[MUNIT_SPLITK_COUNTERS];
+    if (hipMemcpy(host, r.cnt, sizeof(host), hipMemcpyDeviceToHost) != hipSuccess) return -1;
+    for (unsigned v : host) busy += v != 0;
+  }
+  return busy;
+}
```

New measurement: 80.08 images/s, median of 6. No clear change (+0.2%).
